# polarlightman/Scoring-rules-for-Gaussian-process-regression-a-new-approach-to-inference

Measured on AMD Instinct MI355X. Metric: GP fit+predict+CRPS wall-clock (ms) at n=20k full / n=40k FITC; HBM GB/s & MFMA%, higher is better.
Workload: dtype f64; 1 GPU; C3 full GP fit(NLML+LOO-CRPS+LOO-LogS)+predict+score; n=20000, d=8, n_test=5000, kernel=ARD, parallelism=single

## Files before the change

include/gpscore.h:

```cpp
#ifndef GPSCORE_H
#define GPSCORE_H

#include <stdint.h>

#ifdef __cplusplus
extern "C" {
#endif

typedef struct gps_ctx gps_ctx;

enum { GPS_ARD = 0, GPS_RBF = 1 };
enum { GPS_FULL = 0, GPS_LOWER = 1 };

enum {
  GPS_OBJ_NLML = 0,
  GPS_OBJ_LOO_CRPS = 1,
  GPS_OBJ_LOO_LOGS = 2,
  GPS_OBJ_LOGDET = 3,
  GPS_OBJ_QUAD = 4,
  GPS_N_OBJ = 5
};
enum {
  GPS_SC_CRPS = 0, GPS_SC_LOGS = 1, GPS_SC_MSLL = 2, GPS_SC_SMSE = 3,
  GPS_SC_MSE = 4, GPS_SC_COVER = 5, GPS_N_SC = 6
};

#define GPS_ABI_VERSION 800
int gps_version(void);
int gps_build_id(char* out, int cap);
int gps_ctx_create(int device, gps_ctx** out);
int gps_ctx_destroy(gps_ctx* ctx);
const char* gps_last_error(gps_ctx* ctx);
int gps_ctx_set_stream(gps_ctx* ctx, void* hip_stream);
void* gps_ctx_stream(gps_ctx* ctx);
int gps_ctx_synchronize(gps_ctx* ctx);

enum {
  GPS_OPT_OVERLAP = 0,
  GPS_OPT_GEMM_MAP = 3,
  GPS_OPT_TINY_GEMM = 7,
  GPS_OPT_GRAM_REG = 9,
  GPS_OPT_GRAPH = 10,
  GPS_OPT_PRED_PRE = 11,
  GPS_OPT_DAG = 12,
  GPS_OPT_AR_CHUNKS = 15,
  GPS_OPT_DAG_TILES = 13,
  GPS_OPT_STREAM_K = 18,
  GPS_OPT_DAG_WGS = 19,
  GPS_OPT_DAG_GROUP = 17,
  GPS_OPT_SLAB_XCD = 26,
  GPS_OPT_DAG_ORDER = 25,
  GPS_OPT_FITC_DEP = 27,
};
int gps_ctx_set_option(gps_ctx* ctx, int key, int value);

enum { GPS_STAT_GRAPHS = 0, GPS_STAT_GRAPH_CAP = 1, GPS_STAT_GRAPH_OVERFLOW = 2,
       GPS_STAT_DEVICE_BYTES = 3, GPS_STAT_GRAPH_DROPPED = 4, GPS_STAT_GRAPH_EVICTED = 5,
       GPS_N_STATS = 6 };
int gps_ctx_stats(gps_ctx* ctx, int64_t* out, int cap);

int gps_dag_task_list(int T, int flags, uint32_t* out, int cap);

typedef struct gps_gemm_desc {
  int32_t lay_a, lay_b, epi;
  int32_t M, N, K;
  int64_t lda, ldb, ldc;
  double alpha, beta;
  int32_t tri, tri_off;
  int32_t lower_out, mirror;
  int32_t kend;
  int32_t tile, ksplit, map_mode;
  int32_t use_ws, sk_alone, dep_mode;
  int32_t reserved;
  int64_t ld_out, c_kslice_stride;
} gps_gemm_desc;
enum { GPS_GEMM_PLAN_TILE = 0, GPS_GEMM_PLAN_KSPLIT = 1, GPS_GEMM_PLAN_MAP = 2,
       GPS_GEMM_PLAN_SK_DP = 3, GPS_GEMM_PLAN_SK_WGS = 4, GPS_GEMM_PLAN_SLAB_XCD = 5,
       GPS_GEMM_PLAN_GRID_X = 6, GPS_GEMM_PLAN_GRID_Y = 7, GPS_N_GEMM_PLAN = 8 };
int gps_gemm_diag_check(const gps_gemm_desc* d, int have_c, int have_kscale, int have_w,
                        const int32_t* kr, int have_out0, int have_out1);
int gps_gemm_diag(gps_ctx* ctx, const gps_gemm_desc* d, const double* A, const double* B,
                  double* C, const double* kscale, const double* w, const int32_t* kr,
                  double* out0, double* out1, int32_t* plan);
int64_t gps_gemm_schedule(const gps_gemm_desc* d, const int32_t* kr, int have_kscale, int slots,
                          int32_t* plan, int32_t* items, int64_t cap);

int gps_prof_enable(gps_ctx* ctx, int on);
int gps_prof_collect(gps_ctx* ctx, char* json_out, int64_t cap);
int gps_phase_enable(gps_ctx* ctx, int on);
int gps_phase_collect(gps_ctx* ctx, char* json_out, int64_t cap);
int gps_rccl_info(int* version, char* path, int cap);

int gps_gram(gps_ctx* ctx, int kind, const double* X, int64_t n, const double* Xp,
             int64_t m, int d, double log_sf2, const double* log_ell, int n_ell,
             double diag_add, int uplo, double* out);
int gps_potrf(gps_ctx* ctx, int64_t n, double* A, int64_t lda, double* logdet);
int gps_potrs(gps_ctx* ctx, int64_t n, int64_t nrhs, const double* A, int64_t lda,
              const double* B, int64_t ldb, double* X, int64_t ldx);
int gps_diag_inv(gps_ctx* ctx, int64_t n, const double* A, int64_t lda, double* dinv);
int gps_gemm(gps_ctx* ctx, int transA, int transB, int64_t M, int64_t N, int64_t K, double alpha,
             const double* A, int64_t lda, const double* B, int64_t ldb, double beta, double* C,
             int64_t ldc);
int gps_scores(gps_ctx* ctx, const double* mu, const double* var, const double* y,
               int64_t nt, double ytr_mean, double ytr_var_unbiased, double out[GPS_N_SC]);

int gps_full_set_data(gps_ctx* ctx, const double* X, const double* y, int64_t n, int d);
int gps_full_set_test(gps_ctx* ctx, const double* Xt, const double* yt, int64_t nt);
int gps_full_fit(gps_ctx* ctx, int kind, const double* theta, int n_ell,
                 double obj[GPS_N_OBJ], double* mu_loo, double* var_loo);
int gps_full_grad(gps_ctx* ctx, int kind, const double* theta, int n_ell, int objective,
                  double obj[GPS_N_OBJ], double* grad);
int gps_full_predict(gps_ctx* ctx, double* mu, double* var, double sc[GPS_N_SC]);

int gps_fitc_set_data(gps_ctx* ctx, const double* X, const double* y, int64_t n, int d,
                      double ytr_mean, double ytr_var_unbiased, int64_t n_total);
int gps_fitc_set_test(gps_ctx* ctx, const double* Xt, const double* yt, int64_t nt,
                      int64_t nt_total);
int gps_fitc_set_inducing(gps_ctx* ctx, const double* Z, int64_t m);
int gps_fitc_fit(gps_ctx* ctx, const double* theta, int n_ell, double obj[GPS_N_OBJ],
                 double* mu_loo, double* var_loo);
int gps_fitc_grad(gps_ctx* ctx, const double* theta, int n_ell, int objective,
                  double obj[GPS_N_OBJ], double* grad, double* grad_z);
int gps_fitc_predict(gps_ctx* ctx, double* mu, double* var, double sc[GPS_N_SC]);
int gps_fitc_intermediates(gps_ctx* ctx, double* Knm, double* lam, double* Lm_inv, double* Lb_inv,
                           double* Kmm);

enum { GPS_BLOCK_DSS = 0, GPS_BLOCK_KC = 1, GPS_BLOCK_ES = 2 };
int gps_full_blockloo(gps_ctx* ctx, int kind, const double* theta, int n_ell, int nfold,
                      int objective, double* value, double* grad, double* fold_values);
int gps_full_blockloo_es(gps_ctx* ctx, int kind, const double* theta, int n_ell, int nfold,
                         int num_sim, double beta, const double* draws, double* value,
                         double* grad, double* fold_values);
int gps_fitc_blockloo(gps_ctx* ctx, const double* theta, int n_ell, int nfold, int objective,
                      double* value, double* grad, double* grad_z, double* fold_values);
int gps_energy_score(gps_ctx* ctx, const double* m, const double* C, int64_t b, const double* y,
                     int num_sim, double beta, const double* draws, double* out);

int gps_full_predict_cov(gps_ctx* ctx, int64_t r0, int64_t r1, double* mu, double* cov,
                         int64_t ldc);
int gps_fitc_predict_cov(gps_ctx* ctx, int64_t r0, int64_t r1, double* mu, double* cov,
                         int64_t ldc);
enum { GPS_JOINT_DSS = 0, GPS_JOINT_ES = 1 };
int gps_full_predict_joint(gps_ctx* ctx, int nblock, int objective, int num_sim, double beta,
                           const double* draws, double* value, double* block_values);
int gps_fitc_predict_joint(gps_ctx* ctx, int nblock, int objective, int num_sim, double beta,
                           const double* draws, double* value, double* block_values);
int gps_full_predict_draws(gps_ctx* ctx, int64_t r0, int64_t r1, int nsamp, const double* xi,
                           double* out);
int gps_fitc_predict_draws(gps_ctx* ctx, int64_t r0, int64_t r1, int nsamp, const double* xi,
                           double* out);

enum { GPS_SURF_LOO_CRPS = 0, GPS_SURF_INSAMPLE_CRPS = 1, GPS_SURF_NLML = 2, GPS_SURF_LOO_LOGS = 3,
       GPS_N_SURF = 4 };
enum { GPS_SURF_LOGS_ADD_NOISE = 1 };
int gps_full_surface(gps_ctx* ctx, const double* X, const double* y, int64_t n, int d,
                     double log_sf2, const double* ell, int64_t n_ell, const double* noise_sd,
                     int64_t n_noise, int flags, double* out);

int gps_comm_unique_id(char uid[128]);
int gps_comm_init(gps_ctx* ctx, int nranks, int rank, const char uid[128]);
int gps_comm_init_local(gps_ctx* ctx, int nranks, int rank, long long group);
enum { GPS_COMM_NONE = 0, GPS_COMM_RCCL = 1, GPS_COMM_LOCAL = 2 };
int gps_comm_info(gps_ctx* ctx, int* nranks, int* rank, int* kind);
int gps_comm_destroy(gps_ctx* ctx);

#ifdef __cplusplus
}
#endif
#endif
```

scoring-rules-for-gaussian-process-regression-a-new-approach-to-inference_amd/csrc/api.hip:

```cpp
#include "api_internal.h"

namespace gpsapi {

thread_local std::string g_err;

int fail(gps_ctx* ctx, int code, const std::string& msg) {
  if (ctx) ctx->err = msg;
  g_err = msg;
  return code;
}

hipError_t sync_ctx_streams(gps_ctx* ctx) {
  for (hipStream_t st : {ctx->stream, ctx->side, ctx->aux[0], ctx->aux[1]})
    if (st) {
      const hipError_t e = hipStreamSynchronize(st);
      if (e != hipSuccess) return e;
    }
  return hipSuccess;
}

hipError_t drop_graphs_in(gps_ctx* ctx, const void* p, size_t bytes) {
  if (!ctx || !p || ctx->pgraphs.empty()) return hipSuccess;
  const uintptr_t lo = (uintptr_t)p, hi = lo + bytes;
  bool synced = false;
  for (size_t i = 0; i < ctx->pgraphs.size();) {
    bool hit = false;
    for (uintptr_t v : ctx->pgraphs[i].key) hit |= v >= lo && v < hi;
    if (!hit) { ++i; continue; }
    if (!synced) {
      const hipError_t e = sync_ctx_streams(ctx);
      if (e != hipSuccess) return e;
      synced = true;
    }
    const hipError_t e = hipGraphExecDestroy(ctx->pgraphs[i].exec);
    ctx->pgraphs.erase(ctx->pgraphs.begin() + (ptrdiff_t)i);
    ++ctx->graph_dropped;
    if (e != hipSuccess) return e;
  }
  return hipSuccess;
}

void forget_zeroed(gps_ctx* ctx, const void* p, size_t bytes) {
  const uintptr_t lo = (uintptr_t)p, hi = lo + bytes;
  for (auto it = ctx->zeroed.lower_bound(lo); it != ctx->zeroed.end() && it->first < hi;)
    it = ctx->zeroed.erase(it);
}

hipError_t ensure(gps_ctx* ctx, DBuf& b, size_t bytes) {
  if (bytes == 0) bytes = 16;
  if (b.cap >= bytes) return hipSuccess;
  if (b.p) {
    forget_zeroed(ctx, b.p, b.cap);
    hipError_t e = drop_graphs_in(ctx, b.p, b.cap);
    if (e != hipSuccess) return e;
    e = hipFree(b.p);
    if (e != hipSuccess) return e;
  }
  b.p = nullptr;
  b.cap = 0;
  hipError_t e = hipMalloc(&b.p, bytes);
  if (e == hipSuccess) b.cap = bytes;
  return e;
}
void release(gps_ctx* ctx, DBuf& b) {
  if (b.p) {
    forget_zeroed(ctx, b.p, b.cap);
    (void)drop_graphs_in(ctx, b.p, b.cap);
    (void)hipFree(b.p);
  }
  b.p = nullptr;
  b.cap = 0;
}

int get_event(gps_ctx* c) {
  if (c->ev_used == c->ev.size()) {
    hipEvent_t e;
    if (hipEventCreate(&e) != hipSuccess) return -1;
    c->ev.push_back(e);
  }
  return (int)c->ev_used++;
}


int phase_event(gps_ctx* c, hipStream_t st) {
  if (c->ph_used == c->ph_ev.size()) {
    hipEvent_t e;
    if (hipEventCreate(&e) != hipSuccess) return -1;
    c->ph_ev.push_back(e);
  }
  const int i = (int)c->ph_used++;
  return hipEventRecord(c->ph_ev[i], st) == hipSuccess ? i : -1;
}
void phase_mark(gps_ctx* c, const char* name) {
  if (!c->phase) return;
  const int e = phase_event(c, c->stream);
  if (e >= 0) c->ph_marks.push_back({name, e});
}

hipEvent_t sync_event(gps_ctx* c) {
  if (c->sync_used == c->sync_ev.size()) {
    hipEvent_t e;
    if (hipEventCreateWithFlags(&e, hipEventDisableTiming) != hipSuccess) return nullptr;
    c->sync_ev.push_back(e);
  }
  return c->sync_ev[c->sync_used++];
}


GemmParams gp0() {
  GemmParams p;
  memset(&p, 0, sizeof(p));
  p.alpha = 1.0;
  p.ksplit = 1;
  return p;
}

const char* gemm_tag(int al, int bl, int epi, const GemmParams& p) {
  (void)al;
  (void)bl;
  if (epi == EPI_COLRED) return "gemm_trmm_colred";
  if (epi == EPI_ROWSQ || epi == EPI_ROWSQ_DOT) return "gemm_rowsq";
  const int64_t tiles = (int64_t)(p.M / GPS_TILE) * (p.N / GPS_TILE) / (p.lower_out ? 2 : 1);
  const int cls = tiles < 16 ? 0 : (tiles < 256 ? 1 : 2);
  static const char* syrk[3] = {"gemm_syrk_s", "gemm_syrk_m", "gemm_syrk_l"};
  static const char* trmm[3] = {"gemm_trmm_s", "gemm_trmm_m", "gemm_trmm_l"};
  static const char* plain[3] = {"gemm_s", "gemm_m", "gemm_l"};
  if (p.lower_out) return p.ksplit > 1 ? "gemm_syrk_splitk" : syrk[cls];
  return p.tri ? trmm[cls] : plain[cls];
}

double gemm_flops(const GemmParams& p) {
  const double M = p.M, N = p.N, K = p.K;
  if (p.lower_out && p.tri == TRI_K_GE_I) {
    double f = 0.0;
    for (int64_t i = 0; i < p.M; i += GPS_TILE) f += (double)(i + GPS_TILE) * (K - i);
    return 2.0 * GPS_TILE * f;
  }
  if (p.lower_out) return M * (M + 1) * K;
  if ((p.tri == TRI_K_LE_I || p.tri == TRI_K_LE_J) && p.tri_off) {
    const double len = p.tri == TRI_K_LE_I ? M : N, other = p.tri == TRI_K_LE_I ? N : M;
    const double o = p.tri_off, e = std::min<double>(K, o + len);
    return other * (e * e - o * o) + 2.0 * other * K * std::max(0.0, o + len - e);
  }
  if (p.tri) return M * N * K;
  return 2.0 * M * N * K;
}

int gemm(gps_ctx* ctx, int al, int bl, int epi, const GemmParams& p, hipStream_t st,
         GemmLaunchInfo* info) {
  if (!st) st = ctx->stream;
  GemmParams q = p;
  if (q.map_mode == 0) q.map_mode = ctx->gemm_map;
  if (epi == EPI_STORE && (q.ksplit == 1 || q.tile == 64) && !q.ws) {
    DBuf& ws = st == ctx->side      ? ctx->ws_side
               : st == ctx->aux[0] ? ctx->ws_aux[0]
               : st == ctx->aux[1] ? ctx->ws_aux[1]
                                   : ctx->ws_main;
    HIPCHK(ensure(ctx, ws, (size_t)kSplitWsDoubles * 8));
    q.ws = ws.d();
    q.ws_cap = kSplitWsDoubles;
    if (st == ctx->stream && ctx->sk_cnt.p) {
      q.sk_cnt = static_cast<int*>(ctx->sk_cnt.p);
      q.sk_slots = 2 * ctx->ncu;
    }
  }
  std::string tag = gemm_tag(al, bl, epi, p);
  if (ctx->prof > 1) {
    const GemmPlan plan = gemm_plan(epi, q, q.ws ? q.ws_cap : 0);
    char buf[160];
    snprintf(buf, sizeof(buf), " %c%c %dx%dx%d tri%d t%d ks%d ld%lld", al ? 'T' : 'N',
             bl ? 'T' : 'N', p.M, p.N, p.K, (int)p.tri, plan.tile, plan.ksplit, (long long)p.lda);
    tag += buf;
  }
  Prof pr(ctx, tag, gemm_flops(p), 0, st);
  HIPCHK(launch_gemm(al, bl, epi, q, st, info));
  return 0;
}

int gram(gps_ctx* ctx, const char* tag, const double* x, int n, const double* xp, int m, int d,
         const Theta& th, double diag_add, int lower, int pad_identity, double* out, int64_t ldo,
         int M, int N, hipStream_t st) {
  GramParams g;
  memset(&g, 0, sizeof(g));
  g.x = x;
  g.xp = xp;
  g.out = out;
  g.ldo = ldo;
  g.n = n;
  g.m = m;
  g.M = M;
  g.N = N;
  g.d = d;
  g.sf2 = th.sf2;
  g.diag_add = diag_add;
  g.lower = lower;
  g.pad_identity = pad_identity;
  for (int k = 0; k < d; ++k) g.inv_ell[k] = th.inv_ell[k];
  const double elems = lower ? 0.5 * (double)M * (M + 1) : (double)M * N;
  Prof pr(ctx, tag, 0, 8.0 * elems, st);
  HIPCHK(launch_gram(g, st ? st : ctx->stream));
  return 0;
}

int pred_rows(gps_ctx* ctx, int64_t r0, int64_t r1, const double* w, hipStream_t st) {
  const int64_t np = ctx->n_pad, ntp = ctx->nt_pad, tiles_m = np / GPS_TILE;
  GemmParams p = gp0();
  p.A = ctx->Linv.d() + r0 * np; p.lda = np; p.B = ctx->Ksf.d(); p.ldb = np;
  p.M = (int)(r1 - r0); p.N = (int)ntp; p.K = (int)r1; p.tri = TRI_K_LE_I; p.tri_off = (int)r0;
  p.w = w + r0;
  p.out0 = ctx->pslab.d() + (r0 / GPS_TILE) * ntp;
  p.out1 = ctx->pslab.d() + (tiles_m + r0 / GPS_TILE) * ntp;
  p.ld_out = ntp;
  return gemm(ctx, LAY_N, LAY_T, EPI_COLRED, p, st);
}

int fitc_rowsq_cols(gps_ctx* ctx, const double* Lx, int64_t c0, int64_t c1, hipStream_t st) {
  const int64_t np = ctx->fn_pad, mp = ctx->m_pad;
  GemmParams p = gp0();
  p.A = ctx->Knm.d(); p.lda = mp; p.B = Lx + c0 * mp; p.ldb = mp;
  p.M = (int)np; p.N = (int)(c1 - c0); p.K = (int)c1; p.tri = TRI_K_LE_J; p.tri_off = (int)c0;
  p.kend = (int)pad_to(ctx->m, 16);
  p.out0 = ctx->fslab.d() + (c0 / GPS_TILE) * np; p.ld_out = np;
  return gemm(ctx, LAY_N, LAY_T, EPI_ROWSQ, p, st);
}

int fitc_rowsq_dep(gps_ctx* ctx, const double* L, int* sig, int64_t ncols, int mode,
                   hipStream_t st, int64_t nb_dag) {
  const int64_t np = ctx->fn_pad, mp = ctx->m_pad;
  GemmParams p = gp0();
  p.A = ctx->Knm.d(); p.lda = mp; p.B = L; p.ldb = mp;
  p.M = (int)np; p.N = (int)ncols; p.K = (int)ncols; p.tri = TRI_K_LE_J;
  p.kend = (int)pad_to(ctx->m, 16);
  p.out0 = ctx->fslab.d(); p.ld_out = np;
  p.dep_sig = sig; p.dep_q = sig + kSigQueue; p.dep_err = static_cast<int*>(ctx->info.p) + 1;
  p.dep_grid = dag_width(ctx, nb_dag, true); p.dep_mode = mode;
  return gemm(ctx, LAY_N, LAY_T, EPI_ROWSQ, p, st);
}

int dag_list_key(const gps_ctx* ctx, int64_t nb) {
  return (int)(3 * nb + ctx->dag_order);
}

bool dag_block(const gps_ctx* ctx, int64_t nb) { return ctx->dag && nb >= 2 && nb <= ctx->dag_tiles; }

void dag_blocks(const gps_ctx* ctx, int64_t nb, std::vector<int>& sizes, int64_t& cnt) {
  if (nb <= 1) return;
  if (dag_block(ctx, nb)) {
    sizes.push_back((int)nb);
    cnt += dag_cnt_ints((int)nb);
    return;
  }
  dag_blocks(ctx, nb / 2, sizes, cnt);
  dag_blocks(ctx, nb - nb / 2, sizes, cnt);
}

int dag_width(const gps_ctx* ctx, int64_t nb, bool half) {
  const int auto_w = half ? std::max(4, ctx->ncu / 2) : ctx->ncu;
  return (int)std::min<int64_t>(ctx->dag_wgs > 0 ? ctx->dag_wgs : auto_w, std::max<int64_t>(4, 2 * nb * nb));
}

int potrf_inv_rec(gps_ctx* ctx, double* A, int64_t lda, double* Linv, int64_t ldl, double* W,
                  int nb, double* logdiag, int* info, int base, int nreal, double* Lout,
                  int64_t ldlo, bool top) {
  hipStream_t s = ctx->stream;
  if (nb == 1) {
    Prof pr(ctx, "potrf_diag128", 2.0 * 128 * 128 * 128 / 3.0, 0);
    HIPCHK(launch_potrf_leaf(A, lda, Linv, ldl, Lout, ldlo, logdiag, info, base, nreal, s));
    return 0;
  }
  if (dag_block(ctx, nb)) {
    auto it = ctx->dag_lists.find(dag_list_key(ctx, nb));
    const int64_t need = dag_cnt_ints(nb);
    if (it == ctx->dag_lists.end() || ctx->dag_cnt_used + need > (int64_t)(ctx->dag_cnt.cap / 4))
      return fail(ctx, -2, "persistent factorisation: task list / counters not prepared");
    DagParams d;
    d.A = A; d.lda = lda; d.Linv = Linv; d.ldl = ldl; d.Lout = Lout; d.ldlo = ldlo;
    d.logdiag = logdiag; d.info = info; d.base = base; d.nreal = nreal; d.T = nb;
    d.tasks = static_cast<const uint32_t*>(it->second.first.p); d.ntasks = it->second.second;
    d.cnt = static_cast<int*>(ctx->dag_cnt.p) + ctx->dag_cnt_used;
    d.spin_ticks = 200000000ull;
    d.group = ctx->dag_group;
    d.sig = ctx->dag_sig;
    ctx->dag_sig = nullptr;
    ctx->dag_cnt_used += need;
    const double nn = 128.0 * nb;
    Prof pr(ctx, "potrf_dag", 2.0 * nn * nn * nn / 3.0, 0);
    HIPCHK(launch_potrf_dag(d, dag_width(ctx, nb, ctx->dag_half), s));
    return 0;
  }
  const int n1b = nb / 2, n2b = nb - n1b;
  const int n1 = n1b * GPS_TILE, n2 = n2b * GPS_TILE;
  double* A21 = A + (int64_t)n1 * lda;
  double* A22 = A21 + n1;
  double* Li21 = Linv + (int64_t)n1 * ldl;
  double* Li22 = Li21 + n1;
  int rc;
  const bool pre_here = top && ctx->pre.kind == PRE_FITC_Q && ctx->pre.n1 == n1;
  const bool pre_dep = pre_here && ctx->pre.sig && ctx->overlap && dag_block(ctx, n1b);
  auto join_dep = [&]() {
    if (!pre_dep) return;
    hipEvent_t j = sync_event(ctx);
    if (j && hipEventRecord(j, ctx->aux[1]) == hipSuccess) (void)hipStreamWaitEvent(s, j, 0);
  };
  if (pre_dep) {
    hipEvent_t f = sync_event(ctx);
    if (!f) return fail(ctx, -2, "hipEventCreate failed");
    HIPCHK(hipEventRecord(f, s));
    HIPCHK(hipStreamWaitEvent(ctx->aux[1], f, 0));
    if ((rc = fitc_rowsq_dep(ctx, Linv, ctx->pre.sig, n1, 1, ctx->aux[1], n1b))) {
      join_dep();
      return rc;
    }
    ctx->dag_sig = ctx->pre.sig;
  }
  rc = potrf_inv_rec(ctx, A, lda, Linv, ldl, W, n1b, logdiag, info, base, nreal, Lout, ldlo);
  ctx->dag_sig = nullptr;
  if (rc) {
    join_dep();
    return rc;
  }
  {
    GemmParams p = gp0();
    p.A = A21; p.lda = lda; p.B = Linv; p.ldb = ldl; p.C = W; p.ldc = n1;
    p.M = n2; p.N = n1; p.K = n1; p.tri = TRI_K_LE_J;
    if ((rc = gemm(ctx, LAY_N, LAY_T, EPI_STORE, p))) return rc;
  }
  if (Lout) HIPCHK(hipMemcpy2DAsync(Lout + (int64_t)n1 * ldlo, ldlo * 8, W, (size_t)n1 * 8,
                                    (size_t)n1 * 8, n2, hipMemcpyDeviceToDevice, s));
  const bool forked = ctx->overlap;
  hipStream_t ts = forked ? ctx->side : s;
  hipEvent_t fork = sync_event(ctx), join = sync_event(ctx);
  if (!fork || !join) return fail(ctx, -2, "hipEventCreate failed");
  if (forked) {
    HIPCHK(hipEventRecord(fork, s));
    HIPCHK(hipStreamWaitEvent(ts, fork, 0));
  }
  {
    GemmParams p = gp0();
    p.A = W; p.lda = n1; p.B = W; p.ldb = n1; p.C = A22; p.ldc = lda;
    p.M = n2; p.N = n2; p.K = n1; p.alpha = -1.0; p.beta = 1.0; p.lower_out = 1;
    p.sk_alone = forked ? 0 : 1;
    if ((rc = gemm(ctx, LAY_N, LAY_T, EPI_STORE, p))) return rc;
  }
  {
    GemmParams p = gp0();
    p.A = W; p.lda = n1; p.B = Linv; p.ldb = ldl; p.C = A21; p.ldc = lda;
    p.M = n2; p.N = n1; p.K = n1; p.tri = TRI_K_GE_J;
    if ((rc = gemm(ctx, LAY_N, LAY_N, EPI_STORE, p, ts))) return rc;
  }
  if (forked) HIPCHK(hipEventRecord(join, ts));
  if (pre_here) {
    hipStream_t ps = !ctx->overlap ? s : pre_dep ? ctx->aux[1] : ctx->aux[0];
    if (ps != s) {
      hipEvent_t f = sync_event(ctx);
      ctx->pre.join = sync_event(ctx);
      if (!f || !ctx->pre.join) return fail(ctx, -2, "hipEventCreate failed");
      HIPCHK(hipEventRecord(f, s));
      HIPCHK(hipStreamWaitEvent(ps, f, 0));
    }
    if ((rc = pre_dep ? fitc_rowsq_dep(ctx, Linv, ctx->pre.sig, n1, 2, ps, n1b)
                      : fitc_rowsq_cols(ctx, Linv, 0, n1, ps)))
      return rc;
    if (ps != s) HIPCHK(hipEventRecord(ctx->pre.join, ps));
  }
  if ((rc = potrf_inv_rec(ctx, A22, lda, Li22, ldl, W + (int64_t)n1 * n2, n2b, logdiag + n1, info,
                          base + n1, nreal - n1, Lout ? Lout + (int64_t)n1 * ldlo + n1 : nullptr,
                          ldlo)))
    return rc;
  if (forked) HIPCHK(hipStreamWaitEvent(s, join, 0));
  {
    GemmParams p = gp0();
    p.A = Li22; p.lda = ldl; p.B = A21; p.ldb = lda; p.C = Li21; p.ldc = ldl;
    p.M = n2; p.N = n1; p.K = n2; p.alpha = -1.0; p.tri = TRI_K_LE_I;
    if ((rc = gemm(ctx, LAY_N, LAY_N, EPI_STORE, p))) return rc;
  }
  if (top && ctx->pre.join) {
    HIPCHK(hipStreamWaitEvent(s, ctx->pre.join, 0));
    ctx->pre.join = nullptr;
  }
  return 0;
}

size_t potrf_ws_doubles(int64_t n_pad) {
  int64_t nb = n_pad / GPS_TILE, tot = 0;
  while (nb > 1) {
    const int64_t n1 = (nb / 2) * GPS_TILE, n2 = (nb - nb / 2) * GPS_TILE;
    tot += n1 * n2;
    nb = nb - nb / 2;
  }
  return (size_t)std::max<int64_t>(tot, GPS_TILE * GPS_TILE);
}

int reset_info(gps_ctx* ctx) {
  HIPCHK(hipMemsetAsync(ctx->info.p, 0x7f, 2 * sizeof(int), ctx->stream));
  return 0;
}


hipError_t zero_factor(gps_ctx* ctx, double* p, int64_t n_pad, hipStream_t s) {
  const hipError_t e = hipMemsetAsync(p, 0, (size_t)n_pad * n_pad * 8, s);
  if (e == hipSuccess) ctx->zeroed[(uintptr_t)p] = n_pad;
  return e;
}
bool factor_zeroed(const gps_ctx* ctx, const double* p, int64_t n_pad) {
  const auto it = ctx->zeroed.find((uintptr_t)p);
  return it != ctx->zeroed.end() && it->second == n_pad;
}

int potrf_inv(gps_ctx* ctx, double* A, int64_t n_pad, double* Linv, double* W, double* logdiag,
              int nreal, double* Lout) {
  if (!factor_zeroed(ctx, Linv, n_pad) || (Lout && !factor_zeroed(ctx, Lout, n_pad)))
    return fail(ctx, -1, "potrf_inv: factor buffer not zeroed for this size (internal contract)");
  std::vector<int> dsizes;
  int64_t dcnt = 0;
  dag_blocks(ctx, n_pad / GPS_TILE, dsizes, dcnt);
  for (int T : dsizes) {
    const int lk = dag_list_key(ctx, T);
    if (ctx->dag_lists.count(lk)) continue;
    const std::vector<uint32_t> tl = dag_task_list(T, ctx->dag_order, true);
    auto& e = ctx->dag_lists[lk];
    HIPCHK(ensure(ctx, e.first, tl.size() * 4));
    HIPCHK(hipMemcpyAsync(e.first.p, tl.data(), tl.size() * 4, hipMemcpyHostToDevice, ctx->stream));
    HIPCHK(hipStreamSynchronize(ctx->stream));
    e.second = (int)tl.size();
  }
  if (dcnt && ctx->dag_cnt.cap < (size_t)dcnt * 4) {
    HIPCHK(hipStreamSynchronize(ctx->stream));
    HIPCHK(ensure(ctx, ctx->dag_cnt, std::max<size_t>((size_t)dcnt * 4, (size_t)1 << 20)));
    HIPCHK(hipMemsetAsync(ctx->dag_cnt.p, 0, ctx->dag_cnt.cap, ctx->stream));
    HIPCHK(hipStreamSynchronize(ctx->stream));
  }
  auto eager = [&]() {
    ctx->sync_used = 0;
    ctx->pre.join = nullptr;
    ctx->dag_cnt_used = 0;
    return potrf_inv_rec(ctx, A, n_pad, Linv, n_pad, W, (int)(n_pad / GPS_TILE), logdiag,
                         static_cast<int*>(ctx->info.p), 0, nreal, Lout, n_pad, true);
  };
  if (!ctx->graphs || ctx->prof || n_pad <= GPS_TILE) return eager();
  HIPCHK(ensure(ctx, ctx->ws_main, (size_t)kSplitWsDoubles * 8));
  HIPCHK(ensure(ctx, ctx->ws_side, (size_t)kSplitWsDoubles * 8));
  const bool pre = ctx->pre.kind == PRE_FITC_Q;
  std::vector<uintptr_t> key = {
      (uintptr_t)A, (uintptr_t)n_pad, (uintptr_t)Linv, (uintptr_t)W, (uintptr_t)logdiag,
      (uintptr_t)nreal, (uintptr_t)Lout, (uintptr_t)ctx->stream, (uintptr_t)ctx->side,
      (uintptr_t)ctx->overlap, (uintptr_t)ctx->gemm_map,
      (uintptr_t)g_tiny_gemm, (uintptr_t)g_stream_k, (uintptr_t)g_slab_xcd, (uintptr_t)ctx->info.p, (uintptr_t)ctx->ws_main.p,
      (uintptr_t)ctx->ws_side.p, (uintptr_t)pre,
      pre ? (uintptr_t)ctx->pre.n1 : 0, pre ? (uintptr_t)ctx->aux[0] : 0,
      pre ? (uintptr_t)ctx->Knm.p : 0, pre ? (uintptr_t)ctx->fslab.p : 0,
      pre ? (uintptr_t)ctx->fn_pad : 0, pre ? (uintptr_t)ctx->m_pad : 0, pre ? (uintptr_t)ctx->pre.sig : 0,
      (uintptr_t)ctx->dag, (uintptr_t)ctx->dag_tiles, (uintptr_t)ctx->dag_group, (uintptr_t)ctx->dag_wgs, (uintptr_t)ctx->dag_half,
      (uintptr_t)ctx->dag_cnt.p, (uintptr_t)ctx->sk_cnt.p, (uintptr_t)ctx->dag_sig};
  for (int T : dsizes) key.push_back((uintptr_t)ctx->dag_lists[dag_list_key(ctx, T)].first.p);
  for (auto& g : ctx->pgraphs)
    if (g.key == key) {
      g.last_use = ++ctx->graph_tick;
      HIPCHK(hipGraphLaunch(g.exec, ctx->stream));
      return 0;
    }
  if (ctx->pgraphs.size() >= kMaxGraphs) {
    size_t lru = 0;
    for (size_t i = 1; i < ctx->pgraphs.size(); ++i)
      if (ctx->pgraphs[i].last_use < ctx->pgraphs[lru].last_use) lru = i;
    HIPCHK(sync_ctx_streams(ctx));
    const hipError_t e = hipGraphExecDestroy(ctx->pgraphs[lru].exec);
    ctx->pgraphs.erase(ctx->pgraphs.begin() + (ptrdiff_t)lru);
    ++ctx->graph_evicted;
    HIPCHK(e);
  }
  const size_t nev = 2 * (size_t)(n_pad / GPS_TILE) + 8;
  while (ctx->sync_ev.size() < nev) {
    hipEvent_t e;
    HIPCHK(hipEventCreateWithFlags(&e, hipEventDisableTiming));
    ctx->sync_ev.push_back(e);
  }
  HIPCHK(hipStreamBeginCapture(ctx->stream, hipStreamCaptureModeThreadLocal));
  int rc = eager();
  hipGraph_t graph = nullptr;
  const hipError_t ec = hipStreamEndCapture(ctx->stream, &graph);
  if (rc || ec != hipSuccess) {
    if (graph) (void)hipGraphDestroy(graph);
    if (rc) return rc;
    HIPCHK(ec);
  }
  hipGraphExec_t exec = nullptr;
  const hipError_t ei = hipGraphInstantiate(&exec, graph, nullptr, nullptr, 0);
  (void)hipGraphDestroy(graph);
  HIPCHK(ei);
  ctx->pgraphs.push_back({key, exec, ++ctx->graph_tick});
  HIPCHK(hipGraphLaunch(exec, ctx->stream));
  return 0;
}

int check_info(gps_ctx* ctx) {
  HIPCHK(hipMemcpyAsync(ctx->hinfo, ctx->info.p, 2 * sizeof(int), hipMemcpyDeviceToHost, ctx->stream));
  HIPCHK(hipStreamSynchronize(ctx->stream));
  if (ctx->hinfo[1] == 2)
    return fail(ctx, -4, "persistent factorisation: the task queue did not run to completion "
                         "(counters not zero at launch; internal error)");
  if (ctx->hinfo[1] != 0x7f7f7f7f)
    return fail(ctx, -4, "persistent factorisation: a task's dependency wait timed out (internal error)");
  const int info = *ctx->hinfo;
  if (info != 0x7f7f7f7f) {
    char buf[160];
    snprintf(buf, sizeof(buf),
             "cholesky: the leading minor of order %d is not positive definite", info);
    return fail(ctx, info, buf);
  }
  return 0;
}

int set_theta(gps_ctx* ctx, Theta& th, int kind, const double* theta, int n_ell, int d) {
  ARGCHK(theta != nullptr, "theta is NULL");
  ARGCHK(kind == GPS_ARD || kind == GPS_RBF, "kind must be GPS_ARD or GPS_RBF");
  ARGCHK(n_ell == 1 || n_ell == d, "n_ell must be 1 or d");
  th.kind = kind;
  th.sf2 = std::exp(theta[0]);
  th.sn2 = std::exp(theta[1 + n_ell]);
  for (int k = 0; k < d; ++k) {
    const double b = theta[1 + (n_ell == 1 ? 0 : k)];
    th.inv_ell[k] = kind == GPS_ARD ? std::exp(-b) : std::exp(-0.5 * b);
  }
  return 0;
}

int upload(gps_ctx* ctx, DBuf& b, const double* h, int64_t rows, int64_t cols, int64_t rows_pad) {
  HIPCHK(ensure(ctx, b, (size_t)rows_pad * cols * 8));
  HIPCHK(hipMemsetAsync(b.p, 0, (size_t)rows_pad * cols * 8, ctx->stream));
  if (rows * cols)
    HIPCHK(hipMemcpyAsync(b.p, h, (size_t)rows * cols * 8, hipMemcpyHostToDevice, ctx->stream));
  return 0;
}

void score_bundle(const double* sums, double nt, double out[GPS_N_SC]) {
  out[GPS_SC_CRPS] = sums[0] / nt;
  out[GPS_SC_LOGS] = sums[1] / nt;
  out[GPS_SC_MSLL] = sums[2] / nt;
  out[GPS_SC_SMSE] = sums[3] / sums[4];
  out[GPS_SC_MSE] = sums[3] / nt;
  out[GPS_SC_COVER] = sums[5] / nt;
}

int bind(gps_ctx* ctx) {
  if (!ctx) {
    g_err = "NULL context";
    return -1;
  }
  HIPCHK(hipSetDevice(ctx->device));
  return 0;
}

bool sharded(const gps_ctx* ctx) { return ctx->comm != nullptr || ctx->lgroup != nullptr; }



std::vector<DBuf*> ctx_buffers(gps_ctx* ctx) {
  return {&ctx->info, &ctx->small, &ctx->X, &ctx->y, &ctx->Xt, &ctx->yt, &ctx->A,
                 &ctx->Linv, &ctx->W, &ctx->logdiag, &ctx->beta, &ctx->alpha, &ctx->dinv,
                 &ctx->slab, &ctx->mu_loo, &ctx->var_loo, &ctx->Ksf, &ctx->s1, &ctx->s2,
                 &ctx->mu, &ctx->var, &ctx->Lout, &ctx->pslab, &ctx->fX, &ctx->fy, &ctx->fXt, &ctx->fyt,
                 &ctx->Z, &ctx->Kmm, &ctx->Am, &ctx->Lm, &ctx->Lb, &ctx->ldm, &ctx->ldb,
                 &ctx->Knm, &ctx->q, &ctx->lam, &ctx->ilam, &ctx->ys, &ctx->slabB, &ctx->red,
                 &ctx->c, &ctx->tvec, &ctx->r, &ctx->g, &ctx->fmu_loo, &ctx->fvar_loo,
                 &ctx->Ksm, &ctx->qm, &ctx->qb, &ctx->fmu, &ctx->fvar, &ctx->fslab, &ctx->fslab_pre, &ctx->t0,
                 &ctx->t1, &ctx->t2, &ctx->t3, &ctx->t4, &ctx->ws_main, &ctx->ws_side, &ctx->ws_aux[0], &ctx->ws_aux[1],
                 &ctx->gu, &ctx->gct, &ctx->gv, &ctx->Mx, &ctx->gslab, &ctx->gout, &ctx->fgv,
                 &ctx->fgm, &ctx->fgB, &ctx->fR, &ctx->fgred, &ctx->fgslab, &ctx->fgout, &ctx->bP,
                 &ctx->bL, &ctx->bPI, &ctx->bH, &ctx->bvec, &ctx->bGblk, &ctx->bT, &ctx->bkr,
                 &ctx->bEf, &ctx->bF, &ctx->ebuf, &ctx->edraws,
                 &ctx->bSg, &ctx->bBf, &ctx->bLf, &ctx->bldf, &ctx->bRem, &ctx->bW, &ctx->bkv,
                 &ctx->bLR, &ctx->bLRv,
                 &ctx->ebuf_aux[0], &ctx->ebuf_aux[1], &ctx->ebuf_aux[2], &ctx->bPIs, &ctx->bRW, &ctx->escale, &ctx->bfv, &ctx->rpart, &ctx->dag_cnt, &ctx->sk_cnt, &ctx->dsig,
                 &ctx->jK, &ctx->jV, &ctx->jslab, &ctx->jS, &ctx->jL, &ctx->jLo, &ctx->jW, &ctx->jvec,
                 &ctx->jE, &ctx->jdraws, &ctx->jxi, &ctx->jout};
}


std::mutex g_groups_mu;
std::map<long long, std::weak_ptr<LocalGroup>> g_groups;

}

extern "C" {

int gps_version(void) { return GPS_ABI_VERSION; }


int make_aux_streams(gps_ctx* ctx) {
  for (hipStream_t* a : {&ctx->side, &ctx->aux[0], &ctx->aux[1]})
    HIPCHK(hipStreamCreateWithFlags(a, hipStreamNonBlocking));
  return 0;
}
int gps_ctx_create(int device, gps_ctx** out) {
  gps_ctx* ctx = nullptr;
  if (!out) return fail(nullptr, -1, "out is NULL");
  int ndev = 0;
  hipError_t e = hipGetDeviceCount(&ndev);
  if (e != hipSuccess || ndev == 0)
    return fail(nullptr, -2, std::string("no HIP device: ") + hipGetErrorString(e));
  if (device < 0 || device >= ndev) return fail(nullptr, -1, "device index out of range");
  ctx = new gps_ctx();
  ctx->device = device;
  HIPCHK(hipSetDevice(device));
  HIPCHK(hipStreamCreateWithFlags(&ctx->stream, hipStreamNonBlocking));
  HIPCHK(hipDeviceGetAttribute(&ctx->ncu, hipDeviceAttributeMultiprocessorCount, device));
  if (int rc = make_aux_streams(ctx)) return rc;
  HIPCHK(hipHostMalloc((void**)&ctx->hsmall, 256 * sizeof(double), hipHostMallocDefault));
  HIPCHK(hipHostMalloc((void**)&ctx->hinfo, 16, hipHostMallocDefault));
  HIPCHK(ensure(ctx, ctx->info, 16));
  HIPCHK(ensure(ctx, ctx->small, 256 * sizeof(double)));
  HIPCHK(ensure(ctx, ctx->sk_cnt, (size_t)kStreamKTiles * sizeof(int)));
  HIPCHK(hipMemsetAsync(ctx->sk_cnt.p, 0, (size_t)kStreamKTiles * sizeof(int), ctx->stream));
  HIPCHK(hipStreamSynchronize(ctx->stream));
  *out = ctx;
  return 0;
}

int gps_ctx_destroy(gps_ctx* ctx) {
  if (!ctx) return 0;
  (void)hipSetDevice(ctx->device);
  for (hipStream_t st : {ctx->stream, ctx->side, ctx->aux[0], ctx->aux[1]})
    if (st) (void)hipStreamSynchronize(st);
  if (ctx->comm) ncclCommDestroy(ctx->comm);
  leave_local_group(ctx);
  for (auto& g : ctx->pgraphs) (void)hipGraphExecDestroy(g.exec);
  ctx->pgraphs.clear();
  for (DBuf* b : ctx_buffers(ctx)) release(ctx, *b);
  for (auto& kv : ctx->dag_lists) release(ctx, kv.second.first);
  for (hipEvent_t e : ctx->ev) (void)hipEventDestroy(e);
  for (hipEvent_t e : ctx->ph_ev) (void)hipEventDestroy(e);
  for (hipEvent_t e : ctx->sync_ev) (void)hipEventDestroy(e);
  for (hipEvent_t e : ctx->ar_ev) (void)hipEventDestroy(e);
  for (hipEvent_t e : {ctx->pre_fork, ctx->pre_join, ctx->preb_fork, ctx->kn_fork, ctx->kn_join,
                       ctx->b_fork, ctx->b_join})
    if (e) (void)hipEventDestroy(e);
  if (ctx->side) (void)hipStreamDestroy(ctx->side);
  for (hipStream_t l : ctx->aux)
    if (l) (void)hipStreamDestroy(l);
  if (ctx->hsmall) (void)hipHostFree(ctx->hsmall);
  if (ctx->hinfo) (void)hipHostFree(ctx->hinfo);
  if (ctx->own_stream && ctx->stream) (void)hipStreamDestroy(ctx->stream);
  delete ctx;
  return 0;
}

const char* gps_last_error(gps_ctx* ctx) { return ctx ? ctx->err.c_str() : g_err.c_str(); }

int gps_ctx_set_stream(gps_ctx* ctx, void* hip_stream) {
  if (int rc = bind(ctx)) return rc;
  HIPCHK(hipStreamSynchronize(ctx->stream));
  if (ctx->own_stream && ctx->stream) HIPCHK(hipStreamDestroy(ctx->stream));
  if (hip_stream) {
    ctx->stream = static_cast<hipStream_t>(hip_stream);
    ctx->own_stream = false;
  } else {
    HIPCHK(hipStreamCreateWithFlags(&ctx->stream, hipStreamNonBlocking));
    ctx->own_stream = true;
  }
  return 0;
}

int gps_ctx_set_option(gps_ctx* ctx, int key, int value) {
  if (int rc = bind(ctx)) return rc;
  switch (key) {
    case GPS_OPT_OVERLAP: ctx->overlap = value != 0; return 0;
    case GPS_OPT_GEMM_MAP:
      ARGCHK(value >= 0 && value <= 6, "GPS_OPT_GEMM_MAP must be in 0..6");
      ctx->gemm_map = value;
      return 0;
    case GPS_OPT_AR_CHUNKS:
      ARGCHK(value >= 1 && value <= 64, "GPS_OPT_AR_CHUNKS must be in 1..64");
      ctx->ar_chunks = value;
      return 0;
    case GPS_OPT_TINY_GEMM: g_tiny_gemm = value != 0; return 0;
    case GPS_OPT_STREAM_K:
      ARGCHK(value >= 0 && value <= 2, "GPS_OPT_STREAM_K must be 0, 1 or 2");
      g_stream_k = value;
      return 0;
    case GPS_OPT_SLAB_XCD: g_slab_xcd = value != 0; return 0;
    case GPS_OPT_GRAM_REG:
      ARGCHK(value >= 0 && value <= 2, "GPS_OPT_GRAM_REG must be 0, 1 or 2");
      g_gram_reg = value;
      return 0;
    case GPS_OPT_GRAPH: ctx->graphs = value != 0; return 0;
    case GPS_OPT_PRED_PRE: ctx->pred_pre = value != 0; return 0;
    case GPS_OPT_DAG: ctx->dag = value != 0; return 0;
    case GPS_OPT_DAG_WGS:
      ARGCHK(value >= 0, "GPS_OPT_DAG_WGS must be >= 0");
      ctx->dag_wgs = value;
      return 0;
    case GPS_OPT_FITC_DEP: ctx->fitc_dep = value != 0; return 0;
    case GPS_OPT_DAG_ORDER:
      ARGCHK(value >= 0 && value <= 2, "GPS_OPT_DAG_ORDER must be 0, 1 or 2");
      ctx->dag_order = value;
      return 0;
    case GPS_OPT_DAG_GROUP:
      ARGCHK(value >= 2 && value <= 4, "GPS_OPT_DAG_GROUP must be 2, 3 or 4");
      ctx->dag_group = value;
      return 0;
    case GPS_OPT_DAG_TILES:
      ARGCHK(value >= 2 && value <= 64, "GPS_OPT_DAG_TILES must be in 2..64");
      ctx->dag_tiles = value;
      return 0;
    default: return fail(ctx, -1, "unknown option");
  }
}

void* gps_ctx_stream(gps_ctx* ctx) { return ctx ? (void*)ctx->stream : nullptr; }

int gps_ctx_synchronize(gps_ctx* ctx) {
  if (int rc = bind(ctx)) return rc;
  HIPCHK(hipStreamSynchronize(ctx->stream));
  return 0;
}

int gps_ctx_stats(gps_ctx* ctx, int64_t* out, int cap) {
  if (int rc = bind(ctx)) return rc;
  ARGCHK(out != nullptr && cap >= 0, "out is NULL or cap < 0");
  size_t bytes = 0;
  for (DBuf* b : ctx_buffers(ctx)) bytes += b->cap;
  int64_t v[GPS_N_STATS];
  v[GPS_STAT_GRAPHS] = (int64_t)ctx->pgraphs.size();
  v[GPS_STAT_GRAPH_CAP] = (int64_t)kMaxGraphs;
  v[GPS_STAT_GRAPH_OVERFLOW] = ctx->graph_overflow;
  v[GPS_STAT_GRAPH_DROPPED] = ctx->graph_dropped;
  v[GPS_STAT_GRAPH_EVICTED] = ctx->graph_evicted;
  v[GPS_STAT_DEVICE_BYTES] = (int64_t)bytes;
  for (int i = 0; i < cap && i < GPS_N_STATS; ++i) out[i] = v[i];
  return GPS_N_STATS;
}

int gps_dag_task_list(int T, int flags, uint32_t* out, int cap) {
  if (T < 2 || T > 64 || cap < 0 || (cap > 0 && !out) || (flags & ~13))
    return fail(nullptr, -1, "bad arguments");
  const std::vector<uint32_t> tl = dag_task_list(T, (flags >> 2 & 3) == 0 ? 1 : (flags >> 2 & 3) == 3 ? 0 : flags >> 2 & 3,
                                                 (flags & 1) != 0);
  for (int i = 0; i < cap && i < (int)tl.size(); ++i) out[i] = tl[i];
  return (int)tl.size();
}

int gps_phase_enable(gps_ctx* ctx, int on) {
  if (int rc = bind(ctx)) return rc;
  ctx->phase = on != 0;
  return 0;
}

int gps_phase_collect(gps_ctx* ctx, char* json_out, int64_t cap) {
  if (int rc = bind(ctx)) return rc;
  HIPCHK(sync_ctx_streams(ctx));
  std::map<std::string, std::pair<int, double>> agg;
  std::vector<std::string> order;
  for (size_t i = 1; i < ctx->ph_marks.size(); ++i) {
    const auto& m = ctx->ph_marks[i];
    if (m.first == "start") continue;
    float ms = 0.f;
    HIPCHK(hipEventElapsedTime(&ms, ctx->ph_ev[ctx->ph_marks[i - 1].second], ctx->ph_ev[m.second]));
    if (!agg.count(m.first)) order.push_back(m.first);
    agg[m.first].first += 1;
    agg[m.first].second += ms;
  }
  std::string js = "{\"phases\": {";
  for (size_t i = 0; i < order.size(); ++i) {
    char buf[160];
    snprintf(buf, sizeof(buf), "%s\"%s\": {\"count\": %d, \"ms\": %.6f}", i ? ", " : "",
             order[i].c_str(), agg[order[i]].first, agg[order[i]].second);
    js += buf;
  }
  js += "}, \"allreduce\": [";
  for (size_t i = 0; i < ctx->ph_ar.size(); ++i) {
    float ms = 0.f;
    HIPCHK(hipEventElapsedTime(&ms, ctx->ph_ev[ctx->ph_ar[i].e0], ctx->ph_ev[ctx->ph_ar[i].e1]));
    char buf[96];
    snprintf(buf, sizeof(buf), "%s[%.0f, %.6f]", i ? ", " : "", ctx->ph_ar[i].bytes, ms);
    js += buf;
  }
  js += "]}";
  ctx->ph_marks.clear();
  ctx->ph_ar.clear();
  ctx->ph_used = 0;
  if (!json_out || cap <= (int64_t)js.size()) return fail(ctx, -1, "json buffer too small");
  memcpy(json_out, js.c_str(), js.size() + 1);
  return 0;
}

int gps_rccl_info(int* version, char* path, int cap) {
  if (!version || !path || cap < 1) return fail(nullptr, -1, "bad arguments");
  *version = 0;
  if (ncclGetVersion(version) != ncclSuccess) return fail(nullptr, -3, "ncclGetVersion failed");
  Dl_info di;
  memset(&di, 0, sizeof(di));
  const char* f = dladdr(reinterpret_cast<void*>(&ncclAllReduce), &di) && di.dli_fname ? di.dli_fname : "";
  snprintf(path, (size_t)cap, "%s", f);
  return 0;
}

int gps_prof_enable(gps_ctx* ctx, int on) {
  if (int rc = bind(ctx)) return rc;
  ctx->prof = on;
  return 0;
}

int gps_prof_collect(gps_ctx* ctx, char* json_out, int64_t cap) {
  if (int rc = bind(ctx)) return rc;
  HIPCHK(hipStreamSynchronize(ctx->stream));
  struct Agg { int count = 0; double ms = 0, flop = 0, bytes = 0; };
  std::map<std::string, Agg> agg;
  for (const ProfRec& r : ctx->recs) {
    float ms = 0.f;
    HIPCHK(hipEventElapsedTime(&ms, ctx->ev[r.e0], ctx->ev[r.e1]));
    Agg& a = agg[r.tag];
    a.count++;
    a.ms += ms;
    a.flop += r.flop;
    a.bytes += r.bytes;
  }
  ctx->recs.clear();
  ctx->ev_used = 0;
  std::string js = "{";
  bool first = true;
  for (auto& kv : agg) {
    char buf[256];
    snprintf(buf, sizeof(buf), "%s\"%s\": {\"count\": %d, \"ms\": %.6f, \"flop\": %.6e, \"bytes\": %.6e}",
             first ? "" : ", ", kv.first.c_str(), kv.second.count, kv.second.ms, kv.second.flop,
             kv.second.bytes);
    js += buf;
    first = false;
  }
  js += "}";
  if (!json_out || cap <= (int64_t)js.size()) return fail(ctx, -1, "json buffer too small");
  memcpy(json_out, js.c_str(), js.size() + 1);
  return 0;
}

int gps_gram(gps_ctx* ctx, int kind, const double* X, int64_t n, const double* Xp, int64_t m, int d,
             double log_sf2, const double* log_ell, int n_ell, double diag_add, int uplo,
             double* out) {
  if (int rc = bind(ctx)) return rc;
  ARGCHK(X && Xp && out && log_ell, "NULL argument");
  ARGCHK(n > 0 && m > 0 && d >= 1 && d <= GPS_MAX_D, "bad shape");
  ARGCHK(uplo == GPS_FULL || (uplo == GPS_LOWER && n == m), "uplo=LOWER needs a square Gram");
  std::vector<double> theta(n_ell + 2);
  theta[0] = log_sf2;
  for (int k = 0; k < n_ell; ++k) theta[1 + k] = log_ell[k];
  theta[1 + n_ell] = 0.0;
  Theta th;
  if (int rc = set_theta(ctx, th, kind, theta.data(), n_ell, d)) return rc;
  const int64_t M = pad_to(n, 32), N = pad_to(m);
  if (int rc = upload(ctx, ctx->t0, X, n, d, n)) return rc;
  if (int rc = upload(ctx, ctx->t1, Xp, m, d, m)) return rc;
  HIPCHK(ensure(ctx, ctx->t2, (size_t)M * N * 8));
  HIPCHK(hipMemsetAsync(ctx->t2.p, 0, (size_t)M * N * 8, ctx->stream));
  if (int rc = gram(ctx, "gram_user", ctx->t0.d(), (int)n, ctx->t1.d(), (int)m, d, th, diag_add,
                    uplo == GPS_LOWER, 0, ctx->t2.d(), N, (int)M, (int)N))
    return rc;
  HIPCHK(hipMemcpy2DAsync(out, (size_t)m * 8, ctx->t2.p, (size_t)N * 8, (size_t)m * 8, n,
                          hipMemcpyDeviceToHost, ctx->stream));
  HIPCHK(hipStreamSynchronize(ctx->stream));
  return 0;
}

int factor_user(gps_ctx* ctx, int64_t n, const double* A, int64_t lda, bool want_L) {
  ARGCHK(A && n > 0 && lda >= n, "bad matrix argument");
  const int64_t np = pad_to(n);
  HIPCHK(ensure(ctx, ctx->t0, (size_t)n * lda * 8));
  HIPCHK(hipMemcpyAsync(ctx->t0.p, A, (size_t)n * lda * 8, hipMemcpyHostToDevice, ctx->stream));
  HIPCHK(ensure(ctx, ctx->t1, (size_t)np * np * 8));
  HIPCHK(launch_pad_copy(ctx->t0.d(), lda, ctx->t1.d(), np, (int)n, (int)n, (int)np, (int)np, 1,
                         ctx->stream));
  HIPCHK(ensure(ctx, ctx->t2, (size_t)np * np * 8));
  HIPCHK(zero_factor(ctx, ctx->t2.d(), np, ctx->stream));
  HIPCHK(ensure(ctx, ctx->t3, potrf_ws_doubles(np) * 8));
  HIPCHK(ensure(ctx, ctx->t4, (size_t)np * 8 * (want_L ? np + 1 : 1)));
  double* logdiag = ctx->t4.d();
  double* Lout = want_L ? ctx->t4.d() + np : nullptr;
  if (want_L) HIPCHK(zero_factor(ctx, Lout, np, ctx->stream));
  if (int rc = reset_info(ctx)) return rc;
  if (int rc = potrf_inv(ctx, ctx->t1.d(), np, ctx->t2.d(), ctx->t3.d(), logdiag, (int)n, Lout))
    return rc;
  return check_info(ctx);
}

int gps_potrf(gps_ctx* ctx, int64_t n, double* A, int64_t lda, double* logdet) {
  if (int rc = bind(ctx)) return rc;
  if (int rc = factor_user(ctx, n, A, lda, true)) return rc;
  const int64_t np = pad_to(n);
  HIPCHK(launch_dot(ctx->t4.d(), nullptr, (int)np, ctx->small.d(), ctx->stream));
  HIPCHK(hipMemcpy2DAsync(A, (size_t)lda * 8, ctx->t4.d() + np, (size_t)np * 8, (size_t)n * 8, n,
                          hipMemcpyDeviceToHost, ctx->stream));
  HIPCHK(hipMemcpyAsync(ctx->hsmall, ctx->small.p, 8, hipMemcpyDeviceToHost, ctx->stream));
  HIPCHK(hipStreamSynchronize(ctx->stream));
  if (logdet) *logdet = 2.0 * ctx->hsmall[0];
  return 0;
}

int gps_potrs(gps_ctx* ctx, int64_t n, int64_t nrhs, const double* A, int64_t lda, const double* B,
              int64_t ldb, double* X, int64_t ldx) {
  if (int rc = bind(ctx)) return rc;
  ARGCHK(B && X && nrhs > 0 && ldb >= nrhs && ldx >= nrhs, "bad rhs argument");
  if (int rc = factor_user(ctx, n, A, lda, false)) return rc;
  const int64_t np = pad_to(n), rp = pad_to(nrhs);
  HIPCHK(ensure(ctx, ctx->t0, (size_t)n * ldb * 8));
  HIPCHK(hipMemcpyAsync(ctx->t0.p, B, (size_t)n * ldb * 8, hipMemcpyHostToDevice, ctx->stream));
  DBuf Bp, Y;
  HIPCHK(ensure(ctx, Bp, (size_t)np * rp * 8));
  HIPCHK(ensure(ctx, Y, (size_t)np * rp * 8));
  int rc = 0;
  do {
    hipError_t e = launch_pad_copy(ctx->t0.d(), ldb, Bp.d(), rp, (int)n, (int)nrhs, (int)np,
                                   (int)rp, 0, ctx->stream);
    if (e != hipSuccess) { rc = fail(ctx, -2, hipGetErrorString(e)); break; }
    GemmParams p = gp0();
    p.A = ctx->t2.d(); p.lda = np; p.B = Bp.d(); p.ldb = rp; p.C = Y.d(); p.ldc = rp;
    p.M = (int)np; p.N = (int)rp; p.K = (int)np; p.tri = TRI_K_LE_I;
    if ((rc = gemm(ctx, LAY_N, LAY_N, EPI_STORE, p))) break;
    GemmParams q = gp0();
    q.A = ctx->t2.d(); q.lda = np; q.B = Y.d(); q.ldb = rp; q.C = Bp.d(); q.ldc = rp;
    q.M = (int)np; q.N = (int)rp; q.K = (int)np; q.tri = TRI_K_GE_I;
    if ((rc = gemm(ctx, LAY_T, LAY_N, EPI_STORE, q))) break;
    e = hipMemcpy2DAsync(X, (size_t)ldx * 8, Bp.p, (size_t)rp * 8, (size_t)nrhs * 8, n,
                         hipMemcpyDeviceToHost, ctx->stream);
    if (e == hipSuccess) e = hipStreamSynchronize(ctx->stream);
    if (e != hipSuccess) rc = fail(ctx, -2, hipGetErrorString(e));
  } while (0);
  release(ctx, Bp);
  release(ctx, Y);
  return rc;
}

int gps_diag_inv(gps_ctx* ctx, int64_t n, const double* A, int64_t lda, double* dinv) {
  if (int rc = bind(ctx)) return rc;
  ARGCHK(dinv, "dinv is NULL");
  if (int rc = factor_user(ctx, n, A, lda, false)) return rc;
  const int64_t np = pad_to(n);
  const int64_t nchunk = (np + 255) / 256;
  HIPCHK(ensure(ctx, ctx->t0, (size_t)(nchunk * np * 2 + np) * 8));
  double* out = ctx->t0.d() + nchunk * np * 2;
  HIPCHK(launch_colred(ctx->t2.d(), np, (int)np, (int)np, 1, nullptr, nullptr, nullptr, out,
                       ctx->t0.d(), ctx->stream));
  HIPCHK(hipMemcpyAsync(dinv, out, (size_t)n * 8, hipMemcpyDeviceToHost, ctx->stream));
  HIPCHK(hipStreamSynchronize(ctx->stream));
  return 0;
}

int gps_gemm(gps_ctx* ctx, int transA, int transB, int64_t M, int64_t N, int64_t K, double alpha,
             const double* A, int64_t lda, const double* B, int64_t ldb, double beta, double* C,
             int64_t ldc) {
  if (int rc = bind(ctx)) return rc;
  ARGCHK(A && B && C && M > 0 && N > 0 && K > 0, "bad gemm argument");
  const int64_t Mp = pad_to(M), Np = pad_to(N), Kp = pad_to(K);
  const int64_t ar = transA ? K : M, ac = transA ? M : K, arp = transA ? Kp : Mp, acp = transA ? Mp : Kp;
  const int64_t br = transB ? N : K, bc = transB ? K : N, brp = transB ? Np : Kp, bcp = transB ? Kp : Np;
  ARGCHK(lda >= ac && ldb >= bc && ldc >= N, "leading dimension too small");
  HIPCHK(ensure(ctx, ctx->t0, (size_t)(ar * lda + br * ldb + M * ldc) * 8));
  double* rawA = ctx->t0.d();
  double* rawB = rawA + ar * lda;
  double* rawC = rawB + br * ldb;
  HIPCHK(hipMemcpyAsync(rawA, A, (size_t)ar * lda * 8, hipMemcpyHostToDevice, ctx->stream));
  HIPCHK(hipMemcpyAsync(rawB, B, (size_t)br * ldb * 8, hipMemcpyHostToDevice, ctx->stream));
  HIPCHK(ensure(ctx, ctx->t1, (size_t)(arp * acp + brp * bcp + Mp * Np) * 8));
  double* pA = ctx->t1.d();
  double* pB = pA + arp * acp;
  double* pC = pB + brp * bcp;
  HIPCHK(launch_pad_copy(rawA, lda, pA, acp, (int)ar, (int)ac, (int)arp, (int)acp, 0, ctx->stream));
  HIPCHK(launch_pad_copy(rawB, ldb, pB, bcp, (int)br, (int)bc, (int)brp, (int)bcp, 0, ctx->stream));
  if (beta != 0.0) {
    HIPCHK(hipMemcpyAsync(rawC, C, (size_t)M * ldc * 8, hipMemcpyHostToDevice, ctx->stream));
    HIPCHK(launch_pad_copy(rawC, ldc, pC, Np, (int)M, (int)N, (int)Mp, (int)Np, 0, ctx->stream));
  }
  GemmParams p = gp0();
  p.A = pA; p.lda = acp; p.B = pB; p.ldb = bcp; p.C = pC; p.ldc = Np;
  p.M = (int)Mp; p.N = (int)Np; p.K = (int)Kp; p.alpha = alpha; p.beta = beta;
  if (int rc = gemm(ctx, transA ? LAY_T : LAY_N, transB ? LAY_T : LAY_N, EPI_STORE, p)) return rc;
  HIPCHK(hipMemcpy2DAsync(C, (size_t)ldc * 8, pC, (size_t)Np * 8, (size_t)N * 8, M,
                          hipMemcpyDeviceToHost, ctx->stream));
  HIPCHK(hipStreamSynchronize(ctx->stream));
  return 0;
}

double* row_part(gps_ctx* ctx, int64_t rows, int nv) {
  if (ensure(ctx, ctx->rpart, (size_t)(std::max<int64_t>(rows, 1) + 255) / 256 * nv * 8) != hipSuccess)
    return nullptr;
  return ctx->rpart.d();
}

int gps_scores(gps_ctx* ctx, const double* mu, const double* var, const double* y, int64_t nt,
               double ytr_mean, double ytr_var_unbiased, double out[GPS_N_SC]) {
  if (int rc = bind(ctx)) return rc;
  ARGCHK(mu && var && y && out && nt > 0, "bad argument");
  if (int rc = upload(ctx, ctx->t0, mu, nt, 1, nt)) return rc;
  if (int rc = upload(ctx, ctx->t1, var, nt, 1, nt)) return rc;
  if (int rc = upload(ctx, ctx->t2, y, nt, 1, nt)) return rc;
  double* part = row_part(ctx, nt, 6);
  ARGCHK(part != nullptr, "out of device memory");
  HIPCHK(launch_score_sums(ctx->t0.d(), ctx->t1.d(), ctx->t2.d(), (int)nt, ytr_mean,
                           ytr_var_unbiased, ctx->small.d(), part, ctx->stream));
  HIPCHK(hipMemcpyAsync(ctx->hsmall, ctx->small.p, 6 * 8, hipMemcpyDeviceToHost, ctx->stream));
  HIPCHK(hipStreamSynchronize(ctx->stream));
  score_bundle(ctx->hsmall, (double)nt, out);
  return 0;
}

}
```

scoring-rules-for-gaussian-process-regression-a-new-approach-to-inference_amd/csrc/api_diag.hip:

```cpp
#include "api_internal.h"

static_assert(sizeof(gps_gemm_desc) == 128, "gps_gemm_desc layout");

namespace gpsapi {

struct DiagExtents {
  int64_t a, b, c, kscale, w, kr, out0, out1;
};

static bool diag_check(const gps_gemm_desc& d, bool have_c, bool have_kscale, bool have_w,
                       const int32_t* kr, bool have_out0, bool have_out1, DiagExtents& x,
                       std::string& why) {
#define DIAG_REQ(cond, msg) \
  do {                      \
    if (!(cond)) {          \
      why = msg;            \
      return false;         \
    }                       \
  } while (0)
  DIAG_REQ(d.dep_mode == 0, "dep_mode: the dependent row-norm launch cannot run alone");
  DIAG_REQ((d.lay_a == LAY_N || d.lay_a == LAY_T) && (d.lay_b == LAY_N || d.lay_b == LAY_T),
           "layouts must be 0 or 1");
  DIAG_REQ(d.epi == EPI_STORE || d.epi == EPI_ROWSQ || d.epi == EPI_COLRED || d.epi == EPI_ROWSQ_DOT,
           "unknown epilogue");
  DIAG_REQ(d.M > 0 && d.N > 0 && d.K > 0 && d.M % GPS_TILE == 0 && d.N % GPS_TILE == 0 && d.K % 16 == 0,
           "M and N must be positive multiples of 128, K of 16");
  DIAG_REQ(d.M <= (1 << 18) && d.N <= (1 << 18) && (int64_t)d.M * d.N <= ((int64_t)1 << 27) &&
               d.K <= 65536,
           "M, N <= 2^18 with M*N <= 2^27, and K <= 65536");
  DIAG_REQ(d.lda > 0 && d.lda % 2 == 0 && d.lda >= (d.lay_a == LAY_N ? d.K : d.M) && d.lda <= (1 << 20),
           "lda must be even and at least A's stored row length");
  DIAG_REQ(d.ldb > 0 && d.ldb % 2 == 0 && d.ldb >= (d.lay_b == LAY_N ? d.N : d.K) && d.ldb <= (1 << 20),
           "ldb must be even and at least B's stored row length");
  DIAG_REQ(d.tri >= TRI_NONE && d.tri <= TRI_KR_J, "unknown tri mode");
  DIAG_REQ(d.tri_off >= 0 && d.tri_off % 16 == 0 && d.tri_off <= (1 << 24),
           "tri_off must be a non-negative multiple of 16");
  DIAG_REQ(d.tri_off == 0 || (d.tri >= TRI_K_LE_I && d.tri <= TRI_K_GE_I),
           "tri_off needs one of the four triangular k-range modes");
  if (d.tri == TRI_KR_J) {
    DIAG_REQ(kr != nullptr, "TRI_KR_J needs kr");
    for (int g = 0; g < 2 * (d.N / 16); ++g)
      DIAG_REQ(kr[g] >= 0 && kr[g] <= d.K && kr[g] % 16 == 0,
               "kr entries must be multiples of 16 in [0, K]");
  }
  DIAG_REQ(d.kend >= 0 && d.kend % 16 == 0, "kend must be 0 or a positive multiple of 16");
  DIAG_REQ((d.lower_out == 0 || d.lower_out == 1) && (d.mirror == 0 || d.mirror == 1),
           "lower_out and mirror are flags");
  DIAG_REQ(!d.lower_out || d.M == d.N, "lower_out needs a square output");
  DIAG_REQ(!d.mirror || d.lower_out, "mirror needs lower_out");
  DIAG_REQ(d.tile == 0 || d.tile == 16 || d.tile == 32 || d.tile == 64 || d.tile == 128,
           "tile must be 0, 16, 32, 64 or 128");
  DIAG_REQ(d.ksplit >= 1 && d.ksplit <= 8, "ksplit must be in 1..8");
  DIAG_REQ(d.map_mode >= 0 && d.map_mode <= 6, "map_mode must be in 0..6");
  DIAG_REQ(d.map_mode != 3 || (!d.lower_out && d.tri >= TRI_K_LE_I && d.tri <= TRI_K_GE_I),
           "map_mode 3 needs a triangular operand and a full output");
  const bool small = d.tile == 16 || d.tile == 32;
  if (small) {
    DIAG_REQ(d.epi == EPI_STORE && !have_kscale, "the small kernel has no epilogue and no kscale");
    DIAG_REQ(d.ksplit == 1 || d.ksplit == 2 || d.ksplit == 4,
             "the small kernel runs 1, 2 or 4 waves per block");
  }
  DIAG_REQ(d.tile != 64 || d.epi == EPI_STORE, "the epilogues run on 128-tiles");
  x = DiagExtents{};
  x.a = (int64_t)(d.lay_a == LAY_N ? d.M : d.K) * d.lda;
  x.b = (int64_t)(d.lay_b == LAY_N ? d.K : d.N) * d.ldb;
  x.kscale = have_kscale ? d.K : 0;
  x.kr = d.tri == TRI_KR_J ? 2 * (d.N / 16) : 0;
  const bool split = !small && d.ksplit > 1;
  if (d.epi == EPI_STORE) {
    DIAG_REQ(have_c, "C is NULL");
    DIAG_REQ(d.ldc > 0 && d.ldc % 2 == 0 && d.ldc >= d.N && d.ldc <= (1 << 20),
             "ldc must be even and at least N");
    x.c = (int64_t)d.M * d.ldc;
    if (split && d.use_ws) {
      DIAG_REQ((int64_t)d.ksplit * d.M * d.N <= kSplitWsDoubles, "the slabs exceed the workspace");
    } else if (split) {
      DIAG_REQ(d.tile == 0 || d.tile == 128, "the unslabbed split runs on 128-tiles");
      DIAG_REQ(d.beta == 0.0 && !d.mirror, "the unslabbed split needs beta 0 and no mirror");
      DIAG_REQ(d.c_kslice_stride % 2 == 0 && d.c_kslice_stride >= x.c &&
                   d.c_kslice_stride <= ((int64_t)1 << 32),
               "c_kslice_stride must be even and at least M*ldc");
      x.c = (int64_t)d.ksplit * d.c_kslice_stride;
    }
  } else {
    DIAG_REQ(d.lay_a == LAY_N && d.lay_b == LAY_T, "the epilogues exist for A [i][k], B [j][k] only");
    DIAG_REQ(d.tile == 0 || d.tile == 128, "the epilogues run on 128-tiles");
    DIAG_REQ(d.ksplit == 1 && !d.mirror, "the epilogues take no split and no mirror");
    DIAG_REQ(have_out0 && d.ld_out > 0 && d.ld_out <= (1 << 20), "out0 / ld_out missing");
    if (d.epi == EPI_COLRED) {
      DIAG_REQ(have_w && have_out1, "EPI_COLRED needs w and out1");
      DIAG_REQ(d.ld_out >= d.N, "ld_out must be at least N");
      x.w = d.M;
      x.out0 = x.out1 = (int64_t)(d.M / GPS_TILE) * d.ld_out;
    } else {
      DIAG_REQ(d.ld_out >= d.M, "ld_out must be at least M");
      x.out0 = (int64_t)(d.N / GPS_TILE) * d.ld_out;
      if (d.epi == EPI_ROWSQ_DOT) {
        DIAG_REQ(have_w && have_out1, "EPI_ROWSQ_DOT needs w and out1");
        DIAG_REQ(d.tri == TRI_K_LE_J && d.K == d.tri_off + d.N,
                 "EPI_ROWSQ_DOT needs TRI_K_LE_J with K = tri_off + N");
        x.w = d.K;
        x.out1 = d.M;
      }
    }
  }
#undef DIAG_REQ
  return true;
}

static GemmParams desc_params(const gps_gemm_desc& d) {
  GemmParams p = gp0();
  p.lda = d.lda; p.ldb = d.ldb; p.ldc = d.ldc; p.c_kslice_stride = d.c_kslice_stride;
  p.M = d.M; p.N = d.N; p.K = d.K; p.alpha = d.alpha; p.beta = d.beta; p.ld_out = d.ld_out;
  p.lower_out = d.lower_out; p.ksplit = d.ksplit; p.tri = d.tri; p.tri_off = d.tri_off;
  p.map_mode = d.map_mode; p.tile = d.tile; p.mirror = d.mirror; p.kend = d.kend;
  p.sk_alone = d.sk_alone;
  return p;
}
static bool own_slabs(const gps_gemm_desc& d) {
  return d.ksplit > 1 && d.tile != 16 && d.tile != 32 && d.tile != 64 && d.use_ws;
}

}

extern "C" {

int gps_gemm_diag_check(const gps_gemm_desc* d, int have_c, int have_kscale, int have_w,
                        const int32_t* kr, int have_out0, int have_out1) {
  if (!d) return fail(nullptr, -1, "description is NULL");
  DiagExtents x;
  std::string why;
  if (!diag_check(*d, have_c != 0, have_kscale != 0, have_w != 0, kr, have_out0 != 0,
                  have_out1 != 0, x, why))
    return fail(nullptr, -1, "gps_gemm_diag: " + why);
  return 0;
}

int gps_gemm_diag(gps_ctx* ctx, const gps_gemm_desc* d, const double* A, const double* B,
                  double* C, const double* kscale, const double* w, const int32_t* kr,
                  double* out0, double* out1, int32_t* plan) {
  if (!d || !A || !B || !plan) return fail(ctx, -1, "gps_gemm_diag: NULL argument");
  DiagExtents x;
  std::string why;
  if (!diag_check(*d, C != nullptr, kscale != nullptr, w != nullptr, kr, out0 != nullptr,
                  out1 != nullptr, x, why))
    return fail(ctx, -1, "gps_gemm_diag: " + why);
  if (int rc = bind(ctx)) return rc;
  hipStream_t s = ctx->stream;
  auto even = [](int64_t n) { return (n + 1) & ~(int64_t)1; };
  HIPCHK(ensure(ctx, ctx->t0, (size_t)(even(x.a) + even(x.b)) * 8));
  HIPCHK(ensure(ctx, ctx->t1, (size_t)std::max<int64_t>(even(x.c), 2) * 8));
  HIPCHK(ensure(ctx, ctx->t2, (size_t)(even(x.kscale) + even(x.w) + even(x.out0) + even(x.out1) +
                                       even((x.kr + 1) / 2) + 2) * 8));
  double* dA = ctx->t0.d();
  double* dB = dA + even(x.a);
  double* dC = ctx->t1.d();
  double* dks = ctx->t2.d();
  double* dw = dks + even(x.kscale);
  double* do0 = dw + even(x.w);
  double* do1 = do0 + even(x.out0);
  int* dkr = reinterpret_cast<int*>(do1 + even(x.out1));
  auto up = [&](void* dst, const void* src, int64_t bytes) {
    return bytes ? hipMemcpyAsync(dst, src, (size_t)bytes, hipMemcpyHostToDevice, s) : hipSuccess;
  };
  HIPCHK(up(dA, A, x.a * 8));
  HIPCHK(up(dB, B, x.b * 8));
  HIPCHK(up(dC, C, x.c * 8));
  HIPCHK(up(dks, kscale, x.kscale * 8));
  HIPCHK(up(dw, w, x.w * 8));
  HIPCHK(up(do0, out0, x.out0 * 8));
  HIPCHK(up(do1, out1, x.out1 * 8));
  HIPCHK(up(dkr, kr, x.kr * 4));
  GemmParams p = desc_params(*d);
  p.A = dA; p.B = dB; p.C = x.c ? dC : nullptr;
  p.kscale = x.kscale ? dks : nullptr;
  p.w = x.w ? dw : nullptr;
  p.out0 = x.out0 ? do0 : nullptr; p.out1 = x.out1 ? do1 : nullptr;
  p.kr = x.kr ? dkr : nullptr;
  if (own_slabs(*d)) {
    HIPCHK(ensure(ctx, ctx->ws_main, (size_t)kSplitWsDoubles * 8));
    p.ws = ctx->ws_main.d();
    p.ws_cap = kSplitWsDoubles;
  }
  GemmLaunchInfo info{};
  if (int rc = gemm(ctx, d->lay_a, d->lay_b, d->epi, p, nullptr, &info)) return rc;
  auto down = [&](void* dst, const void* src, int64_t bytes) {
    return bytes ? hipMemcpyAsync(dst, src, (size_t)bytes, hipMemcpyDeviceToHost, s) : hipSuccess;
  };
  HIPCHK(down(C, dC, x.c * 8));
  HIPCHK(down(out0, do0, x.out0 * 8));
  HIPCHK(down(out1, do1, x.out1 * 8));
  HIPCHK(hipStreamSynchronize(s));
  const int v[GPS_N_GEMM_PLAN] = {info.tile, info.ksplit, info.map_mode, info.sk_dp,
                                  info.sk_wgs, info.slab_xcd, info.grid_x, info.grid_y};
  for (int i = 0; i < GPS_N_GEMM_PLAN; ++i) plan[i] = v[i];
  return 0;
}

int64_t gps_gemm_schedule(const gps_gemm_desc* d, const int32_t* kr, int have_kscale, int slots,
                          int32_t* plan, int32_t* items, int64_t cap) {
  if (!d || !plan || cap < 0 || (cap > 0 && !items) || slots < 0 || slots > 4096)
    return fail(nullptr, -1, "gps_gemm_schedule: bad argument");
  DiagExtents x;
  std::string why;
  if (!diag_check(*d, true, have_kscale != 0, true, kr, true, true, x, why))
    return fail(nullptr, -1, "gps_gemm_schedule: " + why);
  static double mark[2];
  GemmParams p = desc_params(*d);
  p.A = p.B = mark; p.C = p.out0 = p.out1 = mark; p.w = mark;
  p.kscale = have_kscale ? mark : nullptr;
  p.kr = d->tri == TRI_KR_J ? kr : nullptr;
  if (own_slabs(*d) || (d->epi == EPI_STORE && (p.ksplit == 1 || p.tile == 64))) {
    p.ws = mark;
    p.ws_cap = kSplitWsDoubles;
    if (!own_slabs(*d) && slots > 0) {
      p.sk_cnt = reinterpret_cast<int*>(mark);
      p.sk_slots = slots;
    }
  }
  GemmLaunchInfo info{};
  const int64_t n = gemm_schedule(d->lay_a, d->lay_b, d->epi, p, info, items, cap);
  if (n < 0) return fail(nullptr, -1, "gps_gemm_schedule: launch_gemm refuses the launch");
  const int v[GPS_N_GEMM_PLAN] = {info.tile, info.ksplit, info.map_mode, info.sk_dp,
                                  info.sk_wgs, info.slab_xcd, info.grid_x, info.grid_y};
  for (int i = 0; i < GPS_N_GEMM_PLAN; ++i) plan[i] = v[i];
  return n;
}

}
```

scoring-rules-for-gaussian-process-regression-a-new-approach-to-inference_amd/csrc/api_internal.h:

```cpp
#pragma once
#include <dlfcn.h>
#include <rccl/rccl.h>
#include <stdio.h>
#include <string.h>

#include <chrono>
#include <climits>
#include <cmath>
#include <condition_variable>
#include <map>
#include <memory>
#include <mutex>
#include <string>
#include <vector>

#include "gps_internal.h"
#include "gpscore.h"

using namespace gps;

namespace gpsapi {


struct DBuf {
  void* p = nullptr;
  size_t cap = 0;
  double* d() const { return static_cast<double*>(p); }
};

struct ProfRec {
  std::string tag;
  int e0, e1;
  double flop, bytes;
};

struct Theta {
  int kind = GPS_ARD;
  double sf2 = 1.0, sn2 = 1.0;
  double inv_ell[GPS_MAX_D];
};

struct LocalGroup {
  std::mutex mu;
  std::condition_variable cv;
  int n = 0, arrived = 0;
  uint64_t gen = 0;
  size_t count = 0;
  bool mismatch = false, last_mismatch = false;
  bool aborted = false;
  std::vector<std::vector<double>> in;
  std::vector<double> sum;
  std::vector<char> taken;
  int joined = 0;
  int device = -1;
  bool device_ok = true;
  std::vector<double*> stage;
  std::vector<size_t> stage_cap;
  std::vector<hipEvent_t> ready, done;
  std::vector<hipStream_t> gstream;
  std::vector<hipEvent_t> staged, summed;
  ~LocalGroup() {
    for (hipEvent_t e : done)
      if (e) (void)hipEventSynchronize(e);
    for (hipStream_t g : gstream)
      if (g) {
        (void)hipStreamSynchronize(g);
        (void)hipStreamDestroy(g);
      }
    for (const std::vector<hipEvent_t>* v : {&ready, &done, &staged, &summed})
      for (hipEvent_t e : *v)
        if (e) (void)hipEventDestroy(e);
    for (double* p : stage)
      if (p) (void)hipFree(p);
  }
};

extern std::mutex g_groups_mu;
extern std::map<long long, std::weak_ptr<LocalGroup>> g_groups;

}
using namespace gpsapi;


enum { PRE_NONE = 0, PRE_FITC_Q = 1 };

struct gps_ctx {
  int device = 0;
  hipStream_t stream = nullptr;
  bool own_stream = true;
  hipStream_t side = nullptr;
  hipStream_t aux[2] = {nullptr, nullptr};
  bool overlap = true;
  int gemm_map = 0;
  int ar_chunks = 4;
  std::vector<hipEvent_t> ar_ev;
  int ncu = 0;
  std::vector<hipEvent_t> sync_ev;
  size_t sync_used = 0;
  bool graphs = true;
  bool pred_pre = true;
  bool dag = true;
  int dag_tiles = 20;
  int dag_group = 3;
  int dag_wgs = 0;
  int dag_order = 1;
  bool dag_half = false;
  bool fitc_dep = true;
  int* dag_sig = nullptr;
  DBuf dsig;
  std::map<int, std::pair<DBuf, int>> dag_lists;
  std::map<uintptr_t, int64_t> zeroed;
  DBuf dag_cnt;
  DBuf sk_cnt;
  int64_t dag_cnt_used = 0;
  struct PrePass {
    int kind = 0;
    int64_t n1 = 0;
    const double* L = nullptr;
    hipEvent_t join = nullptr;
    int* sig = nullptr;
  } pre;
  struct PotrfGraph {
    std::vector<uintptr_t> key;
    hipGraphExec_t exec = nullptr;
    uint64_t last_use = 0;
  };
  std::vector<PotrfGraph> pgraphs;
  uint64_t graph_tick = 0;
  int64_t graph_overflow = 0;
  int64_t graph_dropped = 0;
  int64_t graph_evicted = 0;
  std::string err;
  int prof = 0;
  std::vector<hipEvent_t> ev;
  size_t ev_used = 0;
  std::vector<ProfRec> recs;
  bool phase = false;
  std::vector<hipEvent_t> ph_ev;
  size_t ph_used = 0;
  std::vector<std::pair<std::string, int>> ph_marks;
  struct PhAr { double bytes; int e0, e1; };
  std::vector<PhAr> ph_ar;
  double* hsmall = nullptr;
  int* hinfo = nullptr;
  DBuf info, small;
  DBuf X, y, Xt, yt, A, Linv, W, logdiag, beta, alpha, dinv, slab, mu_loo, var_loo, Ksf, s1, s2,
      mu, var, Lout, pslab;
  int n_ell = 1;
  DBuf gu, gct, gv, Mx, gslab, gout;
  int64_t n = 0, n_pad = 0, nt = 0, nt_pad = 0;
  int d = 0;
  double ytr_mean = 0, ytr_var = 1;
  bool have_data = false, have_test = false, fitted = false;
  bool have_yt = false, f_have_yt = false;
  Theta th;
  DBuf fX, fy, fXt, fyt, Z, Kmm, Am, Lm, Lb, ldm, ldb, Knm, q, lam, ilam, ys, slabB, red, c, tvec,
      r, g, fmu_loo, fvar_loo, Ksm, qm, qb, fmu, fvar, fslab;
  DBuf fgv, fgm, fgB, fR, fgred, fgslab, fgout;
  DBuf bP, bL, bPI, bH, bvec, bGblk, bT, bkr, bEf, bF, ebuf, edraws;
  DBuf bSg, bBf, bLf, bldf, bRem, bW, bkv;
  DBuf bLR, bLRv;
  DBuf ebuf_aux[3], bPIs, bRW;
  DBuf escale;
  DBuf bfv;
  DBuf rpart;
  DBuf jK, jV, jslab, jS, jL, jLo, jW, jvec, jE, jdraws, jxi, jout;
  int64_t fn = 0, fn_pad = 0, fnt = 0, fnt_pad = 0, m = 0, m_pad = 0, fn_total = 0, fnt_total = 0;
  int fd = 0;
  double f_ytr_mean = 0, f_ytr_var = 1;
  bool f_data = false, f_test = false, f_z = false, f_fitted = false;
  bool f_pre = false;
  bool f_pre_b = false;
  hipEvent_t pre_fork = nullptr, pre_join = nullptr, preb_fork = nullptr;
  hipEvent_t kn_fork = nullptr, kn_join = nullptr;
  hipEvent_t b_fork = nullptr, b_join = nullptr;
  DBuf fslab_pre;
  Theta fth;
  ncclComm_t comm = nullptr;
  std::shared_ptr<LocalGroup> lgroup;
  int nranks = 1, rank = 0;
  DBuf t0, t1, t2, t3, t4;
  DBuf ws_main, ws_side, ws_aux[2];
};


namespace gpsapi {

struct EsArgs {
  int S = 0;
  double beta = 1.0;
  const double* draws = nullptr;
  double lam_lb = 0.0;
  double diag_ub = 0.0;
  double scale = 0.0;
};
std::vector<int64_t> fold_bounds(int64_t n, int nfold);
int es_fold(gps_ctx* ctx, hipStream_t s, DBuf& eb, bool conc, const EsArgs& es, const double* xi_src,
            int64_t b, int64_t bp, const double* PI, const double* r, double trace_c, double* w,
            double* G, int64_t ldg, double* g, double* out);

extern thread_local std::string g_err;
int fail(gps_ctx* ctx, int code, const std::string& msg);

#define HIPCHK(expr)                                                                      \
  do {                                                                                    \
    hipError_t _e = (expr);                                                               \
    if (_e != hipSuccess)                                                                 \
      return fail(ctx, -2, std::string(#expr) + " failed: " + hipGetErrorString(_e));   \
  } while (0)

#define NCCLCHK(expr)                                                                     \
  do {                                                                                    \
    ncclResult_t _r = (expr);                                                             \
    if (_r != ncclSuccess)                                                                \
      return fail(ctx, -3, std::string(#expr) + " failed: " + ncclGetErrorString(_r));  \
  } while (0)

#define ARGCHK(cond, msg)                  \
  do {                                     \
    if (!(cond)) return fail(ctx, -1, msg); \
  } while (0)

constexpr int64_t kSplitWsDoubles = 32ll << 20;
constexpr size_t kMaxGraphs = 64;

int get_event(gps_ctx* c);
struct Prof {
  gps_ctx* c;
  hipStream_t st;
  int e0 = -1;
  std::string tag;
  double flop, bytes;
  Prof(gps_ctx* c_, std::string t, double f, double b, hipStream_t s_ = nullptr)
      : c(c_), st(s_ ? s_ : c_->stream), tag(t), flop(f), bytes(b) {
    if (c->prof && (e0 = get_event(c)) >= 0) (void)hipEventRecord(c->ev[e0], st);
  }
  ~Prof() {
    if (!c->prof || e0 < 0) return;
    const int e1 = get_event(c);
    if (e1 < 0) return;
    (void)hipEventRecord(c->ev[e1], st);
    c->recs.push_back({tag, e0, e1, flop, bytes});
  }
};

hipError_t sync_ctx_streams(gps_ctx* ctx);
hipError_t drop_graphs_in(gps_ctx* ctx, const void* p, size_t bytes);
void forget_zeroed(gps_ctx* ctx, const void* p, size_t bytes);
hipError_t ensure(gps_ctx* ctx, DBuf& b, size_t bytes);
void release(gps_ctx* ctx, DBuf& b);
int get_event(gps_ctx* c);
int phase_event(gps_ctx* c, hipStream_t st);
void phase_mark(gps_ctx* c, const char* name);
hipEvent_t sync_event(gps_ctx* c);
GemmParams gp0();
const char* gemm_tag(int al, int bl, int epi, const GemmParams& p);
double gemm_flops(const GemmParams& p);
int gemm(gps_ctx* ctx, int al, int bl, int epi, const GemmParams& p, hipStream_t st = nullptr,
         GemmLaunchInfo* info = nullptr);
int gram(gps_ctx* ctx, const char* tag, const double* x, int n, const double* xp, int m, int d,
         const Theta& th, double diag_add, int lower, int pad_identity, double* out, int64_t ldo,
         int M, int N, hipStream_t st = nullptr);
int pred_rows(gps_ctx* ctx, int64_t r0, int64_t r1, const double* w, hipStream_t st);
int fitc_rowsq_cols(gps_ctx* ctx, const double* Lx, int64_t c0, int64_t c1, hipStream_t st);
int fitc_rowsq_dep(gps_ctx* ctx, const double* L, int* sig, int64_t ncols, int mode,
                   hipStream_t st, int64_t nb_dag);
int dag_list_key(const gps_ctx* ctx, int64_t nb);
bool dag_block(const gps_ctx* ctx, int64_t nb);
void dag_blocks(const gps_ctx* ctx, int64_t nb, std::vector<int>& sizes, int64_t& cnt);
int dag_width(const gps_ctx* ctx, int64_t nb, bool half);
int potrf_inv_rec(gps_ctx* ctx, double* A, int64_t lda, double* Linv, int64_t ldl, double* W,
                  int nb, double* logdiag, int* info, int base, int nreal, double* Lout,
                  int64_t ldlo, bool top = false);
size_t potrf_ws_doubles(int64_t n_pad);
int reset_info(gps_ctx* ctx);
hipError_t zero_factor(gps_ctx* ctx, double* p, int64_t n_pad, hipStream_t s);
bool factor_zeroed(const gps_ctx* ctx, const double* p, int64_t n_pad);
int potrf_inv(gps_ctx* ctx, double* A, int64_t n_pad, double* Linv, double* W, double* logdiag,
              int nreal, double* Lout);
int check_info(gps_ctx* ctx);
int set_theta(gps_ctx* ctx, Theta& th, int kind, const double* theta, int n_ell, int d);
int upload(gps_ctx* ctx, DBuf& b, const double* h, int64_t rows, int64_t cols, int64_t rows_pad);
void score_bundle(const double* sums, double nt, double out[GPS_N_SC]);
int bind(gps_ctx* ctx);
bool sharded(const gps_ctx* ctx);
std::vector<DBuf*> ctx_buffers(gps_ctx* ctx);
void leave_local_group(gps_ctx* ctx);
int group_barrier(gps_ctx* ctx, LocalGroup& G, size_t count);
int allreduce_sum(gps_ctx* ctx, double* buf, size_t count, hipStream_t s);
int allreduce_sum_impl(gps_ctx* ctx, double* buf, size_t count, hipStream_t s);

}

extern "C" {
int make_aux_streams(gps_ctx* ctx);
int factor_user(gps_ctx* ctx, int64_t n, const double* A, int64_t lda, bool want_L);
double* row_part(gps_ctx* ctx, int64_t rows, int nv);
int full_fit_core(gps_ctx* ctx, int kind, const double* theta, int n_ell);
int fitc_syrk_ks(const gps_ctx* ctx);
int fitc_syrk_rows(gps_ctx* ctx, const double* kscale, int ks, int64_t R0, int64_t R1);
int fitc_syrk(gps_ctx* ctx, const double* kscale, const double* base, double* dst,
              bool packed = false, const double* A = nullptr, int64_t lda = 0);
int fitc_syrk_allreduce(gps_ctx* ctx, double* red, int64_t blen, int64_t tail);
int fitc_test_prepass(gps_ctx* ctx);
int fitc_test_prepass_b(gps_ctx* ctx);
int fitc_fit_core(gps_ctx* ctx, const double* theta, int n_ell, double obj[GPS_N_OBJ],
                  bool pre_test = false);
int fitc_knm_xt(gps_ctx* ctx, int64_t ldc, const double* X, double* C);
int fitc_lt_vec(gps_ctx* ctx, const double* X, const double* x, double* y);
int fitc_tri_right(gps_ctx* ctx, const double* A, int64_t lda, const double* X, double* C,
                   int64_t ldc, int64_t rows);
int fitc_tri_left_t(gps_ctx* ctx, const double* X, const double* B, double* C);
}
```

scoring-rules-for-gaussian-process-regression-a-new-approach-to-inference_amd/csrc/gemm_schedule.h:

```cpp
#pragma once
#include "gps_internal.h"

#define GPS_HD __host__ __device__ __forceinline__

namespace gps {

constexpr int BK = 16;
constexpr int GROUP_M = 8;

GPS_HD int sched_min(int a, int b) { return a < b ? a : b; }

GPS_HD bool tile_of(const GemmParams& p, int t, int& ti, int& tj) {
  if (p.lower_out) {
    int r = (int)((sqrt(8.0 * (double)t + 1.0) - 1.0) * 0.5);
    while ((r + 1) * (r + 2) / 2 <= t) ++r;
    while (r * (r + 1) / 2 > t) --r;
    ti = r;
    tj = t - r * (r + 1) / 2;
    return true;
  }
  if (p.map_mode == 3) {
    const int x = t & 7, i = t >> 3;
    if (p.tri == TRI_K_LE_I || p.tri == TRI_K_GE_I) {
      const int bw = (p.tiles_n + 7) >> 3;
      const int ri = i / bw;
      tj = x * bw + i % bw;
      ti = p.tri == TRI_K_LE_I ? p.tiles_m - 1 - ri : ri;
      return tj < p.tiles_n && ri < p.tiles_m;
    }
    const int bh = (p.tiles_m + 7) >> 3;
    const int cj = i / bh;
    ti = x * bh + i % bh;
    tj = p.tri == TRI_K_LE_J ? p.tiles_n - 1 - cj : cj;
    return ti < p.tiles_m && cj < p.tiles_n;
  }
  if (p.map_mode == 5) {
    const int x = t & 7, i = t >> 3;
    const bool wi = p.tri == TRI_K_LE_I || p.tri == TRI_K_GE_I;
    const int nb = wi ? p.tiles_n : p.tiles_m, nw = wi ? p.tiles_m : p.tiles_n;
    const int bb = (nb + 7) >> 3, per = ((bb + 7) >> 3) * 64;
    const int wg = i / per, rem = i - wg * per, w = rem & 63;
    const int bi = x * bb + (rem >> 6) * 8 + (w & 7), wk = wg * 8 + (w >> 3);
    if (bi >= sched_min(nb, x * bb + bb) || wk >= nw) return false;
    const int widx = (p.tri == TRI_K_LE_I || p.tri == TRI_K_LE_J) ? nw - 1 - wk : wk;
    ti = wi ? widx : bi;
    tj = wi ? bi : widx;
    return true;
  }
  const int per_group = GROUP_M * p.tiles_n;
  const int g = t / per_group;
  const int first = g * GROUP_M;
  const int gm = sched_min(GROUP_M, p.tiles_m - first);
  const int tt = t - g * per_group;
  ti = first + tt % gm;
  tj = tt / gm;
  if (p.map_mode != 0) return true;
  if (p.tri == TRI_K_LE_I) ti = p.tiles_m - 1 - ti;
  else if (p.tri == TRI_K_LE_J) tj = p.tiles_n - 1 - tj;
  return true;
}

GPS_HD int xcd_remap(int b, int nblk) {
  const int q = nblk / 8, r = nblk % 8, x = b % 8;
  return (x < r ? x * (q + 1) : r * (q + 1) + (x - r) * q) + b / 8;
}

GPS_HD bool pair_of(const GemmParams& p, int b, int nblk, int& ri, int& q, int& qh) {
  const int np = (p.tiles_n + 1) >> 1;
  const int l = xcd_remap(b, nblk);
  const int per_group = GROUP_M * np, g = l / per_group, first = g * GROUP_M;
  const int gm = sched_min(GROUP_M, p.tiles_m - first), tt = l - g * per_group;
  ri = first + tt % gm;
  q = tt / gm;
  qh = p.tiles_n - 1 - q;
  return q < qh;
}

GPS_HD void slab_xcd_of(int bx, int by, int nt, int ny, int& t, int& slice) {
  const int l = xcd_remap(bx + by * nt, nt * ny);
  t = l % nt;
  slice = l / nt;
}

GPS_HD void tile_k_range(const GemmParams& p, int row0, int col0, int tile, int& kb, int& ke) {
  kb = 0;
  ke = p.K;
  switch (p.tri) {
    case TRI_K_LE_I: ke = sched_min(ke, p.tri_off + row0 + tile); break;
    case TRI_K_LE_J: ke = sched_min(ke, p.tri_off + col0 + tile); break;
    case TRI_K_GE_J: kb = p.tri_off + col0; break;
    case TRI_K_GE_I: kb = p.tri_off + row0; break;
    case TRI_KR_J:
      kb = p.kr[2 * (col0 / 16)];
      ke = p.kr[2 * ((col0 + tile) / 16 - 1) + 1];
      break;
    default: break;
  }
}

GPS_HD void slice_part(int nk, int parts, int s, int& s0, int& s1) {
  const int q = nk / parts, r = nk % parts;
  s0 = s * q + sched_min(s, r);
  s1 = s0 + q + (s < r ? 1 : 0);
}

template <int TE>
GPS_HD bool small_block_of(const GemmParams& p, int t, int& ti, int& tj) {
  const int tm = p.M / TE, tn = p.N / TE;
  bool valid;
  if (p.lower_out) {
    constexpr int u = 64 / TE;
    auto pre = [](int r) { const int a = r / u, b = r % u; return u * (u * a * (a + 1) / 2 + b * (a + 1)); };
    valid = t < pre(tm);
    if (valid) {
      int lo = 0, hi = tm;
      while (hi - lo > 1) { const int mid = (lo + hi) / 2; if (pre(mid) <= t) lo = mid; else hi = mid; }
      ti = lo;
      tj = t - pre(ti);
    }
  } else {
    valid = t < tm * tn;
    if (valid) { ti = t / tn; tj = t - ti * tn; }
  }
  return valid;
}

struct StreamKPart {
  int64_t I, S;
  GPS_HD int64_t bnd(int64_t q) const { return q * I / S; }
  GPS_HD int owner(int64_t x) const {
    int64_t q = x * S / I;
    while (q + 1 < S && bnd(q + 1) <= x) ++q;
    while (q > 0 && bnd(q) > x) --q;
    return (int)q;
  }
};

}
```

scoring-rules-for-gaussian-process-regression-a-new-approach-to-inference_amd/csrc/gps_internal.h:

```cpp
#pragma once

#include <hip/hip_runtime.h>
#include <stdint.h>

#include <string>
#include <vector>

#define GPS_TILE 128
#define GPS_MAX_D 64

namespace gps {

inline int64_t pad_to(int64_t n, int64_t t = GPS_TILE) { return (n + t - 1) / t * t; }

struct GramParams {
  const double* x;
  const double* xp;
  double* out;
  int64_t ldo;
  int n, m;
  int M, N;
  int d;
  double sf2;
  double diag_add;
  int lower;
  int pad_identity;
  double inv_ell[GPS_MAX_D];
  int edge;
};

enum Layout { LAY_N = 0, LAY_T = 1 };
enum Tri {
  TRI_NONE = 0,
  TRI_K_LE_I = 1,
  TRI_K_LE_J = 2,
  TRI_K_GE_J = 3,
  TRI_K_GE_I = 4,
  TRI_KR_J = 5,
};
enum Epi { EPI_STORE = 0, EPI_ROWSQ = 1, EPI_COLRED = 2, EPI_ROWSQ_DOT = 3 };

struct GemmParams {
  const double* A; int64_t lda;
  const double* B; int64_t ldb;
  double* C; int64_t ldc;
  int64_t c_kslice_stride;
  int M, N, K;
  double alpha, beta;
  const double* kscale;
  const double* w;
  double* out0; double* out1; int64_t ld_out;
  int lower_out;
  int ksplit;
  int tri;
  int tri_off;
  const int* kr;
  int tiles_m, tiles_n;
  int map_mode;
  int tile;
  double* ws;
  int64_t ws_cap;
  int* sk_cnt;
  int sk_slots;
  int sk_dp, sk_wgs;
  int prio;
  int mirror;
  int slab_xcd;
  int kend;
  int sk_alone;
  int* dep_sig; int* dep_q; int* dep_err; int dep_grid; int dep_mode;
};
constexpr int kSigStarted = 0;
constexpr int kSigRowCnt = 64;
constexpr int kSigRdy = 128;
constexpr int kSigQueue = 192;
constexpr int kSigInts = kSigQueue + 8 * 64;

struct GemmPlan { int tile, ksplit; };
GemmPlan gemm_plan(int epi, const GemmParams& p, int64_t ws_cap_doubles);
struct GemmLaunchInfo { int tile, ksplit, map_mode, sk_dp, sk_wgs, slab_xcd, grid_x, grid_y; };
extern int g_gram_reg;
extern int g_tiny_gemm;
extern int g_stream_k;
extern int g_slab_xcd;
constexpr int kStreamKTiles = 4096;

#ifdef __HIPCC__
__device__ __forceinline__ double wave_sum(double v) {
#pragma unroll
  for (int o = 32; o > 0; o >>= 1) v += __shfl_xor(v, o);
  return v;
}

template <int NV>
__device__ void block_sum(double (&v)[NV], double* sh) {
  const int lane = threadIdx.x & 63, wave = threadIdx.x >> 6, nw = blockDim.x >> 6;
#pragma unroll
  for (int q = 0; q < NV; ++q) v[q] = wave_sum(v[q]);
  __syncthreads();
  if (lane == 0)
#pragma unroll
    for (int q = 0; q < NV; ++q) sh[q * 16 + wave] = v[q];
  __syncthreads();
#pragma unroll
  for (int q = 0; q < NV; ++q) {
    double t = 0.0;
    for (int w = 0; w < nw; ++w) t += sh[q * 16 + w];
    v[q] = t;
  }
  __syncthreads();
}

__constant__ static const double g_exp_tab[64][2] = {
    {0x1.0000000000000p+0, 0x0.0p+0}, {0x1.02c9a3e778061p+0, -0x1.19083535b085dp-56},
    {0x1.059b0d3158574p+0, 0x1.d73e2a475b465p-55}, {0x1.0874518759bc8p+0, 0x1.186be4bb284ffp-57},
    {0x1.0b5586cf9890fp+0, 0x1.8a62e4adc610bp-54}, {0x1.0e3ec32d3d1a2p+0, 0x1.03a1727c57b53p-59},
    {0x1.11301d0125b51p+0, -0x1.6c51039449b3ap-54}, {0x1.1429aaea92de0p+0, -0x1.32fbf9af1369ep-54},
    {0x1.172b83c7d517bp+0, -0x1.19041b9d78a76p-55}, {0x1.1a35beb6fcb75p+0, 0x1.e5b4c7b4968e4p-55},
    {0x1.1d4873168b9aap+0, 0x1.e016e00a2643cp-54}, {0x1.2063b88628cd6p+0, 0x1.dc775814a8495p-55},
    {0x1.2387a6e756238p+0, 0x1.9b07eb6c70573p-54}, {0x1.26b4565e27cddp+0, 0x1.2bd339940e9d9p-55},
    {0x1.29e9df51fdee1p+0, 0x1.612e8afad1255p-55}, {0x1.2d285a6e4030bp+0, 0x1.0024754db41d5p-54},
    {0x1.306fe0a31b715p+0, 0x1.6f46ad23182e4p-55}, {0x1.33c08b26416ffp+0, 0x1.32721843659a6p-54},
    {0x1.371a7373aa9cbp+0, -0x1.63aeabf42eae2p-54}, {0x1.3a7db34e59ff7p+0, -0x1.5e436d661f5e3p-56},
    {0x1.3dea64c123422p+0, 0x1.ada0911f09ebcp-55}, {0x1.4160a21f72e2ap+0, -0x1.ef3691c309278p-58},
    {0x1.44e086061892dp+0, 0x1.89b7a04ef80d0p-59}, {0x1.486a2b5c13cd0p+0, 0x1.3c1a3b69062f0p-56},
    {0x1.4bfdad5362a27p+0, 0x1.d4397afec42e2p-56}, {0x1.4f9b2769d2ca7p+0, -0x1.4b309d25957e3p-54},
    {0x1.5342b569d4f82p+0, -0x1.07abe1db13cadp-55}, {0x1.56f4736b527dap+0, 0x1.9bb2c011d93adp-54},
    {0x1.5ab07dd485429p+0, 0x1.6324c054647adp-54}, {0x1.5e76f15ad2148p+0, 0x1.ba6f93080e65ep-54},
    {0x1.6247eb03a5585p+0, -0x1.383c17e40b497p-54}, {0x1.6623882552225p+0, -0x1.bb60987591c34p-54},
    {0x1.6a09e667f3bcdp+0, -0x1.bdd3413b26456p-54}, {0x1.6dfb23c651a2fp+0, -0x1.bbe3a683c88abp-57},
    {0x1.71f75e8ec5f74p+0, -0x1.16e4786887a99p-55}, {0x1.75feb564267c9p+0, -0x1.0245957316dd3p-54},
    {0x1.7a11473eb0187p+0, -0x1.41577ee04992fp-55}, {0x1.7e2f336cf4e62p+0, 0x1.05d02ba15797ep-56},
    {0x1.82589994cce13p+0, -0x1.d4c1dd41532d8p-54}, {0x1.868d99b4492edp+0, -0x1.fc6f89bd4f6bap-54},
    {0x1.8ace5422aa0dbp+0, 0x1.6e9f156864b27p-54}, {0x1.8f1ae99157736p+0, 0x1.5cc13a2e3976cp-55},
    {0x1.93737b0cdc5e5p+0, -0x1.75fc781b57ebcp-57}, {0x1.97d829fde4e50p+0, -0x1.d185b7c1b85d1p-54},
    {0x1.9c49182a3f090p+0, 0x1.c7c46b071f2bep-56}, {0x1.a0c667b5de565p+0, -0x1.359495d1cd533p-54},
    {0x1.a5503b23e255dp+0, -0x1.d2f6edb8d41e1p-54}, {0x1.a9e6b5579fdbfp+0, 0x1.0fac90ef7fd31p-54},
    {0x1.ae89f995ad3adp+0, 0x1.7a1cd345dcc81p-54}, {0x1.b33a2b84f15fbp+0, -0x1.2805e3084d708p-57},
    {0x1.b7f76f2fb5e47p+0, -0x1.5584f7e54ac3bp-56}, {0x1.bcc1e904bc1d2p+0, 0x1.23dd07a2d9e84p-55},
    {0x1.c199bdd85529cp+0, 0x1.11065895048ddp-55}, {0x1.c67f12e57d14bp+0, 0x1.2884dff483cadp-54},
    {0x1.cb720dcef9069p+0, 0x1.503cbd1e949dbp-56}, {0x1.d072d4a07897cp+0, -0x1.cbc3743797a9cp-54},
    {0x1.d5818dcfba487p+0, 0x1.2ed02d75b3707p-55}, {0x1.da9e603db3285p+0, 0x1.c2300696db532p-54},
    {0x1.dfc97337b9b5fp+0, -0x1.1a5cd4f184b5cp-54}, {0x1.e502ee78b3ff6p+0, 0x1.39e8980a9cc8fp-55},
    {0x1.ea4afa2a490dap+0, -0x1.e9c23179c2893p-54}, {0x1.efa1bee615a27p+0, 0x1.dc7f486a4b6b0p-54},
    {0x1.f50765b6e4540p+0, 0x1.9d3e12dd8a18bp-54}, {0x1.fa7c1819e90d8p+0, 0x1.74853f3a5931ep-55},
};
__device__ __forceinline__ void exp_tab_stage(double2* tab) {
  if (threadIdx.x < 64) tab[threadIdx.x] = make_double2(g_exp_tab[threadIdx.x][0], g_exp_tab[threadIdx.x][1]);
}
__device__ __forceinline__ double exp_neg(double x, const double2* tab) {
  x = x < -746.0 ? -746.0 : x;
  const double j = rint(x * 0x1.71547652b82fep+6);
  const int n = (int)j;
  const double r = fma(-j, 0x1.1cf79abc9e3b4p-42, fma(-j, 0x1.62e42fef80000p-7, x));
  const double pr = r * fma(r, fma(r, fma(r, fma(r, 1.0 / 120.0, 1.0 / 24.0), 1.0 / 6.0), 0.5), 1.0);
  const double2 t = tab[n & 63];
  return ldexp(t.x + fma(t.x, pr, t.y), n >> 6);
}

__device__ __forceinline__ double crps_term(double m, double c, double y) {
  const double s = sqrt(c);
  const double z = (y - m) / s;
  const double cdf = 0.5 * (1.0 + erf(z * 0.70710678118654752440));
  const double pdf = 0.39894228040143267794 * exp(-z * z * 0.5);
  return s * (z * (2.0 * cdf - 1.0) + 2.0 * pdf - 0.56418958354775628695);
}
__device__ __forceinline__ double logs_term(double m, double c, double y) {
  const double e = y - m;
  return e * e / (2.0 * c) + log(sqrt(c)) + 0.91893853320467274178;
}
#endif

struct GradParams {
  const double* x;
  int n, d;
  double sf2;
  double inv_ell[GPS_MAX_D];
  const double* Ainv; const double* Mx; int64_t ldm;
  const double* alpha; const double* v;
  double a0, a1, a2, a3;
  double* slab;
};

struct FitcContractParams {
  const double* xr; const double* xc;
  int nr, nc, nc_pad, d;
  double sf2;
  double inv_ell[GPS_MAX_D];
  int nt;
  const double* R[4]; int64_t ldr[4]; double coef[4]; const double* rs[4];
  double pc[2]; const double* pv[2]; const double* qv[2];
  double* slab;
  double* zslab;
  int rchunk;
};

#define GPS_SURFACE_MAX_N 128
struct SurfaceParams {
  const double* x; const double* y;
  int n, d;
  double sf2;
  const double* ell; int nl;
  const double* sd; int ns;
  int logs_add_noise;
  double* out;
};

hipError_t launch_surface(const SurfaceParams& p, hipStream_t s);
hipError_t launch_gram(const GramParams& p, hipStream_t s);
hipError_t launch_gemm(int alay, int blay, int epi, const GemmParams& p, hipStream_t s,
                       GemmLaunchInfo* info = nullptr, GemmParams* resolved = nullptr);
constexpr int kGemmItemInts = 8;
int64_t gemm_schedule(int alay, int blay, int epi, const GemmParams& p, GemmLaunchInfo& info,
                      int32_t* items, int64_t cap);

hipError_t launch_potrf_leaf(const double* A, int64_t lda, double* Linv, int64_t ldl,
                             double* Lout, int64_t ldlo, double* logdiag, int* info,
                             int base, int n_real_in_block, hipStream_t s);

struct DagParams {
  double* A; int64_t lda;
  double* Linv; int64_t ldl;
  double* Lout; int64_t ldlo;
  double* logdiag; int* info; int base; int nreal;
  int T;
  const uint32_t* tasks; int ntasks;
  int* cnt;
  unsigned long long spin_ticks;
  unsigned long long* trace = nullptr;
  int group = 3;
  int* sig = nullptr;
};
hipError_t launch_potrf_dag(const DagParams& p, int nwg, hipStream_t s);
std::vector<uint32_t> dag_task_list(int T, int order = 1, bool fine = true);
inline int64_t dag_cnt_ints(int T) { return (16 + 2 * (int64_t)T * T + 63) / 64 * 64; }

hipError_t launch_gemv_lower(const double* L, int64_t ldl, const double* x, double* y,
                             int n_pad, hipStream_t s);
hipError_t launch_gemv_full(const double* M, int64_t ldm, const double* x, double* y,
                            int rows, int cols, hipStream_t s);
hipError_t launch_colred(const double* M, int64_t ldm, int rows, int cols, int lower,
                         const double* w, const double* rowscale, double* s1, double* s2,
                         double* slab, hipStream_t s, int crows = 256);
hipError_t launch_slab_sum(const double* slab, int64_t ld, int nslab, int64_t len,
                           const double* init, double* out, hipStream_t s);
hipError_t launch_sym_slab_sum(const double* slab, int64_t slice_stride, int nslab, int M,
                               const double* base, double* dst, hipStream_t s);

hipError_t launch_sym_pack(const double* slab, int64_t slice_stride, int nslab, int r0, int r1,
                           int M, double* packed, hipStream_t s);
hipError_t launch_sym_unpack(const double* packed, int m, int M, const double* base, int full,
                             double* dst, hipStream_t s);
hipError_t launch_full_loo(const double* y, const double* slab, int nslab, int64_t ld,
                           const double* beta, const double* logdiag, int n, double* alpha,
                           double* dinv, double* mu_loo, double* var_loo, double* obj,
                           double* part, hipStream_t s);
hipError_t launch_surface_point_sums(const double* y, const double* alpha, const double* dinv,
                                     int n, double s2, int add_noise, double* sums, double* part,
                                     hipStream_t s);
int launch_colred_partials(const double* M, int64_t ldm, int rows, int cols, int lower,
                           const double* w, double* slab, hipStream_t s);
hipError_t launch_pred_finalize(const double* s1, const double* s2, int nt, double base_var,
                                double* mu, double* var, hipStream_t s);
hipError_t launch_fitc_pred_finalize(const double* qm, const double* qb, int nt, double base_var,
                                     double* var, hipStream_t s);
hipError_t launch_score_sums(const double* mu, const double* var, const double* y, int nt,
                             double ytr_mean, double ytr_var, double* sums, double* part,
                             hipStream_t s);
hipError_t launch_fitc_lambda(const double* slab, int64_t ld, int nslab, const double* y, int n,
                              int n_pad, double sf2, double sn2, double* q, double* lam,
                              double* inv_lam, double* ys, double* scal, double* part,
                              hipStream_t s);
hipError_t launch_fitc_loo(const double* y, const double* lam, const double* slab, int64_t ld,
                           int nslab, const double* g, int n, int n_pad, double* r,
                           double* mu_loo, double* var_loo, double* sums, double* part,
                           hipStream_t s);
hipError_t launch_trmv_lower(const double* L, int64_t ldl, const double* x, double* y,
                             int n_pad, int trans, hipStream_t s);
hipError_t launch_dot(const double* a, const double* b, int n, double* out, hipStream_t s);
hipError_t launch_pad_copy(const double* src, int64_t lds, double* dst, int64_t ldd, int rows,
                           int cols, int rows_pad, int cols_pad, int pad_identity, hipStream_t s);

hipError_t launch_loo_grad_terms(const double* y, const double* alpha, const double* dinv, int n,
                                 int n_pad, int obj, double* u, double* ct, hipStream_t s);
hipError_t launch_sym_mirror(double* M, int64_t ld, int n_pad, hipStream_t s);
hipError_t launch_norm_inf(const double* A, int64_t lda, int n, double* rowsum, double* out,
                           hipStream_t s);
int grad_contract_passes(int d);
int64_t grad_contract_slab_doubles(int n, int d);
hipError_t launch_grad_contract(const GradParams& p, double* out, hipStream_t s);

hipError_t launch_fold_terms(const double* y, const double* r, const double* c, int b, double* gm,
                             double* gc, double* out, hipStream_t s);
hipError_t launch_fold_grad(const double* PI, int64_t ldp, const double* H, int64_t ldh,
                            const double* r, const double* w, int b, double c0, double c1,
                            double c2, double c3, double gr, double gw, double* G, int64_t ldg,
                            double* g, hipStream_t s);
hipError_t launch_add_diag(double* P, int64_t ld, const double* vals, int nreal, int npad,
                           hipStream_t s);
hipError_t launch_row_scale(double* M, int64_t ld, int rows, int cols, const double* scale,
                            hipStream_t s);
hipError_t launch_vec_mul(const double* a, const double* b, int n, double* out, hipStream_t s);
hipError_t launch_fold_sum(const double* slab, int64_t stride, int nslab, int skip, const double* base,
                           const double* base2, double sgn, double* dst, int64_t len, hipStream_t s);
constexpr int kLocalSumMax = 64;
struct LocalSumPtrs {
  const double* p[kLocalSumMax];
};
hipError_t launch_local_sum(const LocalSumPtrs& sp, int n, int64_t count, double* out, hipStream_t s);
hipError_t launch_row_dots(const double* A, int64_t lda, const double* B, int64_t ldb,
                           const double* t, int rows, int cols, double* at, double* ab,
                           hipStream_t s);
hipError_t launch_lr_fold_vec(int mode, int b, int bp, const double* lam, const double* x,
                              const double* at, const double* ab, const double* r, const double* c,
                              const double* w, const double* gc, const double* q, double* o1,
                              double* o2, hipStream_t s);
hipError_t launch_lr_combine(const double* X, int64_t ldx, const double* Y, int64_t ldy,
                             const double* lam, const double* rs, double c0, const double* u1,
                             const double* v1, double c1, const double* u2, const double* v2,
                             double c2, int rows, int rows_pad, int cols, double* out, int64_t ldo,
                             hipStream_t s);
hipError_t launch_fold_logdet(const double* ldf, const double* ldb, int m, const double* lam, int b,
                              double* out, hipStream_t s);
hipError_t launch_blk_mdiag(const double* F, int64_t ldf, const double* US, int64_t ldus,
                            const double* U, int64_t ldu, int m_pad, const double* gd,
                            const double* lam, const double* v, const double* alpha, int n,
                            int n_pad, double* md, double* sc, double* Y, int64_t ldy,
                            hipStream_t s);
hipError_t launch_ns_init(const double* C, int64_t ldc, int b, int bp, double scale, double pad,
                          double* Y, hipStream_t s);
hipError_t launch_diag_add_const(double* M, int64_t ld, int n, double c, hipStream_t s);
hipError_t launch_sym_avg(double* M, int64_t ld, int n, hipStream_t s);
hipError_t launch_scaled_row(const double* src, int b, int bp, double scale, double* dst,
                             hipStream_t s);
hipError_t launch_row_axpy(double* C, int64_t ldc, const double* Z, int64_t ldz, const double* sv,
                           int rows, int cols, hipStream_t s);
hipError_t launch_ns_resid(const double* T, int64_t ld, int n, double* out, hipStream_t s);
hipError_t launch_es_dist(const double* Z, const double* Zh, int64_t ld, int S, int bp, double* D,
                          int64_t ldd, hipStream_t s);
hipError_t launch_es_reduce(double* D, int64_t ldd, int S, int Sp, double beta, int grad,
                            double* rs, double* cs, double* out, hipStream_t s);

struct JointCovParams {
  const double* x;
  int b, bp, d;
  double sf2, sn2;
  double inv_ell[GPS_MAX_D];
  const double* slab; int64_t stride; int ks;
  double* out;
};
hipError_t launch_joint_cov(const JointCovParams& p, hipStream_t s);
hipError_t launch_joint_resid(const double* y, const double* mu, int b, int bp, double* r,
                              hipStream_t s);
hipError_t launch_joint_dss(const double* logdiag, const double* t, int b, double* out,
                            hipStream_t s);
hipError_t launch_sign_fill(double* dst, int npos, int n, hipStream_t s);
hipError_t launch_row_add(double* M, int64_t ld, const double* mu, int rows, int cols,
                          hipStream_t s);

hipError_t launch_fitc_grad_terms(const double* y, const double* lam, const double* r,
                                  const double* g, int n, int n_pad, int obj, double n_total,
                                  double* alpha, double* dinv, double* v, double* ulam, double* h,
                                  double* hl2, hipStream_t s);
hipError_t launch_fitc_grad_v(const double* ulam, const double* z, const double* lam, int n,
                              double* v, hipStream_t s);
hipError_t launch_fitc_grad_mdiag(const double* KN, int64_t ldkn, const double* K, int64_t ldk,
                                  int m_pad, const double* lam, const double* r, const double* dinv,
                                  const double* alpha, const double* v, const double* h, double a,
                                  int n, int n_pad, double* mdiag, double* s1, double* s2,
                                  double* s3, hipStream_t s);
hipError_t launch_fitc_grad_y(const double* U, const double* UP, int64_t ld, const double* s1,
                              const double* s2, int rows, int cols, double* Y, hipStream_t s);
int fitc_contract_passes(int d);
int64_t fitc_contract_slab_doubles(int nr, int nc_pad, int d);
hipError_t launch_fitc_grad_contract(FitcContractParams p, double* out, double* zout,
                                     hipStream_t s);

}
```

scoring-rules-for-gaussian-process-regression-a-new-approach-to-inference_amd/csrc/kernels_gemm.hip:

```cpp
#include "gemm_schedule.h"
#include "gps_internal.h"

namespace gps {

typedef double d4 __attribute__((ext_vector_type(4)));
typedef double dv2 __attribute__((ext_vector_type(2)));


__device__ __forceinline__ int dep_band0(int tm, int x) { return (int)((int64_t)tm * x / 8); }
__device__ __forceinline__ int dep_ld(const int* p) {
  return __hip_atomic_load(p, __ATOMIC_RELAXED, __HIP_MEMORY_SCOPE_AGENT);
}
__device__ bool dep_take(const GemmParams& p, double* smem, int& ti, int& tj) {
  const int T = p.tiles_n, tm = p.tiles_m;
  if (p.dep_mode == 2) {
    const int b = (int)blockIdx.x;
    tj = T - 1 - b / tm;
    ti = b - (b / tm) * tm;
    if (tj < 0) return false;
    int x = 7;
    while (x > 0 && dep_band0(tm, x) > ti) --x;
    const int len = dep_band0(tm, x + 1) - dep_band0(tm, x);
    return ti - dep_band0(tm, x) >= min(p.dep_q[x * 64 + tj], len);
  }
  int* sh = reinterpret_cast<int*>(smem);
  if (threadIdx.x < 64) {
    const int lane = (int)threadIdx.x;
    unsigned int xcc;
    asm volatile("s_getreg_b32 %0, hwreg(HW_REG_XCC_ID)" : "=s"(xcc));
    const int me = (int)(xcc & 7);
    int* st = p.dep_sig + kSigRdy;
    const int xb = (me + lane) & 7;
    const int b0 = dep_band0(tm, xb), len = dep_band0(tm, xb + 1) - b0;
    int res = -1;
    unsigned long long t0 = __builtin_amdgcn_s_memrealtime();
    int seen = -1;
    unsigned int polls = 0;
    for (;;) {
      const int sv = lane < T ? dep_ld(st + lane) : 0;
      const unsigned long long ready = __ballot(sv != 0);
      unsigned long long cand = __ballot(sv == 1);
      while (cand && res < 0) {
        const int j = 63 - __builtin_clzll(cand);
        cand &= ~(1ull << j);
        int* qj = p.dep_q + xb * 64 + j;
        const int qv = lane < 8 ? dep_ld(qj) : 0;
        unsigned long long open = __ballot(lane < 8 && qv < len);
        while (open && res < 0) {
          const int l = __builtin_ctzll(open);
          open &= open - 1;
          int r = 0;
          if (lane == l) r = __hip_atomic_fetch_add(qj, 1, __ATOMIC_RELAXED, __HIP_MEMORY_SCOPE_AGENT);
          r = __shfl(r, l);
          const int lb0 = __shfl(b0, l), llen = __shfl(len, l);
          if (r < llen) res = (lb0 + r) << 8 | j;
        }
        if (res < 0 && lane == 0)
          __hip_atomic_store(st + j, 2, __ATOMIC_RELAXED, __HIP_MEMORY_SCOPE_AGENT);
      }
      const int nready = __popcll(ready);
      if (res >= 0 || nready == T) break;
      if (dep_ld(p.dep_err) != 0x7f7f7f7f) break;
      const unsigned long long now = __builtin_amdgcn_s_memrealtime();
      if (dep_ld(p.dep_sig + kSigStarted) < p.dep_grid) {
        if (now - t0 > 2000) break;
      } else {
        if (nready != seen) {
          seen = nready;
          t0 = now;
          polls = 0;
        } else if (++polls > 100000u && now - t0 > 200000000ull) {
          if (lane == 0) __hip_atomic_store(p.dep_err, 3, __ATOMIC_RELAXED, __HIP_MEMORY_SCOPE_AGENT);
          break;
        }
      }
      __builtin_amdgcn_s_sleep(2);
    }
    __builtin_amdgcn_fence(__ATOMIC_ACQUIRE, "agent");
    if (lane == 0) sh[0] = res;
  }
  __syncthreads();
  const int res = __builtin_amdgcn_readfirstlane(sh[0]);
  __syncthreads();
  if (res < 0) return false;
  ti = res >> 8;
  tj = res & 255;
  return true;
}

template <int ALAY, int BLAY, int EPI, int TILE>
__device__ __forceinline__ void gemm_tile(const GemmParams& p, int ti, int tj, int kslice,
                                          double* smem, int kb_o = -1, int ke_o = -1,
                                          double* part = nullptr);
template <int ALAY, int BLAY>
__device__ void gemm_sk_block(const GemmParams& p, int s, double* smem);

template <int ALAY, int BLAY, int EPI, int TILE>
__global__ __launch_bounds__(256) void gemm_f64_kernel(GemmParams p) {
  constexpr int LS = TILE + 16;
  constexpr int STAGE = 2 * BK * LS;
  __shared__ __attribute__((aligned(16))) double smem[2 * STAGE];
  const bool remap = p.map_mode == 2 || (p.map_mode == 0 && p.tri == TRI_NONE);
  if constexpr (EPI == EPI_STORE && TILE == 128) {
    if (p.sk_wgs > 0 && (int)blockIdx.x >= p.sk_dp) {
      gemm_sk_block<ALAY, BLAY>(p, (int)blockIdx.x - p.sk_dp, smem);
      return;
    }
  }
  if constexpr (EPI == EPI_ROWSQ) {
    if (p.dep_mode) {
      int ti, tj;
      if (dep_take(p, smem, ti, tj)) gemm_tile<ALAY, BLAY, EPI, TILE>(p, ti, tj, 0, smem);
      return;
    }
  }
  if constexpr (EPI == EPI_ROWSQ || EPI == EPI_ROWSQ_DOT) {
    if (p.map_mode == 6) {
      int ri, q, qh;
      const bool second = pair_of(p, (int)blockIdx.x, (int)gridDim.x, ri, q, qh);
      gemm_tile<ALAY, BLAY, EPI, TILE>(p, ri, qh, 0, smem);
      if (second) {
        __syncthreads();
        gemm_tile<ALAY, BLAY, EPI, TILE>(p, ri, q, 0, smem);
      }
      return;
    }
  }
  int ti, tj;
  if (p.slab_xcd) {
    int t, slice;
    slab_xcd_of((int)blockIdx.x, (int)blockIdx.y, (int)gridDim.x, (int)gridDim.y, t, slice);
    if (!tile_of(p, t, ti, tj)) return;
    gemm_tile<ALAY, BLAY, EPI, TILE>(p, ti, tj, slice, smem);
    return;
  }
  const int nblk = p.sk_wgs > 0 ? p.sk_dp : (int)gridDim.x;
  if (!tile_of(p, remap ? xcd_remap(blockIdx.x, nblk) : (int)blockIdx.x, ti, tj)) return;
  gemm_tile<ALAY, BLAY, EPI, TILE>(p, ti, tj, blockIdx.y, smem);
}

template <int TILE>
__device__ __forceinline__ void store_acc(const GemmParams& p, int ti, int tj, int kslice,
                                          const d4 (&acc)[TILE / 32][TILE / 32]) {
  constexpr int WT = TILE / 2, MI = WT / 16;
  const int tid = threadIdx.x, lane = tid & 63, wave = tid >> 6;
  const int wr = wave >> 1, wc = wave & 1;
  const int lrow = lane >> 4, lcol = lane & 15;
  const int row0 = ti * TILE, col0 = tj * TILE;
  double* Cb = p.C + (int64_t)kslice * p.c_kslice_stride;
#pragma unroll
  for (int mi = 0; mi < MI; ++mi)
#pragma unroll
    for (int r = 0; r < 4; ++r) {
      const int row = row0 + wr * WT + mi * 16 + lrow + 4 * r;
      double* crow = Cb + (int64_t)row * p.ldc + col0 + wc * WT + lcol;
#pragma unroll
      for (int ni = 0; ni < MI; ++ni) {
        double v = p.alpha * acc[mi][ni][r];
        if (p.beta != 0.0) v = fma(p.beta, crow[ni * 16], v);
        crow[ni * 16] = v;
      }
    }
}

template <int ALAY, int BLAY>
__device__ void gemm_sk_block(const GemmParams& p, int s, double* smem) {
  constexpr int TILE = 128, MI = TILE / 32, TT = TILE * TILE;
  const int tiles = p.lower_out ? p.tiles_m * (p.tiles_m + 1) / 2 : p.tiles_m * p.tiles_n;
  const int nk = p.K / BK;
  const StreamKPart part{(int64_t)(tiles - p.sk_dp) * nk, (int64_t)p.sk_wgs};
  const int tid = threadIdx.x;
  int64_t it = part.bnd(s);
  const int64_t it1 = part.bnd(s + 1);
  while (it < it1) {
    const int u = (int)(it / nk);
    const int k0 = (int)(it - (int64_t)u * nk);
    const int k1 = (int)min<int64_t>(nk, k0 + (it1 - it));
    int ti, tj;
    tile_of(p, p.sk_dp + u, ti, tj);
    const int s0 = part.owner((int64_t)u * nk), s1 = part.owner((int64_t)u * nk + nk - 1);
    if (s0 == s1) {
      gemm_tile<ALAY, BLAY, EPI_STORE, TILE>(p, ti, tj, 0, smem);
      __syncthreads();
    } else {
      gemm_tile<ALAY, BLAY, EPI_STORE, TILE>(p, ti, tj, 0, smem, k0 * BK, k1 * BK,
                                             p.ws + (int64_t)(u + s) * TT);
      asm volatile("s_waitcnt vmcnt(0)" ::: "memory");
      __syncthreads();
      unsigned int* flag = reinterpret_cast<unsigned int*>(smem);
      if (tid == 0) {
        __builtin_amdgcn_fence(__ATOMIC_RELEASE, "agent");
        asm volatile("s_waitcnt vmcnt(0)" ::: "memory");
        const int t = __hip_atomic_fetch_add(p.sk_cnt + u, 1, __ATOMIC_RELAXED, __HIP_MEMORY_SCOPE_AGENT);
        const unsigned int last = t == s1 - s0 ? 1u : 0u;
        if (last) {
          __hip_atomic_store(p.sk_cnt + u, 0, __ATOMIC_RELAXED, __HIP_MEMORY_SCOPE_AGENT);
          __builtin_amdgcn_fence(__ATOMIC_ACQUIRE, "agent");
          asm volatile("s_waitcnt vmcnt(0)" ::: "memory");
        }
        flag[0] = last;
      }
      __syncthreads();
      const unsigned int last = __builtin_amdgcn_readfirstlane(flag[0]);
      __syncthreads();
      if (last) {
        d4 acc[MI][MI];
#pragma unroll
        for (int mi = 0; mi < MI; ++mi)
#pragma unroll
          for (int ni = 0; ni < MI; ++ni) acc[mi][ni] = (d4){0.0, 0.0, 0.0, 0.0};
        for (int q = s0; q <= s1; ++q) {
          const double* src = p.ws + (int64_t)(u + q) * TT + tid;
#pragma unroll
          for (int mi = 0; mi < MI; ++mi)
#pragma unroll
            for (int ni = 0; ni < MI; ++ni)
#pragma unroll
              for (int r = 0; r < 4; ++r) acc[mi][ni][r] += src[((mi * MI + ni) * 4 + r) * 256];
        }
        store_acc<TILE>(p, ti, tj, 0, acc);
      }
    }
    it += k1 - k0;
  }
}

template <int ALAY, int BLAY, int EPI, int TILE>
__device__ __forceinline__ void gemm_tile(const GemmParams& p, int ti, int tj, int kslice,
                                          double* smem, int kb_o, int ke_o, double* part) {
  constexpr int LS = TILE + 16;
  constexpr int STAGE = 2 * BK * LS;
  constexpr int WT = TILE / 2;
  constexpr int MI = WT / 16;
  constexpr int PER = TILE * BK / 256;
  constexpr int NQ = PER / 2;
  constexpr int TPR = TILE / PER;
  constexpr int TPI = BK / PER;
  constexpr bool SK = TILE == 64 || (ALAY == LAY_N && BLAY == LAY_T);
  auto rowoff = [](int k) { return k * LS + (SK ? 4 * (k >> 2) : 0); };
  const int tid = threadIdx.x, lane = tid & 63, wave = tid >> 6;
  const int wr = wave >> 1, wc = wave & 1;
  const int row0 = ti * TILE, col0 = tj * TILE;

  int kb, ke;
  tile_k_range(p, row0, col0, TILE, kb, ke);
  if (p.kend > 0 && ke > p.kend) ke = p.kend;
  if (kb_o >= 0) {
    kb = kb_o;
    ke = ke_o;
  } else if (p.ksplit > 1) {
    int s0, s1;
    slice_part(ke > kb ? (ke - kb) / BK : 0, p.ksplit, kslice, s0, s1);
    ke = kb + s1 * BK;
    kb = kb + s0 * BK;
  }
  const int nk = ke > kb ? (ke - kb) / BK : 0;

  dv2 ra[NQ], rb[NQ];
  auto load_tile = [&](int k0) {
    if constexpr (ALAY == LAY_T) {
      const int k = tid / TPR, i = (tid % TPR) * 2;
      const dv2* src = reinterpret_cast<const dv2*>(p.A + (int64_t)(k0 + k) * p.lda + row0 + i);
#pragma unroll
      for (int q = 0; q < NQ; ++q) ra[q] = src[q * TPR];
      if (p.kscale) {
        const double sc = p.kscale[k0 + k];
#pragma unroll
        for (int q = 0; q < NQ; ++q) { ra[q].x *= sc; ra[q].y *= sc; }
      }
    } else {
      const int i = tid / TPI, k = (tid % TPI) * PER;
      const dv2* src = reinterpret_cast<const dv2*>(p.A + (int64_t)(row0 + i) * p.lda + k0 + k);
#pragma unroll
      for (int q = 0; q < NQ; ++q) ra[q] = src[q];
      if (p.kscale) {
#pragma unroll
        for (int q = 0; q < NQ; ++q) {
          ra[q].x *= p.kscale[k0 + k + 2 * q];
          ra[q].y *= p.kscale[k0 + k + 2 * q + 1];
        }
      }
    }
    if constexpr (BLAY == LAY_N) {
      const int k = tid / TPR, j = (tid % TPR) * 2;
      const dv2* src = reinterpret_cast<const dv2*>(p.B + (int64_t)(k0 + k) * p.ldb + col0 + j);
#pragma unroll
      for (int q = 0; q < NQ; ++q) rb[q] = src[q * TPR];
    } else {
      const int j = tid / TPI, k = (tid % TPI) * PER;
      const dv2* src = reinterpret_cast<const dv2*>(p.B + (int64_t)(col0 + j) * p.ldb + k0 + k);
#pragma unroll
      for (int q = 0; q < NQ; ++q) rb[q] = src[q];
    }
  };
  auto store_tile = [&](int buf) {
    double* As = smem + buf * STAGE;
    double* Bs = As + BK * LS;
    if constexpr (ALAY == LAY_T) {
      const int k = tid / TPR, i = (tid % TPR) * 2;
#pragma unroll
      for (int q = 0; q < NQ; ++q) *reinterpret_cast<dv2*>(&As[rowoff(k) + i + 2 * TPR * q]) = ra[q];
    } else {
      const int i = tid / TPI, k = (tid % TPI) * PER;
#pragma unroll
      for (int q = 0; q < NQ; ++q) {
        As[rowoff(k + 2 * q) + i] = ra[q].x;
        As[rowoff(k + 2 * q + 1) + i] = ra[q].y;
      }
    }
    if constexpr (BLAY == LAY_N) {
      const int k = tid / TPR, j = (tid % TPR) * 2;
#pragma unroll
      for (int q = 0; q < NQ; ++q) *reinterpret_cast<dv2*>(&Bs[rowoff(k) + j + 2 * TPR * q]) = rb[q];
    } else {
      const int j = tid / TPI, k = (tid % TPI) * PER;
#pragma unroll
      for (int q = 0; q < NQ; ++q) {
        Bs[rowoff(k + 2 * q) + j] = rb[q].x;
        Bs[rowoff(k + 2 * q + 1) + j] = rb[q].y;
      }
    }
  };

  d4 acc[MI][MI];
#pragma unroll
  for (int mi = 0; mi < MI; ++mi)
#pragma unroll
    for (int ni = 0; ni < MI; ++ni) acc[mi][ni] = (d4){0.0, 0.0, 0.0, 0.0};

  auto compute = [&](int buf) {
    const double* As = smem + buf * STAGE;
    const double* Bs = As + BK * LS;
#pragma unroll
    for (int kk = 0; kk < BK / 4; ++kk) {
      const int krow = rowoff(kk * 4 + (lane >> 4)) + (lane & 15);
      double a[MI], b[MI];
#pragma unroll
      for (int mi = 0; mi < MI; ++mi) a[mi] = As[krow + wr * WT + mi * 16];
#pragma unroll
      for (int ni = 0; ni < MI; ++ni) b[ni] = Bs[krow + wc * WT + ni * 16];
#pragma unroll
      for (int mi = 0; mi < MI; ++mi)
#pragma unroll
        for (int ni = 0; ni < MI; ++ni)
          acc[mi][ni] = __builtin_amdgcn_mfma_f64_16x16x4f64(a[mi], b[ni], acc[mi][ni], 0, 0, 0);
    }
  };

  const bool rdot = EPI == EPI_ROWSQ_DOT && tj == p.tiles_n - 1 && kb == 0;
  double dacc = 0.0;
  auto row_dot = [&](int buf, int k0) {
    if constexpr (EPI == EPI_ROWSQ_DOT) {
      if (rdot && tid < TILE) {
        const double* As = smem + buf * STAGE;
#pragma unroll
        for (int k = 0; k < BK; ++k) dacc = fma(As[rowoff(k) + tid], p.w[k0 + k], dacc);
      }
    }
  };

  if (nk > 0) {
    load_tile(kb);
    store_tile(0);
    __syncthreads();
    for (int it = 0; it < nk - 1; ++it) {
      load_tile(kb + (it + 1) * BK);
      if (p.prio) __builtin_amdgcn_s_setprio(1);
      compute(it & 1);
      if (p.prio) __builtin_amdgcn_s_setprio(0);
      row_dot(it & 1, kb + it * BK);
      store_tile((it + 1) & 1);
      __syncthreads();
    }
    compute((nk - 1) & 1);
    row_dot((nk - 1) & 1, kb + (nk - 1) * BK);
  }
  if constexpr (EPI == EPI_ROWSQ_DOT) {
    if (rdot && tid < TILE) p.out1[row0 + tid] = dacc;
  }

  const int lrow = lane >> 4, lcol = lane & 15;
  if constexpr (EPI == EPI_STORE) {
    if (part) {
#pragma unroll
      for (int mi = 0; mi < MI; ++mi)
#pragma unroll
        for (int ni = 0; ni < MI; ++ni)
#pragma unroll
          for (int r = 0; r < 4; ++r) part[((mi * MI + ni) * 4 + r) * 256 + tid] = acc[mi][ni][r];
      return;
    }
    store_acc<TILE>(p, ti, tj, kslice, acc);
  } else if constexpr (EPI == EPI_ROWSQ || EPI == EPI_ROWSQ_DOT) {
    double* red = smem;
    __syncthreads();
#pragma unroll
    for (int mi = 0; mi < MI; ++mi)
#pragma unroll
      for (int r = 0; r < 4; ++r) {
        double s = 0.0;
#pragma unroll
        for (int ni = 0; ni < MI; ++ni) s = fma(acc[mi][ni][r], acc[mi][ni][r], s);
        s += __shfl_xor(s, 1);
        s += __shfl_xor(s, 2);
        s += __shfl_xor(s, 4);
        s += __shfl_xor(s, 8);
        if (lcol == 0) red[wc * TILE + wr * WT + mi * 16 + lrow + 4 * r] = s;
      }
    __syncthreads();
    if (tid < TILE)
      p.out0[(int64_t)tj * p.ld_out + row0 + tid] = p.alpha * p.alpha * (red[tid] + red[TILE + tid]);
  } else {
    double* red = smem;
    __syncthreads();
    double wv[MI][4];
#pragma unroll
    for (int mi = 0; mi < MI; ++mi)
#pragma unroll
      for (int r = 0; r < 4; ++r) wv[mi][r] = p.w[row0 + wr * WT + mi * 16 + lrow + 4 * r];
#pragma unroll
    for (int ni = 0; ni < MI; ++ni) {
      double s1 = 0.0, s2 = 0.0;
#pragma unroll
      for (int mi = 0; mi < MI; ++mi)
#pragma unroll
        for (int r = 0; r < 4; ++r) {
          s1 = fma(acc[mi][ni][r], wv[mi][r], s1);
          s2 = fma(acc[mi][ni][r], acc[mi][ni][r], s2);
        }
      s1 += __shfl_xor(s1, 16);
      s1 += __shfl_xor(s1, 32);
      s2 += __shfl_xor(s2, 16);
      s2 += __shfl_xor(s2, 32);
      if (lrow == 0) {
        red[wr * 2 * TILE + wc * WT + ni * 16 + lcol] = s1;
        red[wr * 2 * TILE + TILE + wc * WT + ni * 16 + lcol] = s2;
      }
    }
    __syncthreads();
    if (tid < TILE) {
      p.out0[(int64_t)ti * p.ld_out + col0 + tid] = p.alpha * (red[tid] + red[2 * TILE + tid]);
      p.out1[(int64_t)ti * p.ld_out + col0 + tid] =
          p.alpha * p.alpha * (red[TILE + tid] + red[3 * TILE + tid]);
    }
  }
}

template <int ALAY, int BLAY, int R, int WPT>
__global__ __launch_bounds__(256) void gemm_f64_small_kernel(GemmParams p) {
  constexpr int TE = 16 * R;
  constexpr int TPB = 4 / WPT;
  constexpr int G = R == 1 ? 4 : 2;
  constexpr int NACC = R * R * 4;
  __shared__ double red[WPT > 1 ? 4 * NACC * 64 : 1];
  const int lane = threadIdx.x & 63, wave = threadIdx.x >> 6;
  const int slot = wave / WPT, part = wave - slot * WPT;
  const int t = blockIdx.x * TPB + slot;
  int ti = 0, tj = 0;
  const bool valid = small_block_of<TE>(p, t, ti, tj);
  if (WPT == 1 && !valid) return;
  const int row0 = ti * TE, col0 = tj * TE;
  int kb, ke;
  tile_k_range(p, row0, col0, TE, kb, ke);
  const int nk = valid && ke > kb ? (ke - kb) / 16 : 0;
  int c0, c1;
  slice_part(nk, WPT, part, c0, c1);
  const int r = lane & 15, g = lane >> 4;

  typedef double Frag[G][R][4];
  auto load_chunk = [&](int c, double (&a)[R][4], double (&b)[R][4]) {
    const int k = kb + 16 * c + 4 * g;
#pragma unroll
    for (int i = 0; i < R; ++i) {
      const int row = row0 + 16 * i + r;
      if constexpr (ALAY == LAY_N) {
        const dv2* s = reinterpret_cast<const dv2*>(p.A + (int64_t)row * p.lda + k);
        const dv2 u0 = s[0], u1 = s[1];
        a[i][0] = u0.x; a[i][1] = u0.y; a[i][2] = u1.x; a[i][3] = u1.y;
      } else {
#pragma unroll
        for (int e = 0; e < 4; ++e) a[i][e] = p.A[(int64_t)(k + e) * p.lda + row];
      }
      const int col = col0 + 16 * i + r;
      if constexpr (BLAY == LAY_T) {
        const dv2* s = reinterpret_cast<const dv2*>(p.B + (int64_t)col * p.ldb + k);
        const dv2 u0 = s[0], u1 = s[1];
        b[i][0] = u0.x; b[i][1] = u0.y; b[i][2] = u1.x; b[i][3] = u1.y;
      } else {
#pragma unroll
        for (int e = 0; e < 4; ++e) b[i][e] = p.B[(int64_t)(k + e) * p.ldb + col];
      }
    }
  };
  d4 acc[R][R];
#pragma unroll
  for (int i = 0; i < R; ++i)
#pragma unroll
    for (int j = 0; j < R; ++j) acc[i][j] = (d4){0.0, 0.0, 0.0, 0.0};
  auto load_group = [&](int c, Frag& a, Frag& b) {
#pragma unroll
    for (int j = 0; j < G; ++j)
      if (c + j < c1) load_chunk(c + j, a[j], b[j]);
  };
  auto mma_group = [&](int c, const Frag& a, const Frag& b) {
#pragma unroll
    for (int j = 0; j < G; ++j)
      if (c + j < c1) {
#pragma unroll
        for (int kk = 0; kk < 4; ++kk)
#pragma unroll
          for (int i = 0; i < R; ++i)
#pragma unroll
            for (int jj = 0; jj < R; ++jj)
              acc[i][jj] = __builtin_amdgcn_mfma_f64_16x16x4f64(a[j][i][kk], b[j][jj][kk], acc[i][jj], 0, 0, 0);
      }
  };
  Frag fa0, fb0, fa1, fb1;
  int c = c0;
  if (c < c1) load_group(c, fa0, fb0);
  while (c < c1) {
    if (c + G < c1) load_group(c + G, fa1, fb1);
    mma_group(c, fa0, fb0);
    c += G;
    if (c >= c1) break;
    if (c + G < c1) load_group(c + G, fa0, fb0);
    mma_group(c, fa1, fb1);
    c += G;
  }
  if constexpr (WPT > 1) {
    double* mine = red + (int64_t)wave * NACC * 64 + lane;
    if (part > 0) {
#pragma unroll
      for (int i = 0; i < R; ++i)
#pragma unroll
        for (int j = 0; j < R; ++j)
#pragma unroll
          for (int e = 0; e < 4; ++e) mine[((i * R + j) * 4 + e) * 64] = acc[i][j][e];
    }
    __syncthreads();
    if (part > 0 || !valid) return;
#pragma unroll
    for (int w = 1; w < WPT; ++w) {
      const double* o = mine + w * NACC * 64;
#pragma unroll
      for (int i = 0; i < R; ++i)
#pragma unroll
        for (int j = 0; j < R; ++j)
#pragma unroll
          for (int e = 0; e < 4; ++e) acc[i][j][e] += o[((i * R + j) * 4 + e) * 64];
    }
  }
#pragma unroll
  for (int i = 0; i < R; ++i)
#pragma unroll
    for (int e = 0; e < 4; ++e) {
      double* crow = p.C + (int64_t)(row0 + 16 * i + g + 4 * e) * p.ldc + col0 + r;
#pragma unroll
      for (int j = 0; j < R; ++j) {
        double v = p.alpha * acc[i][j][e];
        if (p.beta != 0.0) v = fma(p.beta, crow[16 * j], v);
        crow[16 * j] = v;
      }
    }
}

static int64_t small_tiles(const GemmParams& p, int te) {
  const int64_t tm = p.M / te, tn = p.N / te;
  if (!p.lower_out) return tm * tn;
  const int64_t u = 64 / te, a = tm / u;
  return u * u * a * (a + 1) / 2;
}

__global__ __launch_bounds__(256) void splitk_reduce_kernel(const double* __restrict__ ws, int ks,
                                                            int M, int N, int lower_tile,
                                                            double alpha, double beta,
                                                            double* __restrict__ C, int64_t ldc) {
  const int64_t e = 2 * ((int64_t)blockIdx.x * 256 + threadIdx.x);
  if (e >= (int64_t)M * N) return;
  const int i = (int)(e / N), j = (int)(e - (int64_t)i * N);
  if (lower_tile && j / lower_tile > i / lower_tile) return;
  const int64_t slab = (int64_t)M * N;
  dv2 s = *reinterpret_cast<const dv2*>(ws + e);
  for (int q = 1; q < ks; ++q) s += *reinterpret_cast<const dv2*>(ws + q * slab + e);
  dv2* c = reinterpret_cast<dv2*>(C + (int64_t)i * ldc + j);
  dv2 v = alpha * s;
  if (beta != 0.0) v += beta * *c;
  *c = v;
}

__global__ __launch_bounds__(256) void splitk_reduce_sym_kernel(const double* __restrict__ ws, int ks,
                                                                int N, double alpha, double beta,
                                                                double* __restrict__ C, int64_t ldc) {
  __shared__ double t[32][33];
  const int b = blockIdx.x;
  int r = (int)((sqrt(8.0 * (double)b + 1.0) - 1.0) * 0.5);
  while ((r + 1) * (r + 2) / 2 <= b) ++r;
  while (r * (r + 1) / 2 > b) --r;
  const int c = b - r * (r + 1) / 2;
  const int tx = threadIdx.x & 31, ty = threadIdx.x >> 5;
  const int64_t slab = (int64_t)N * N;
#pragma unroll
  for (int k = 0; k < 4; ++k) {
    const int i = r * 32 + ty + 8 * k, j = c * 32 + tx;
    const int64_t e = (int64_t)i * N + j;
    double sum = ws[e];
    for (int q = 1; q < ks; ++q) sum += ws[q * slab + e];
    double v = alpha * sum;
    double* cp = C + (int64_t)i * ldc + j;
    if (beta != 0.0) v += beta * *cp;
    *cp = v;
    t[ty + 8 * k][tx] = v;
  }
  if (r == c) return;
  __syncthreads();
#pragma unroll
  for (int k = 0; k < 4; ++k) C[(int64_t)(c * 32 + ty + 8 * k) * ldc + r * 32 + tx] = t[tx][ty + 8 * k];
}

int g_tiny_gemm = 1;
int g_slab_xcd = 1;
int g_stream_k = 2;

static int small_wpt(int K) { return K >= 64 ? 4 : (K >= 32 ? 2 : 1); }

static int64_t tiles_for(const GemmParams& p, int tile) {
  const int64_t tm = p.M / tile, tn = p.N / tile;
  return p.lower_out ? tm * (tm + 1) / 2 : tm * tn;
}

GemmPlan gemm_plan(int epi, const GemmParams& p, int64_t ws_cap) {
  if (p.tile) return {p.tile, p.ksplit > 1 ? p.ksplit : 1};
  if (epi != EPI_STORE || p.ksplit > 1) return {128, p.ksplit > 1 ? p.ksplit : 1};
  if (g_tiny_gemm && !p.kscale && p.K <= 1280) {
    const int64_t mn = (int64_t)p.M * p.N;
    if ((mn <= 256 * 256 && p.K <= 1024) || (p.lower_out && p.M <= 384 && p.K <= 640))
      return {16, small_wpt(p.K)};
    if (p.lower_out ? (p.M <= 640 && p.K <= 640) : (mn <= 1280 * 1280 && (p.tri || p.K <= 640)))
      return {32, small_wpt(p.K)};
  }
  if (tiles_for(p, 128) >= 512) return {128, 1};
  const int64_t t64 = tiles_for(p, 64);
  const int64_t target = p.lower_out ? 2048 : 1024;
  int ks = 1;
  while (ks < 8 && t64 * ks < target && p.K / (2 * ks) >= 64 &&
         (int64_t)(2 * ks) * p.M * p.N <= ws_cap)
    ks *= 2;
  return {64, ks};
}

hipError_t launch_gemm(int alay, int blay, int epi, const GemmParams& pin, hipStream_t s,
                       GemmLaunchInfo* info, GemmParams* resolved) {
  GemmParams p = pin;
  if (p.M % GPS_TILE || p.N % GPS_TILE || p.K % BK || p.M <= 0 || p.N <= 0)
    return hipErrorInvalidValue;
  if ((p.lda & 1) || (p.ldb & 1) || (p.ldc & 1)) return hipErrorInvalidValue;
  if (p.lower_out && p.M != p.N) return hipErrorInvalidValue;
  if (p.mirror && (!p.lower_out || p.M % 32)) return hipErrorInvalidValue;
  if (p.ksplit < 1) p.ksplit = 1;
  if (epi == EPI_ROWSQ_DOT &&
      (!p.w || !p.out1 || p.tri != TRI_K_LE_J || p.tri_off < 0 || p.K != p.tri_off + p.N ||
       p.ksplit != 1))
    return hipErrorInvalidValue;
  const GemmPlan plan = gemm_plan(epi, p, p.ws ? p.ws_cap : 0);
  const int tile = plan.tile;
  if (tile == 16 || tile == 32) {
    if (epi != EPI_STORE || p.kscale) return hipErrorInvalidValue;
    const int wpt = plan.ksplit;
    if (wpt != 1 && wpt != 2 && wpt != 4) return hipErrorInvalidValue;
    const int64_t tt = small_tiles(p, tile);
    const dim3 grid((unsigned)((tt * wpt + 3) / 4)), block(256);
    if (info) *info = {tile, wpt, p.map_mode, 0, 0, 0, (int)grid.x, 1};
    if (resolved) {
      *resolved = p;
      return hipSuccess;
    }
    hipError_t err = hipErrorInvalidValue;
#define GPS_SMALL_CASE(AL, BL, RR, W)                                                           \
    if (err == hipErrorInvalidValue && alay == AL && blay == BL && tile == 16 * RR && wpt == W) { \
      hipLaunchKernelGGL((gemm_f64_small_kernel<AL, BL, RR, W>), grid, block, 0, s, p);           \
      err = hipGetLastError();                                                                    \
    }
#define GPS_SMALL_LAYOUTS(RR, W)                                                                \
    GPS_SMALL_CASE(LAY_N, LAY_T, RR, W) GPS_SMALL_CASE(LAY_N, LAY_N, RR, W)                     \
    GPS_SMALL_CASE(LAY_T, LAY_N, RR, W) GPS_SMALL_CASE(LAY_T, LAY_T, RR, W)
    GPS_SMALL_LAYOUTS(1, 1) GPS_SMALL_LAYOUTS(1, 2) GPS_SMALL_LAYOUTS(1, 4)
    GPS_SMALL_LAYOUTS(2, 1) GPS_SMALL_LAYOUTS(2, 2) GPS_SMALL_LAYOUTS(2, 4)
#undef GPS_SMALL_LAYOUTS
#undef GPS_SMALL_CASE
    if (err == hipSuccess && p.mirror) err = launch_sym_mirror(p.C, p.ldc, p.M, s);
    return err;
  }
  if (tile != 64 && tile != 128) return hipErrorInvalidValue;
  if (tile == 64 && epi != EPI_STORE) return hipErrorInvalidValue;
  p.ksplit = plan.ksplit;
  const bool slabbed = p.ksplit > 1 && p.ws != nullptr;
  if (p.ksplit > 1 && !slabbed && (epi != EPI_STORE || p.beta != 0.0)) return hipErrorInvalidValue;
  if (p.ksplit > 1 && !slabbed && p.mirror) return hipErrorInvalidValue;
  GemmParams q = p;
  if (slabbed) {
    if (epi != EPI_STORE) return hipErrorInvalidValue;
    q.C = p.ws;
    q.ldc = p.N;
    q.c_kslice_stride = (int64_t)p.M * p.N;
    q.alpha = 1.0;
    q.beta = 0.0;
  }
  q.tiles_m = q.M / tile;
  q.tiles_n = q.N / tile;
  int tiles = (int)tiles_for(q, tile);
  const bool rowsq = epi == EPI_ROWSQ || epi == EPI_ROWSQ_DOT;
  if (q.dep_mode) {
    if (epi != EPI_ROWSQ || alay != LAY_N || blay != LAY_T || q.tri != TRI_K_LE_J || q.tri_off != 0 ||
        tile != 128 || q.ksplit != 1 || q.tiles_n > 64 || !q.dep_sig || !q.dep_q || !q.dep_err ||
        q.dep_mode > 2 || q.K != q.N)
      return hipErrorInvalidValue;
    q.map_mode = 0;
    q.prio = 0;
    q.slab_xcd = 0;
    q.sk_dp = q.sk_wgs = 0;
    if (resolved) return hipErrorInvalidValue;
    const dim3 grid((unsigned)(q.tiles_m * q.tiles_n)), block(256);
    hipLaunchKernelGGL((gemm_f64_kernel<LAY_N, LAY_T, EPI_ROWSQ, 128>), grid, block, 0, s, q);
    return hipGetLastError();
  }
  const bool pairable = rowsq && q.tri == TRI_K_LE_J && tile == 128 && q.ksplit == 1;
  if (q.map_mode == 6 && !pairable) q.map_mode = 0;
  const bool paired = pairable;
  if (q.map_mode == 0 && q.tri != TRI_NONE && q.tri != TRI_KR_J && !q.lower_out)
    q.map_mode = rowsq ? (paired ? 6 : 5) : 3;
  else if (q.map_mode == 4) q.map_mode = 0;
  if (q.map_mode == 6) tiles = q.tiles_m * ((q.tiles_n + 1) / 2);
  if (q.map_mode == 5 && (q.lower_out || q.tri == TRI_NONE || q.tri == TRI_KR_J)) q.map_mode = 0;
  if (q.map_mode == 5) {
    const bool wi = q.tri == TRI_K_LE_I || q.tri == TRI_K_GE_I;
    const int nb = wi ? q.tiles_n : q.tiles_m, nw = wi ? q.tiles_m : q.tiles_n;
    tiles = 8 * ((nw + 7) / 8) * (((nb + 7) / 8 + 7) / 8) * 64;
  }
  if (q.map_mode == 3) {
    if (q.lower_out || q.tri == TRI_NONE || q.tri == TRI_KR_J) return hipErrorInvalidValue;
    tiles = (q.tri == TRI_K_LE_I || q.tri == TRI_K_GE_I) ? 8 * ((q.tiles_n + 7) / 8) * q.tiles_m
                                                          : 8 * ((q.tiles_m + 7) / 8) * q.tiles_n;
  }
  q.sk_dp = q.sk_wgs = 0;
  if ((g_stream_k == 1 || (g_stream_k == 2 && q.sk_alone)) && epi == EPI_STORE && tile == 128 &&
      q.ksplit == 1 && q.sk_cnt && q.ws &&
      q.sk_slots > 0 && q.tri == TRI_NONE && (q.lower_out || q.map_mode == 0 || q.map_mode == 2)) {
    const int slots = q.sk_slots, rem = tiles % slots;
    if (tiles >= slots && rem > 0 && 4 * rem <= 3 * slots && rem <= kStreamKTiles &&
        (int64_t)(rem + slots) * 128 * 128 <= q.ws_cap && q.K / BK >= 2) {
      q.sk_dp = tiles - rem;
      const int64_t runs = (int64_t)rem * (q.K / BK);
      q.sk_wgs = runs < slots ? (int)runs : slots;
      tiles = q.sk_dp + q.sk_wgs;
    }
  }
  q.prio = (epi == EPI_STORE || epi == EPI_COLRED) && !q.kscale;
  q.slab_xcd = g_slab_xcd && q.ksplit > 1 && q.sk_wgs == 0 &&
               (q.map_mode == 0 || q.map_mode == 2) && (q.lower_out || q.tri == TRI_NONE);
  dim3 grid(tiles, q.ksplit), block(256);
  if (info) *info = {tile, q.ksplit, q.map_mode, q.sk_dp, q.sk_wgs, q.slab_xcd, tiles, q.ksplit};
  if (resolved) {
    *resolved = q;
    return hipSuccess;
  }
  hipError_t err = hipErrorInvalidValue;
#define GPS_GEMM_CASE(AL, BL, EP, T)                                                        \
  if (err == hipErrorInvalidValue && alay == AL && blay == BL && epi == EP && tile == T) { \
    hipLaunchKernelGGL((gemm_f64_kernel<AL, BL, EP, T>), grid, block, 0, s, q);            \
    err = hipGetLastError();                                                                \
  }
  GPS_GEMM_CASE(LAY_N, LAY_T, EPI_STORE, 128)
  GPS_GEMM_CASE(LAY_N, LAY_N, EPI_STORE, 128)
  GPS_GEMM_CASE(LAY_T, LAY_N, EPI_STORE, 128)
  GPS_GEMM_CASE(LAY_T, LAY_T, EPI_STORE, 128)
  GPS_GEMM_CASE(LAY_N, LAY_T, EPI_ROWSQ, 128)
  GPS_GEMM_CASE(LAY_N, LAY_T, EPI_ROWSQ_DOT, 128)
  GPS_GEMM_CASE(LAY_N, LAY_T, EPI_COLRED, 128)
  GPS_GEMM_CASE(LAY_N, LAY_T, EPI_STORE, 64)
  GPS_GEMM_CASE(LAY_N, LAY_N, EPI_STORE, 64)
  GPS_GEMM_CASE(LAY_T, LAY_N, EPI_STORE, 64)
  GPS_GEMM_CASE(LAY_T, LAY_T, EPI_STORE, 64)
#undef GPS_GEMM_CASE
  if (err != hipSuccess) return err;
  if (!slabbed) return p.mirror ? launch_sym_mirror(p.C, p.ldc, p.M, s) : hipSuccess;
  if (p.mirror) {
    const int64_t t32 = p.M / 32;
    hipLaunchKernelGGL(splitk_reduce_sym_kernel, dim3((unsigned)(t32 * (t32 + 1) / 2)), dim3(256), 0,
                       s, p.ws, p.ksplit, p.N, p.alpha, p.beta, p.C, p.ldc);
    return hipGetLastError();
  }
  const int64_t pairs = (int64_t)p.M * p.N / 2;
  hipLaunchKernelGGL(splitk_reduce_kernel, dim3((unsigned)((pairs + 255) / 256)), dim3(256), 0, s,
                     p.ws, p.ksplit, p.M, p.N, p.lower_out ? tile : 0, p.alpha, p.beta, p.C, p.ldc);
  return hipGetLastError();
}

int64_t gemm_schedule(int alay, int blay, int epi, const GemmParams& p, GemmLaunchInfo& info,
                      int32_t* items, int64_t cap) {
  GemmParams q;
  if (launch_gemm(alay, blay, epi, p, nullptr, &info, &q) != hipSuccess) return -1;
  int64_t n = 0;
  auto emit = [&](int wg, int ti, int tj, int kb, int ke, int slice, int slot, int tickets) {
    if (n < cap) {
      int32_t* o = items + n * kGemmItemInts;
      o[0] = wg; o[1] = ti; o[2] = tj; o[3] = kb; o[4] = ke > kb ? ke : kb; o[5] = slice; o[6] = slot;
      o[7] = tickets;
    }
    ++n;
  };
  const int tile = info.tile;
  if (tile == 16 || tile == 32) {
    const int wpt = info.ksplit, tpb = 4 / wpt;
    for (int b = 0; b < info.grid_x; ++b)
      for (int wave = 0; wave < 4; ++wave) {
        const int slot = wave / wpt, part = wave - slot * wpt;
        int ti = 0, tj = 0;
        const bool valid = tile == 16 ? small_block_of<16>(q, b * tpb + slot, ti, tj)
                                      : small_block_of<32>(q, b * tpb + slot, ti, tj);
        if (!valid) continue;
        int kb, ke, c0, c1;
        tile_k_range(q, ti * tile, tj * tile, tile, kb, ke);
        slice_part(ke > kb ? (ke - kb) / 16 : 0, wpt, part, c0, c1);
        emit(b, ti, tj, kb + 16 * c0, kb + 16 * c1, part, -1, 0);
      }
    return n;
  }
  auto tile_item = [&](int wg, int ti, int tj, int kslice) {
    int kb, ke;
    tile_k_range(q, ti * tile, tj * tile, tile, kb, ke);
    if (q.kend > 0 && ke > q.kend) ke = q.kend;
    if (q.ksplit > 1) {
      int s0, s1;
      slice_part(ke > kb ? (ke - kb) / BK : 0, q.ksplit, kslice, s0, s1);
      ke = kb + s1 * BK;
      kb = kb + s0 * BK;
    }
    emit(wg, ti, tj, kb, ke, kslice, -1, 0);
  };
  const bool rowsq = epi == EPI_ROWSQ || epi == EPI_ROWSQ_DOT;
  const bool remap = q.map_mode == 2 || (q.map_mode == 0 && q.tri == TRI_NONE);
  for (int by = 0; by < info.grid_y; ++by)
    for (int bx = 0; bx < info.grid_x; ++bx) {
      const int wg = bx + by * info.grid_x;
      int ti, tj;
      if (epi == EPI_STORE && tile == 128 && q.sk_wgs > 0 && bx >= q.sk_dp) {
        const int s = bx - q.sk_dp;
        const int tiles = q.lower_out ? q.tiles_m * (q.tiles_m + 1) / 2 : q.tiles_m * q.tiles_n;
        const int nk = q.K / BK;
        const StreamKPart part{(int64_t)(tiles - q.sk_dp) * nk, (int64_t)q.sk_wgs};
        int64_t it = part.bnd(s);
        const int64_t it1 = part.bnd(s + 1);
        while (it < it1) {
          const int u = (int)(it / nk);
          const int k0 = (int)(it - (int64_t)u * nk);
          const int k1 = (int)(nk < k0 + (it1 - it) ? nk : k0 + (it1 - it));
          tile_of(q, q.sk_dp + u, ti, tj);
          const int s0 = part.owner((int64_t)u * nk), s1 = part.owner((int64_t)u * nk + nk - 1);
          if (s0 == s1) tile_item(wg, ti, tj, 0);
          else emit(wg, ti, tj, k0 * BK, k1 * BK, 0, u + s, s1 - s0);
          it += k1 - k0;
        }
        continue;
      }
      if (rowsq && q.map_mode == 6) {
        int ri, c, ch;
        const bool second = pair_of(q, bx, info.grid_x, ri, c, ch);
        tile_item(wg, ri, ch, 0);
        if (second) tile_item(wg, ri, c, 0);
        continue;
      }
      if (q.slab_xcd) {
        int t, slice;
        slab_xcd_of(bx, by, info.grid_x, info.grid_y, t, slice);
        if (tile_of(q, t, ti, tj)) tile_item(wg, ti, tj, slice);
        continue;
      }
      const int nblk = q.sk_wgs > 0 ? q.sk_dp : info.grid_x;
      if (tile_of(q, remap ? xcd_remap(bx, nblk) : bx, ti, tj)) tile_item(wg, ti, tj, by);
    }
  return n;
}

}
```

scoring-rules-for-gaussian-process-regression-a-new-approach-to-inference_amd/gpscore/_lib.py:

```python
from __future__ import annotations

import ctypes
import os

import numpy as np

_HERE = os.path.dirname(os.path.abspath(__file__))
LIB_PATH = os.environ.get("GPSCORE_LIB", os.path.join(_HERE, "libgpscore.so"))
ABI_VERSION = 800
GPS_N_STATS = 6
GPS_COMM_NONE, GPS_COMM_RCCL, GPS_COMM_LOCAL = 0, 1, 2
COMM_KINDS = {GPS_COMM_NONE: "none", GPS_COMM_RCCL: "rccl", GPS_COMM_LOCAL: "local"}

GPS_ARD, GPS_RBF = 0, 1
GPS_FULL, GPS_LOWER = 0, 1
GPS_OPT_OVERLAP, GPS_OPT_GEMM_MAP, GPS_OPT_TINY_GEMM, GPS_OPT_GRAM_REG = 0, 3, 7, 9
GPS_OPT_GRAPH = 10
GPS_OPT_PRED_PRE = 11
GPS_OPT_DAG = 12
GPS_OPT_DAG_TILES = 13
GPS_OPT_DAG_GROUP = 17
GPS_OPT_STREAM_K = 18
GPS_OPT_DAG_WGS = 19
GPS_OPT_DAG_ORDER = 25
GPS_OPT_SLAB_XCD = 26
GPS_OPT_FITC_DEP = 27
GPS_OPT_AR_CHUNKS = 15
OBJ_NAMES = ("nlml", "loo_crps", "loo_logs", "logdet", "quad")
SURFACE_NAMES = ("loo_crps", "insample_crps", "nlml", "loo_logs")
GPS_SURF_LOGS_ADD_NOISE = 1
SCORE_NAMES = ("test_crps", "test_logs", "test_msll", "test_smse", "test_mse", "test_cover")

_c_int, _c_i64, _c_dbl, _c_vp, _c_cp = (ctypes.c_int, ctypes.c_int64, ctypes.c_double,
                                        ctypes.c_void_p, ctypes.c_char_p)
_P = ctypes.POINTER(ctypes.c_double)

_PI = ctypes.POINTER(ctypes.c_int32)


class GemmDesc(ctypes.Structure):
    _fields_ = [("lay_a", ctypes.c_int32), ("lay_b", ctypes.c_int32), ("epi", ctypes.c_int32),
                ("M", ctypes.c_int32), ("N", ctypes.c_int32), ("K", ctypes.c_int32),
                ("lda", _c_i64), ("ldb", _c_i64), ("ldc", _c_i64),
                ("alpha", _c_dbl), ("beta", _c_dbl),
                ("tri", ctypes.c_int32), ("tri_off", ctypes.c_int32),
                ("lower_out", ctypes.c_int32), ("mirror", ctypes.c_int32),
                ("kend", ctypes.c_int32),
                ("tile", ctypes.c_int32), ("ksplit", ctypes.c_int32), ("map_mode", ctypes.c_int32),
                ("use_ws", ctypes.c_int32), ("sk_alone", ctypes.c_int32),
                ("dep_mode", ctypes.c_int32), ("reserved", ctypes.c_int32),
                ("ld_out", _c_i64), ("c_kslice_stride", _c_i64)]


GEMM_PLAN_NAMES = ("tile", "ksplit", "map_mode", "sk_dp", "sk_wgs", "slab_xcd", "grid_x", "grid_y")

SIGNATURES = {
    "gps_version": (_c_int, []),
    "gps_build_id": (_c_int, [_c_cp, _c_int]),
    "gps_ctx_create": (_c_int, [_c_int, ctypes.POINTER(_c_vp)]),
    "gps_ctx_destroy": (_c_int, [_c_vp]),
    "gps_last_error": (_c_cp, [_c_vp]),
    "gps_ctx_set_stream": (_c_int, [_c_vp, _c_vp]),
    "gps_ctx_stream": (_c_vp, [_c_vp]),
    "gps_ctx_synchronize": (_c_int, [_c_vp]),
    "gps_ctx_set_option": (_c_int, [_c_vp, _c_int, _c_int]),
    "gps_ctx_stats": (_c_int, [_c_vp, _c_vp, _c_int]),
    "gps_dag_task_list": (_c_int, [_c_int, _c_int, _c_vp, _c_int]),
    "gps_gemm_diag_check": (_c_int, [ctypes.POINTER(GemmDesc), _c_int, _c_int, _c_int, _PI, _c_int,
                                     _c_int]),
    "gps_gemm_schedule": (_c_i64, [ctypes.POINTER(GemmDesc), _PI, _c_int, _c_int, _PI, _PI, _c_i64]),
    "gps_gemm_diag": (_c_int, [_c_vp, ctypes.POINTER(GemmDesc), _P, _P, _P, _P, _P, _PI, _P, _P,
                               _PI]),
    "gps_prof_enable": (_c_int, [_c_vp, _c_int]),
    "gps_prof_collect": (_c_int, [_c_vp, _c_cp, _c_i64]),
    "gps_phase_enable": (_c_int, [_c_vp, _c_int]),
    "gps_phase_collect": (_c_int, [_c_vp, _c_cp, _c_i64]),
    "gps_rccl_info": (_c_int, [ctypes.POINTER(_c_int), _c_cp, _c_int]),
    "gps_gram": (_c_int, [_c_vp, _c_int, _P, _c_i64, _P, _c_i64, _c_int, _c_dbl, _P, _c_int,
                          _c_dbl, _c_int, _P]),
    "gps_potrf": (_c_int, [_c_vp, _c_i64, _P, _c_i64, _P]),
    "gps_potrs": (_c_int, [_c_vp, _c_i64, _c_i64, _P, _c_i64, _P, _c_i64, _P, _c_i64]),
    "gps_diag_inv": (_c_int, [_c_vp, _c_i64, _P, _c_i64, _P]),
    "gps_gemm": (_c_int, [_c_vp, _c_int, _c_int, _c_i64, _c_i64, _c_i64, _c_dbl, _P, _c_i64, _P,
                          _c_i64, _c_dbl, _P, _c_i64]),
    "gps_scores": (_c_int, [_c_vp, _P, _P, _P, _c_i64, _c_dbl, _c_dbl, _P]),
    "gps_full_set_data": (_c_int, [_c_vp, _P, _P, _c_i64, _c_int]),
    "gps_full_set_test": (_c_int, [_c_vp, _P, _P, _c_i64]),
    "gps_full_fit": (_c_int, [_c_vp, _c_int, _P, _c_int, _P, _P, _P]),
    "gps_full_grad": (_c_int, [_c_vp, _c_int, _P, _c_int, _c_int, _P, _P]),
    "gps_full_predict": (_c_int, [_c_vp, _P, _P, _P]),
    "gps_fitc_set_data": (_c_int, [_c_vp, _P, _P, _c_i64, _c_int, _c_dbl, _c_dbl, _c_i64]),
    "gps_fitc_set_test": (_c_int, [_c_vp, _P, _P, _c_i64, _c_i64]),
    "gps_fitc_set_inducing": (_c_int, [_c_vp, _P, _c_i64]),
    "gps_fitc_fit": (_c_int, [_c_vp, _P, _c_int, _P, _P, _P]),
    "gps_fitc_grad": (_c_int, [_c_vp, _P, _c_int, _c_int, _P, _P, _P]),
    "gps_full_blockloo": (_c_int, [_c_vp, _c_int, _P, _c_int, _c_int, _c_int, _P, _P, _P]),
    "gps_full_blockloo_es": (_c_int, [_c_vp, _c_int, _P, _c_int, _c_int, _c_int, _c_dbl, _P, _P,
                                      _P, _P]),
    "gps_fitc_blockloo": (_c_int, [_c_vp, _P, _c_int, _c_int, _c_int, _P, _P, _P, _P]),
    "gps_energy_score": (_c_int, [_c_vp, _P, _P, _c_i64, _P, _c_int, _c_dbl, _P, _P]),
    "gps_fitc_predict": (_c_int, [_c_vp, _P, _P, _P]),
    "gps_fitc_intermediates": (_c_int, [_c_vp, _P, _P, _P, _P, _P]),
    "gps_full_predict_cov": (_c_int, [_c_vp, _c_i64, _c_i64, _P, _P, _c_i64]),
    "gps_fitc_predict_cov": (_c_int, [_c_vp, _c_i64, _c_i64, _P, _P, _c_i64]),
    "gps_full_predict_joint": (_c_int, [_c_vp, _c_int, _c_int, _c_int, _c_dbl, _P, _P, _P]),
    "gps_fitc_predict_joint": (_c_int, [_c_vp, _c_int, _c_int, _c_int, _c_dbl, _P, _P, _P]),
    "gps_full_predict_draws": (_c_int, [_c_vp, _c_i64, _c_i64, _c_int, _P, _P]),
    "gps_fitc_predict_draws": (_c_int, [_c_vp, _c_i64, _c_i64, _c_int, _P, _P]),
    "gps_full_surface": (_c_int, [_c_vp, _P, _P, _c_i64, _c_int, _c_dbl, _P, _c_i64, _P, _c_i64,
                                  _c_int, _P]),
    "gps_comm_unique_id": (_c_int, [_c_cp]),
    "gps_comm_init": (_c_int, [_c_vp, _c_int, _c_int, _c_cp]),
    "gps_comm_init_local": (_c_int, [_c_vp, _c_int, _c_int, ctypes.c_longlong]),
    "gps_comm_info": (_c_int, [_c_vp, ctypes.POINTER(_c_int), ctypes.POINTER(_c_int),
                               ctypes.POINTER(_c_int)]),
    "gps_comm_destroy": (_c_int, [_c_vp]),
}

_lib = None


def gemm_schedule(desc, kr=None, have_kscale=False, slots=512):
    lib = load()
    plan = np.zeros(len(GEMM_PLAN_NAMES), np.int32)
    krp = None if kr is None else kr.ctypes.data_as(_PI)
    pp = plan.ctypes.data_as(_PI)
    n = lib.gps_gemm_schedule(ctypes.byref(desc), krp, int(have_kscale), slots, pp, None, 0)
    if n < 0:
        raise GpsError(lib.gps_last_error(None).decode())
    items = np.zeros((n, 8), np.int32)
    lib.gps_gemm_schedule(ctypes.byref(desc), krp, int(have_kscale), slots, pp,
                          items.ctypes.data_as(_PI), n)
    return dict(zip(GEMM_PLAN_NAMES, (int(v) for v in plan))), items


class GpsError(RuntimeError):
    """A HIP / RCCL / argument error reported by libgpscore (status < 0)."""


class NotPositiveDefinite(GpsError):

    def __init__(self, info, msg):
        super().__init__(msg)
        self.info = info


def load():
    global _lib
    if _lib is not None:
        return _lib
    if not os.path.exists(LIB_PATH):
        raise ImportError(
            f"libgpscore.so not found at {LIB_PATH}: build it with "
            "`python -c 'import __graft_entry__ as g; g.build()'` (or make -C <pkg>/csrc)")
    lib = ctypes.CDLL(LIB_PATH)
    lib.gps_version.restype = _c_int
    lib.gps_version.argtypes = []
    if lib.gps_version() != ABI_VERSION:
        raise ImportError(f"{LIB_PATH} has ABI version {lib.gps_version()}, this binding "
                          f"expects {ABI_VERSION}: rebuild the library")
    for name, (res, args) in SIGNATURES.items():
        fn = getattr(lib, name)
        fn.restype = res
        fn.argtypes = args
    _lib = lib
    return lib


def rccl_info():
    lib = load()
    v = _c_int()
    buf = ctypes.create_string_buffer(4096)
    rc = lib.gps_rccl_info(ctypes.byref(v), buf, len(buf))
    if rc != 0:
        raise GpsError(f"gps_rccl_info failed ({rc})")
    return v.value, buf.value.decode()


def build_id():
    lib = load()
    buf = ctypes.create_string_buffer(80)
    lib.gps_build_id(buf, len(buf))
    return buf.value.decode()


def check_build_id():
    from . import buildid
    want = buildid.source_hash()
    got = build_id()
    if want is not None and got != want:
        raise ImportError(f"{LIB_PATH} was built from other sources (build id {got[:16]}, the "
                          f"checked-out csrc/ hashes to {want[:16]}): rebuild it with "
                          "`make -C <pkg>/csrc`")
    return got


def ptr(a):
    if a is None:
        return None
    return a.ctypes.data_as(_P)


def f64(a, ndim=None):
    a = np.ascontiguousarray(np.asarray(a, dtype=np.float64))
    if ndim == 2 and a.ndim == 1:
        a = a.reshape(-1, 1)
    return a


class Context:

    def __init__(self, device=0):
        self.lib = load()
        h = _c_vp()
        rc = self.lib.gps_ctx_create(int(device), ctypes.byref(h))
        if rc != 0:
            raise GpsError(f"gps_ctx_create(device={device}) failed: "
                           f"{self.lib.gps_last_error(None).decode()}")
        self.h = h
        self.device = device
        self.resident = {}

    def check(self, rc, what):
        if rc == 0:
            return
        msg = self.lib.gps_last_error(self.h).decode()
        if rc > 0:
            raise NotPositiveDefinite(rc, f"{what}: {msg}")
        raise GpsError(f"{what} failed ({rc}): {msg}")

    def call(self, name, *args):
        self.check(getattr(self.lib, name)(self.h, *args), name)

    def close(self):
        if getattr(self, "h", None):
            self.lib.gps_ctx_destroy(self.h)
            self.h = None

    def __del__(self):
        try:
            self.close()
        except Exception:
            pass

    def prof(self, on=True):
        self.call("gps_prof_enable", 1 if on else 0)

    def prof_collect(self):
        import json
        buf = ctypes.create_string_buffer(1 << 16)
        self.call("gps_prof_collect", buf, len(buf))
        return json.loads(buf.value.decode())

    def phases(self, on=True):
        self.call("gps_phase_enable", 1 if on else 0)

    def phase_collect(self):
        import json
        buf = ctypes.create_string_buffer(1 << 20)
        self.call("gps_phase_collect", buf, len(buf))
        return json.loads(buf.value.decode())

    def set_overlap(self, on=True):
        self.call("gps_ctx_set_option", GPS_OPT_OVERLAP, 1 if on else 0)

    def set_tiny_gemm(self, on=True):
        self.call("gps_ctx_set_option", GPS_OPT_TINY_GEMM, 1 if on else 0)

    def set_gram_reg(self, on=True):
        v = on if isinstance(on, int) and not isinstance(on, bool) else (2 if on else 0)
        self.call("gps_ctx_set_option", GPS_OPT_GRAM_REG, v)

    def set_graphs(self, on=True):
        self.call("gps_ctx_set_option", GPS_OPT_GRAPH, 1 if on else 0)

    def set_ar_chunks(self, chunks):
        self.call("gps_ctx_set_option", GPS_OPT_AR_CHUNKS, int(chunks))

    def set_dag(self, on=True, tiles=None):
        self.call("gps_ctx_set_option", GPS_OPT_DAG, 1 if on else 0)
        if tiles is not None:
            self.call("gps_ctx_set_option", GPS_OPT_DAG_TILES, int(tiles))

    def set_pred_pre(self, on=True):
        self.call("gps_ctx_set_option", GPS_OPT_PRED_PRE, 1 if on else 0)

    def synchronize(self):
        self.call("gps_ctx_synchronize")

    def stats(self):
        out = np.zeros(GPS_N_STATS, np.int64)
        rc = self.lib.gps_ctx_stats(self.h, out.ctypes.data_as(ctypes.c_void_p), GPS_N_STATS)
        self.check(0 if rc >= 0 else rc, "gps_ctx_stats")
        return dict(zip(("graphs", "graph_cap", "graph_overflow", "device_bytes", "graph_dropped",
                         "graph_evicted"), (int(v) for v in out)))

    def gemm_diag(self, desc, A, B, C=None, kscale=None, w=None, kr=None, out0=None, out1=None):
        plan = np.zeros(len(GEMM_PLAN_NAMES), np.int32)
        krp = None if kr is None else kr.ctypes.data_as(_PI)
        self.check(self.lib.gps_gemm_diag(self.h, ctypes.byref(desc), ptr(A), ptr(B), ptr(C),
                                          ptr(kscale), ptr(w), krp, ptr(out0), ptr(out1),
                                          plan.ctypes.data_as(_PI)), "gps_gemm_diag")
        return dict(zip(GEMM_PLAN_NAMES, (int(v) for v in plan)))

    def comm_info(self):
        n, r, k = _c_int(), _c_int(), _c_int()
        self.call("gps_comm_info", ctypes.byref(n), ctypes.byref(r), ctypes.byref(k))
        return n.value, r.value, COMM_KINDS.get(k.value, str(k.value))

    def set_stream(self, stream_handle):
        self.call("gps_ctx_set_stream", _c_vp(stream_handle))


_default_ctx = None


def default_context():
    global _default_ctx
    if _default_ctx is None:
        dev = int(os.environ.get("GPSCORE_DEVICE", os.environ.get("LOCAL_RANK", "0")))
        _default_ctx = Context(dev)
    return _default_ctx
```

Before: 8.086 fit+predict+score units/s (C3 full GP, whole job).

## Precompute load-balanced tile lists for triangular GEMMs in recursive Cholesky-inverse

Adds a persistent list-driven GEMM kernel for triangular-K GEMMs in the recursive potrf/inverse. Tile-to-workgroup assignments are built on the host by cost-based bin packing, or by greedy dealing when there are many tiles, cached per shape on the device, and prepared before graph capture. The aim is to remove the load imbalance caused by uneven per-tile K ranges in triangular products. In exchange it adds host-side table construction, a synchronous upload per new shape, and the loss of the stream-K/remap paths for those launches.

```diff
diff --git a/include/gpscore.h b/include/gpscore.h
--- a/include/gpscore.h
+++ b/include/gpscore.h
@@ -25,7 +25,7 @@
   GPS_SC_MSE = 4, GPS_SC_COVER = 5, GPS_N_SC = 6
 };
 
-#define GPS_ABI_VERSION 800
+#define GPS_ABI_VERSION 810
 int gps_version(void);
 int gps_build_id(char* out, int cap);
 int gps_ctx_create(int device, gps_ctx** out);
@@ -51,7 +51,9 @@
   GPS_OPT_SLAB_XCD = 26,
   GPS_OPT_DAG_ORDER = 25,
   GPS_OPT_FITC_DEP = 27,
+  GPS_OPT_TILE_LISTS = 28,
 };
+#define GPS_TILE_LIST_C0 2
 int gps_ctx_set_option(gps_ctx* ctx, int key, int value);
 
 enum { GPS_STAT_GRAPHS = 0, GPS_STAT_GRAPH_CAP = 1, GPS_STAT_GRAPH_OVERFLOW = 2,
@@ -71,7 +73,7 @@
   int32_t kend;
   int32_t tile, ksplit, map_mode;
   int32_t use_ws, sk_alone, dep_mode;
-  int32_t reserved;
+  int32_t lists;
   int64_t ld_out, c_kslice_stride;
 } gps_gemm_desc;
 enum { GPS_GEMM_PLAN_TILE = 0, GPS_GEMM_PLAN_KSPLIT = 1, GPS_GEMM_PLAN_MAP = 2,
diff --git a/scoring-rules-for-gaussian-process-regression-a-new-approach-to-inference_amd/csrc/api.hip b/scoring-rules-for-gaussian-process-regression-a-new-approach-to-inference_amd/csrc/api.hip
--- a/scoring-rules-for-gaussian-process-regression-a-new-approach-to-inference_amd/csrc/api.hip
+++ b/scoring-rules-for-gaussian-process-regression-a-new-approach-to-inference_amd/csrc/api.hip
@@ -146,10 +146,33 @@
   return 2.0 * M * N * K;
 }
 
-int gemm(gps_ctx* ctx, int al, int bl, int epi, const GemmParams& p, hipStream_t st,
-         GemmLaunchInfo* info) {
-  if (!st) st = ctx->stream;
-  GemmParams q = p;
+static int tile_list_for(gps_ctx* ctx, const GemmParams& r, int tile, const int** tab) {
+  const std::vector<int> key = {r.tiles_m, r.tiles_n, r.tri, r.tri_off, r.K, r.kend, tile,
+                                r.list_grid, r.lists};
+  auto it = ctx->list_tabs.find(key);
+  if (it == ctx->list_tabs.end()) {
+    hipStreamCaptureStatus cs = hipStreamCaptureStatusNone;
+    HIPCHK(hipStreamIsCapturing(ctx->stream, &cs));
+    if (cs != hipStreamCaptureStatusNone)
+      return fail(ctx, -2, "tile lists: the launch's table was not prepared before the capture");
+    const std::vector<int32_t> t = tile_lists_build(r, tile, r.list_grid);
+    DBuf b;
+    HIPCHK(ensure(ctx, b, t.size() * 4));
+    hipError_t e = hipMemcpyAsync(b.p, t.data(), t.size() * 4, hipMemcpyHostToDevice, ctx->stream);
+    if (e == hipSuccess) e = hipStreamSynchronize(ctx->stream);
+    if (e != hipSuccess) {
+      release(ctx, b);
+      HIPCHK(e);
+    }
+    it = ctx->list_tabs.emplace(key, b).first;
+  }
+  *tab = static_cast<const int*>(it->second.p);
+  return 0;
+}
+
+static int gemm_resolve(gps_ctx* ctx, int al, int bl, int epi, const GemmParams& p, hipStream_t st,
+                        GemmParams& q) {
+  q = p;
   if (q.map_mode == 0) q.map_mode = ctx->gemm_map;
   if (epi == EPI_STORE && (q.ksplit == 1 || q.tile == 64) && !q.ws) {
     DBuf& ws = st == ctx->side      ? ctx->ws_side
@@ -164,12 +187,29 @@
       q.sk_slots = 2 * ctx->ncu;
     }
   }
+  if (q.lists < 0) q.lists = ctx->tile_lists ? 1 + GPS_TILE_LIST_C0 : 0;
+  if (q.lists > 0) {
+    GemmLaunchInfo li{};
+    GemmParams r = q;
+    const bool list_mode = launch_gemm(al, bl, epi, q, nullptr, &li, &r) == hipSuccess && r.list_grid > 0;
+    if (!list_mode || (p.lists < 0 && li.tile != kListProdTile)) q.lists = 0;
+    else if (int rc = tile_list_for(ctx, r, li.tile, &q.list_tab)) return rc;
+  }
+  return 0;
+}
+
+int gemm(gps_ctx* ctx, int al, int bl, int epi, const GemmParams& p, hipStream_t st,
+         GemmLaunchInfo* info) {
+  if (!st) st = ctx->stream;
+  GemmParams q;
+  if (int rc = gemm_resolve(ctx, al, bl, epi, p, st, q)) return rc;
   std::string tag = gemm_tag(al, bl, epi, p);
   if (ctx->prof > 1) {
     const GemmPlan plan = gemm_plan(epi, q, q.ws ? q.ws_cap : 0);
     char buf[160];
-    snprintf(buf, sizeof(buf), " %c%c %dx%dx%d tri%d t%d ks%d ld%lld", al ? 'T' : 'N',
-             bl ? 'T' : 'N', p.M, p.N, p.K, (int)p.tri, plan.tile, plan.ksplit, (long long)p.lda);
+    snprintf(buf, sizeof(buf), " %c%c %dx%dx%d tri%d t%d ks%d ld%lld%s", al ? 'T' : 'N',
+             bl ? 'T' : 'N', p.M, p.N, p.K, (int)p.tri, plan.tile, plan.ksplit, (long long)p.lda,
+             q.list_tab ? " lists" : "");
     tag += buf;
   }
   Prof pr(ctx, tag, gemm_flops(p), 0, st);
@@ -257,6 +297,31 @@
 int dag_width(const gps_ctx* ctx, int64_t nb, bool half) {
   const int auto_w = half ? std::max(4, ctx->ncu / 2) : ctx->ncu;
   return (int)std::min<int64_t>(ctx->dag_wgs > 0 ? ctx->dag_wgs : auto_w, std::max<int64_t>(4, 2 * nb * nb));
+}
+
+static GemmParams rec_shape(int which, int n1, int n2) {
+  GemmParams p = gp0();
+  p.M = n2; p.N = n1; p.K = which == 2 ? n2 : n1;
+  p.tri = which == 0 ? TRI_K_LE_J : which == 1 ? TRI_K_GE_J : TRI_K_LE_I;
+  if (which == 2) p.alpha = -1.0;
+  p.lists = -1;
+  return p;
+}
+static const int kRecLay[3][2] = {{LAY_N, LAY_T}, {LAY_N, LAY_N}, {LAY_N, LAY_N}};
+
+static int potrf_list_prep(gps_ctx* ctx, int nb) {
+  if (nb <= 1 || dag_block(ctx, nb)) return 0;
+  const int n1b = nb / 2, n2b = nb - n1b;
+  for (int which = 0; which < 3; ++which) {
+    GemmParams p = rec_shape(which, n1b * GPS_TILE, n2b * GPS_TILE);
+    p.lda = p.ldb = p.ldc = 2;
+    hipStream_t st = which == 1 && ctx->overlap ? ctx->side : ctx->stream;
+    GemmParams q;
+    if (int rc = gemm_resolve(ctx, kRecLay[which][0], kRecLay[which][1], EPI_STORE, p, st, q)) return rc;
+    if (q.list_tab) ctx->list_ptrs.push_back((uintptr_t)q.list_tab);
+  }
+  if (int rc = potrf_list_prep(ctx, n1b)) return rc;
+  return potrf_list_prep(ctx, n2b);
 }
 
 int potrf_inv_rec(gps_ctx* ctx, double* A, int64_t lda, double* Linv, int64_t ldl, double* W,
@@ -320,10 +385,9 @@
     return rc;
   }
   {
-    GemmParams p = gp0();
+    GemmParams p = rec_shape(0, n1, n2);
     p.A = A21; p.lda = lda; p.B = Linv; p.ldb = ldl; p.C = W; p.ldc = n1;
-    p.M = n2; p.N = n1; p.K = n1; p.tri = TRI_K_LE_J;
-    if ((rc = gemm(ctx, LAY_N, LAY_T, EPI_STORE, p))) return rc;
+    if ((rc = gemm(ctx, kRecLay[0][0], kRecLay[0][1], EPI_STORE, p))) return rc;
   }
   if (Lout) HIPCHK(hipMemcpy2DAsync(Lout + (int64_t)n1 * ldlo, ldlo * 8, W, (size_t)n1 * 8,
                                     (size_t)n1 * 8, n2, hipMemcpyDeviceToDevice, s));
@@ -343,10 +407,9 @@
     if ((rc = gemm(ctx, LAY_N, LAY_T, EPI_STORE, p))) return rc;
   }
   {
-    GemmParams p = gp0();
+    GemmParams p = rec_shape(1, n1, n2);
     p.A = W; p.lda = n1; p.B = Linv; p.ldb = ldl; p.C = A21; p.ldc = lda;
-    p.M = n2; p.N = n1; p.K = n1; p.tri = TRI_K_GE_J;
-    if ((rc = gemm(ctx, LAY_N, LAY_N, EPI_STORE, p, ts))) return rc;
+    if ((rc = gemm(ctx, kRecLay[1][0], kRecLay[1][1], EPI_STORE, p, ts))) return rc;
   }
   if (forked) HIPCHK(hipEventRecord(join, ts));
   if (pre_here) {
@@ -369,10 +432,9 @@
     return rc;
   if (forked) HIPCHK(hipStreamWaitEvent(s, join, 0));
   {
-    GemmParams p = gp0();
+    GemmParams p = rec_shape(2, n1, n2);
     p.A = Li22; p.lda = ldl; p.B = A21; p.ldb = lda; p.C = Li21; p.ldc = ldl;
-    p.M = n2; p.N = n1; p.K = n2; p.alpha = -1.0; p.tri = TRI_K_LE_I;
-    if ((rc = gemm(ctx, LAY_N, LAY_N, EPI_STORE, p))) return rc;
+    if ((rc = gemm(ctx, kRecLay[2][0], kRecLay[2][1], EPI_STORE, p))) return rc;
   }
   if (top && ctx->pre.join) {
     HIPCHK(hipStreamWaitEvent(s, ctx->pre.join, 0));
@@ -430,6 +492,9 @@
     HIPCHK(hipMemsetAsync(ctx->dag_cnt.p, 0, ctx->dag_cnt.cap, ctx->stream));
     HIPCHK(hipStreamSynchronize(ctx->stream));
   }
+  ctx->list_ptrs.clear();
+  if (ctx->tile_lists)
+    if (int rc = potrf_list_prep(ctx, (int)(n_pad / GPS_TILE))) return rc;
   auto eager = [&]() {
     ctx->sync_used = 0;
     ctx->pre.join = nullptr;
@@ -451,7 +516,9 @@
       pre ? (uintptr_t)ctx->Knm.p : 0, pre ? (uintptr_t)ctx->fslab.p : 0,
       pre ? (uintptr_t)ctx->fn_pad : 0, pre ? (uintptr_t)ctx->m_pad : 0, pre ? (uintptr_t)ctx->pre.sig : 0,
       (uintptr_t)ctx->dag, (uintptr_t)ctx->dag_tiles, (uintptr_t)ctx->dag_group, (uintptr_t)ctx->dag_wgs, (uintptr_t)ctx->dag_half,
-      (uintptr_t)ctx->dag_cnt.p, (uintptr_t)ctx->sk_cnt.p, (uintptr_t)ctx->dag_sig};
+      (uintptr_t)ctx->dag_cnt.p, (uintptr_t)ctx->sk_cnt.p, (uintptr_t)ctx->dag_sig,
+      (uintptr_t)ctx->tile_lists};
+  for (uintptr_t t : ctx->list_ptrs) key.push_back(t);
   for (int T : dsizes) key.push_back((uintptr_t)ctx->dag_lists[dag_list_key(ctx, T)].first.p);
   for (auto& g : ctx->pgraphs)
     if (g.key == key) {
@@ -628,6 +695,7 @@
   ctx->pgraphs.clear();
   for (DBuf* b : ctx_buffers(ctx)) release(ctx, *b);
   for (auto& kv : ctx->dag_lists) release(ctx, kv.second.first);
+  for (auto& kv : ctx->list_tabs) release(ctx, kv.second);
   for (hipEvent_t e : ctx->ev) (void)hipEventDestroy(e);
   for (hipEvent_t e : ctx->ph_ev) (void)hipEventDestroy(e);
   for (hipEvent_t e : ctx->sync_ev) (void)hipEventDestroy(e);
@@ -691,6 +759,7 @@
       ctx->dag_wgs = value;
       return 0;
     case GPS_OPT_FITC_DEP: ctx->fitc_dep = value != 0; return 0;
+    case GPS_OPT_TILE_LISTS: ctx->tile_lists = value != 0; return 0;
     case GPS_OPT_DAG_ORDER:
       ARGCHK(value >= 0 && value <= 2, "GPS_OPT_DAG_ORDER must be 0, 1 or 2");
       ctx->dag_order = value;
diff --git a/scoring-rules-for-gaussian-process-regression-a-new-approach-to-inference_amd/csrc/api_diag.hip b/scoring-rules-for-gaussian-process-regression-a-new-approach-to-inference_amd/csrc/api_diag.hip
--- a/scoring-rules-for-gaussian-process-regression-a-new-approach-to-inference_amd/csrc/api_diag.hip
+++ b/scoring-rules-for-gaussian-process-regression-a-new-approach-to-inference_amd/csrc/api_diag.hip
@@ -19,6 +19,8 @@
     }                       \
   } while (0)
   DIAG_REQ(d.dep_mode == 0, "dep_mode: the dependent row-norm launch cannot run alone");
+  DIAG_REQ(d.lists >= 0 && d.lists < 768 && (d.lists == 0 || (d.lists & 255)),
+           "lists must be 0 or 1 + c0 (c0 in 0..254) | kind << 8 (kind 0, 1, 2)");
   DIAG_REQ((d.lay_a == LAY_N || d.lay_a == LAY_T) && (d.lay_b == LAY_N || d.lay_b == LAY_T),
            "layouts must be 0 or 1");
   DIAG_REQ(d.epi == EPI_STORE || d.epi == EPI_ROWSQ || d.epi == EPI_COLRED || d.epi == EPI_ROWSQ_DOT,
@@ -115,6 +117,7 @@
   p.lower_out = d.lower_out; p.ksplit = d.ksplit; p.tri = d.tri; p.tri_off = d.tri_off;
   p.map_mode = d.map_mode; p.tile = d.tile; p.mirror = d.mirror; p.kend = d.kend;
   p.sk_alone = d.sk_alone;
+  p.lists = d.lists;
   return p;
 }
 static bool own_slabs(const gps_gemm_desc& d) {
diff --git a/scoring-rules-for-gaussian-process-regression-a-new-approach-to-inference_amd/csrc/api_internal.h b/scoring-rules-for-gaussian-process-regression-a-new-approach-to-inference_amd/csrc/api_internal.h
--- a/scoring-rules-for-gaussian-process-regression-a-new-approach-to-inference_amd/csrc/api_internal.h
+++ b/scoring-rules-for-gaussian-process-regression-a-new-approach-to-inference_amd/csrc/api_internal.h
@@ -109,6 +109,9 @@
   int* dag_sig = nullptr;
   DBuf dsig;
   std::map<int, std::pair<DBuf, int>> dag_lists;
+  bool tile_lists = true;
+  std::map<std::vector<int>, DBuf> list_tabs;
+  std::vector<uintptr_t> list_ptrs;
   std::map<uintptr_t, int64_t> zeroed;
   DBuf dag_cnt;
   DBuf sk_cnt;
diff --git a/scoring-rules-for-gaussian-process-regression-a-new-approach-to-inference_amd/csrc/gemm_schedule.h b/scoring-rules-for-gaussian-process-regression-a-new-approach-to-inference_amd/csrc/gemm_schedule.h
--- a/scoring-rules-for-gaussian-process-regression-a-new-approach-to-inference_amd/csrc/gemm_schedule.h
+++ b/scoring-rules-for-gaussian-process-regression-a-new-approach-to-inference_amd/csrc/gemm_schedule.h
@@ -125,6 +125,13 @@
   return valid;
 }
 
+GPS_HD int list_begin(const int* tab, int grid, int b) { return grid + tab[b]; }
+GPS_HD bool list_tile(const GemmParams& p, int v, int& ti, int& tj) {
+  ti = v >> 16;
+  tj = v & 0xffff;
+  return ti < p.tiles_m && tj < p.tiles_n;
+}
+
 struct StreamKPart {
   int64_t I, S;
   GPS_HD int64_t bnd(int64_t q) const { return q * I / S; }
diff --git a/scoring-rules-for-gaussian-process-regression-a-new-approach-to-inference_amd/csrc/gps_internal.h b/scoring-rules-for-gaussian-process-regression-a-new-approach-to-inference_amd/csrc/gps_internal.h
--- a/scoring-rules-for-gaussian-process-regression-a-new-approach-to-inference_amd/csrc/gps_internal.h
+++ b/scoring-rules-for-gaussian-process-regression-a-new-approach-to-inference_amd/csrc/gps_internal.h
@@ -69,6 +69,7 @@
   int kend;
   int sk_alone;
   int* dep_sig; int* dep_q; int* dep_err; int dep_grid; int dep_mode;
+  int lists; const int* list_tab; int list_grid;
 };
 constexpr int kSigStarted = 0;
 constexpr int kSigRowCnt = 64;
@@ -79,6 +80,9 @@
 struct GemmPlan { int tile, ksplit; };
 GemmPlan gemm_plan(int epi, const GemmParams& p, int64_t ws_cap_doubles);
 struct GemmLaunchInfo { int tile, ksplit, map_mode, sk_dp, sk_wgs, slab_xcd, grid_x, grid_y; };
+constexpr int kListDealtOver = 4;
+constexpr int kListProdTile = 128;
+std::vector<int32_t> tile_lists_build(const GemmParams& q, int tile, int grid);
 extern int g_gram_reg;
 extern int g_tiny_gemm;
 extern int g_stream_k;
diff --git a/scoring-rules-for-gaussian-process-regression-a-new-approach-to-inference_amd/csrc/kernels_gemm.hip b/scoring-rules-for-gaussian-process-regression-a-new-approach-to-inference_amd/csrc/kernels_gemm.hip
--- a/scoring-rules-for-gaussian-process-regression-a-new-approach-to-inference_amd/csrc/kernels_gemm.hip
+++ b/scoring-rules-for-gaussian-process-regression-a-new-approach-to-inference_amd/csrc/kernels_gemm.hip
@@ -1,3 +1,8 @@
+#include <algorithm>
+#include <cmath>
+#include <queue>
+#include <vector>
+
 #include "gemm_schedule.h"
 #include "gps_internal.h"
 
@@ -137,6 +142,19 @@
   const int nblk = p.sk_wgs > 0 ? p.sk_dp : (int)gridDim.x;
   if (!tile_of(p, remap ? xcd_remap(blockIdx.x, nblk) : (int)blockIdx.x, ti, tj)) return;
   gemm_tile<ALAY, BLAY, EPI, TILE>(p, ti, tj, blockIdx.y, smem);
+}
+
+template <int ALAY, int BLAY, int TILE>
+__global__ __launch_bounds__(256) void gemm_f64_list_kernel(GemmParams p) {
+  constexpr int STAGE = 2 * BK * (TILE + 16);
+  __shared__ __attribute__((aligned(16))) double smem[2 * STAGE];
+  for (int e = list_begin(p.list_tab, p.list_grid, (int)blockIdx.x);; ++e) {
+    const int v = p.list_tab[e];
+    int ti, tj;
+    if (v < 0 || !list_tile(p, v, ti, tj)) return;
+    gemm_tile<ALAY, BLAY, EPI_STORE, TILE>(p, ti, tj, 0, smem);
+    __syncthreads();
+  }
 }
 
 template <int TILE>
@@ -648,6 +666,153 @@
   return {64, ks};
 }
 
+std::vector<int32_t> tile_lists_build(const GemmParams& q, int tile, int grid) {
+  const int c0 = (q.lists & 255) - 1, kind = (q.lists >> 8) & 3;
+  struct Item { int32_t v; int cost; };
+  const bool wi = q.tri == TRI_K_LE_I || q.tri == TRI_K_GE_I;
+  const bool down = q.tri == TRI_K_LE_I || q.tri == TRI_K_LE_J;
+  const int nb = wi ? q.tiles_n : q.tiles_m, nw = wi ? q.tiles_m : q.tiles_n;
+  auto cost_of = [&](int ti, int tj) {
+    int kb, ke;
+    tile_k_range(q, ti * tile, tj * tile, tile, kb, ke);
+    if (q.kend > 0 && ke > q.kend) ke = q.kend;
+    return (ke > kb ? (ke - kb) / BK : 0) + c0;
+  };
+  std::vector<Item> seq;
+  seq.reserve((size_t)nb * nw);
+  int64_t total = 0;
+  for (int bi = 0; bi < nb; ++bi)
+    for (int wk = 0; wk < nw; ++wk) {
+      const int widx = down ? nw - 1 - wk : wk;
+      const int ti = wi ? widx : bi, tj = wi ? bi : widx;
+      seq.push_back({(int32_t)(ti << 16 | tj), cost_of(ti, tj)});
+      total += seq.back().cost;
+    }
+  std::vector<std::vector<Item>> lists((size_t)grid);
+  auto pack = [&]() {
+    int64_t packed_max = 0;
+    int cls_n[8], last = 0;
+    for (int x = 0; x < 8; ++x) {
+      cls_n[x] = x < grid ? (grid - x + 7) / 8 : 0;
+      if (cls_n[x]) last = x;
+    }
+    std::vector<Item> part[8];
+    int x = 0, blocks = cls_n[0];
+    int64_t cum = 0;
+    for (const Item& it : seq) {
+      while (x < last && 2 * cum + it.cost > 2 * total * blocks / grid) blocks += cls_n[++x];
+      part[x].push_back(it);
+      cum += it.cost;
+    }
+    static const double slacks[] = {0.0, 0.0025, 0.005, 0.01, 0.015, 0.02, 0.03, 0.05};
+    for (x = 0; x < 8; ++x) {
+      const int n = cls_n[x];
+      if (!n) continue;
+      std::stable_sort(part[x].begin(), part[x].end(),
+                       [](const Item& a, const Item& b) { return a.cost > b.cost; });
+      int64_t w = 0;
+      for (const Item& it : part[x]) w += it.cost;
+      std::vector<int> best_bin;
+      int64_t best_max = -1;
+      for (double sl : slacks) {
+        const int64_t cap = (int64_t)std::ceil((double)w / n * (1.0 + sl));
+        std::vector<int64_t> load((size_t)n, 0);
+        std::vector<int> bin(part[x].size());
+        for (size_t i = 0; i < part[x].size(); ++i) {
+          int fit = -1, low = 0;
+          for (int j = 0; j < n; ++j) {
+            if (load[j] + part[x][i].cost <= cap && (fit < 0 || load[j] > load[fit])) fit = j;
+            if (load[j] < load[low]) low = j;
+          }
+          bin[i] = fit >= 0 ? fit : low;
+          load[bin[i]] += part[x][i].cost;
+        }
+        const int64_t mx = *std::max_element(load.begin(), load.end());
+        if (best_max < 0 || mx < best_max) {
+          best_max = mx;
+          best_bin = bin;
+        }
+      }
+      {
+        std::vector<int64_t> load((size_t)n, 0);
+        for (size_t i = 0; i < part[x].size(); ++i) load[(size_t)best_bin[i]] += part[x][i].cost;
+        for (int round = 0; round < 4096; ++round) {
+          const int a = (int)(std::max_element(load.begin(), load.end()) - load.begin());
+          int64_t best = load[(size_t)a];
+          size_t mi = 0, mj = 0;
+          int mb = -1;
+          bool swap = false;
+          for (size_t i = 0; i < part[x].size(); ++i) {
+            if (best_bin[i] != a) continue;
+            const int ci = part[x][i].cost;
+            for (int b = 0; b < n; ++b) {
+              const int64_t v = std::max(load[(size_t)a] - ci, load[(size_t)b] + ci);
+              if (b != a && v < best) { best = v; mi = i; mb = b; swap = false; }
+            }
+            for (size_t j = 0; j < part[x].size(); ++j) {
+              const int b = best_bin[j], dc = ci - part[x][j].cost;
+              if (b == a || dc <= 0) continue;
+              const int64_t v = std::max(load[(size_t)a] - dc, load[(size_t)b] + dc);
+              if (v < best) { best = v; mi = i; mj = j; mb = b; swap = true; }
+            }
+          }
+          if (mb < 0) break;
+          const int d = part[x][mi].cost - (swap ? part[x][mj].cost : 0);
+          load[(size_t)a] -= d;
+          load[(size_t)mb] += d;
+          best_bin[mi] = mb;
+          if (swap) best_bin[mj] = a;
+        }
+        best_max = *std::max_element(load.begin(), load.end());
+      }
+      for (size_t i = 0; i < part[x].size(); ++i) lists[(size_t)(x + 8 * best_bin[i])].push_back(part[x][i]);
+      packed_max = std::max(packed_max, best_max);
+    }
+    return packed_max;
+  };
+  auto deal_out = [&](std::vector<std::vector<Item>>& deal) {
+    GemmParams m = q;
+    m.map_mode = 3;
+    const int span = wi ? 8 * ((q.tiles_n + 7) / 8) * q.tiles_m : 8 * ((q.tiles_m + 7) / 8) * q.tiles_n;
+    typedef std::pair<int64_t, int> Slot;
+    std::priority_queue<Slot, std::vector<Slot>, std::greater<Slot>> free_at;
+    for (int j = 0; j < grid; ++j) free_at.push({0, j});
+    int64_t mx = 0;
+    for (int t = 0; t < span; ++t) {
+      int ti, tj;
+      if (!tile_of(m, t, ti, tj)) continue;
+      Slot s = free_at.top();
+      free_at.pop();
+      const int c = cost_of(ti, tj);
+      deal[(size_t)s.second].push_back({(int32_t)(ti << 16 | tj), c});
+      s.first += c;
+      mx = std::max(mx, s.first);
+      free_at.push(s);
+    }
+    for (auto& l : deal)
+      std::stable_sort(l.begin(), l.end(), [](const Item& a, const Item& b) { return a.cost > b.cost; });
+    return mx;
+  };
+  const bool many = (int64_t)seq.size() > (int64_t)kListDealtOver * grid;
+  if (kind == 2 || (kind == 0 && many)) {
+    deal_out(lists);
+  } else {
+    const int64_t packed_max = pack();
+    if (kind == 0) {
+      std::vector<std::vector<Item>> deal((size_t)grid);
+      if (deal_out(deal) < packed_max) lists.swap(deal);
+    }
+  }
+  std::vector<int32_t> tab((size_t)grid + seq.size() + (size_t)grid);
+  int32_t e = 0;
+  for (int b = 0; b < grid; ++b) {
+    tab[(size_t)b] = e;
+    for (const Item& it : lists[(size_t)b]) tab[(size_t)grid + (size_t)e++] = it.v;
+    tab[(size_t)grid + (size_t)e++] = -1;
+  }
+  return tab;
+}
+
 hipError_t launch_gemm(int alay, int blay, int epi, const GemmParams& pin, hipStream_t s,
                        GemmLaunchInfo* info, GemmParams* resolved) {
   GemmParams p = pin;
@@ -741,6 +906,13 @@
     tiles = (q.tri == TRI_K_LE_I || q.tri == TRI_K_GE_I) ? 8 * ((q.tiles_n + 7) / 8) * q.tiles_m
                                                           : 8 * ((q.tiles_m + 7) / 8) * q.tiles_n;
   }
+  q.list_grid = 0;
+  if (q.lists > 0 && q.sk_slots > 0 && epi == EPI_STORE && q.map_mode == 3 && q.ksplit == 1 &&
+      q.tiles_m < 32768 && q.tiles_n < 32768 && (int64_t)q.tiles_m * q.tiles_n > q.sk_slots) {
+    if (!resolved && !q.list_tab) return hipErrorInvalidValue;
+    q.list_grid = q.sk_slots;
+    tiles = q.list_grid;
+  }
   q.sk_dp = q.sk_wgs = 0;
   if ((g_stream_k == 1 || (g_stream_k == 2 && q.sk_alone)) && epi == EPI_STORE && tile == 128 &&
       q.ksplit == 1 && q.sk_cnt && q.ws &&
@@ -758,12 +930,26 @@
   q.slab_xcd = g_slab_xcd && q.ksplit > 1 && q.sk_wgs == 0 &&
                (q.map_mode == 0 || q.map_mode == 2) && (q.lower_out || q.tri == TRI_NONE);
   dim3 grid(tiles, q.ksplit), block(256);
-  if (info) *info = {tile, q.ksplit, q.map_mode, q.sk_dp, q.sk_wgs, q.slab_xcd, tiles, q.ksplit};
+  if (info)
+    *info = {tile, q.ksplit, q.list_grid ? 7 : q.map_mode, q.sk_dp, q.sk_wgs, q.slab_xcd, tiles, q.ksplit};
   if (resolved) {
     *resolved = q;
     return hipSuccess;
   }
   hipError_t err = hipErrorInvalidValue;
+  if (q.list_grid > 0) {
+#define GPS_LIST_CASE(AL, BL, T)                                                      \
+    if (err == hipErrorInvalidValue && alay == AL && blay == BL && tile == T) {      \
+      hipLaunchKernelGGL((gemm_f64_list_kernel<AL, BL, T>), grid, block, 0, s, q);   \
+      err = hipGetLastError();                                                        \
+    }
+    GPS_LIST_CASE(LAY_N, LAY_T, 128) GPS_LIST_CASE(LAY_N, LAY_N, 128)
+    GPS_LIST_CASE(LAY_T, LAY_N, 128) GPS_LIST_CASE(LAY_T, LAY_T, 128)
+    GPS_LIST_CASE(LAY_N, LAY_T, 64) GPS_LIST_CASE(LAY_N, LAY_N, 64)
+    GPS_LIST_CASE(LAY_T, LAY_N, 64) GPS_LIST_CASE(LAY_T, LAY_T, 64)
+#undef GPS_LIST_CASE
+    return err;
+  }
 #define GPS_GEMM_CASE(AL, BL, EP, T)                                                        \
   if (err == hipErrorInvalidValue && alay == AL && blay == BL && epi == EP && tile == T) { \
     hipLaunchKernelGGL((gemm_f64_kernel<AL, BL, EP, T>), grid, block, 0, s, q);            \
@@ -839,6 +1025,7 @@
   };
   const bool rowsq = epi == EPI_ROWSQ || epi == EPI_ROWSQ_DOT;
   const bool remap = q.map_mode == 2 || (q.map_mode == 0 && q.tri == TRI_NONE);
+  std::vector<int32_t> list_tab;
   for (int by = 0; by < info.grid_y; ++by)
     for (int bx = 0; bx < info.grid_x; ++bx) {
       const int wg = bx + by * info.grid_x;
@@ -862,6 +1049,13 @@
         }
         continue;
       }
+      if (q.list_grid > 0) {
+        if (bx == 0) list_tab = tile_lists_build(q, tile, q.list_grid);
+        for (int e = list_begin(list_tab.data(), q.list_grid, bx);
+             list_tab[(size_t)e] >= 0 && list_tile(q, list_tab[(size_t)e], ti, tj); ++e)
+          tile_item(wg, ti, tj, 0);
+        continue;
+      }
       if (rowsq && q.map_mode == 6) {
         int ri, c, ch;
         const bool second = pair_of(q, bx, info.grid_x, ri, c, ch);
diff --git a/scoring-rules-for-gaussian-process-regression-a-new-approach-to-inference_amd/gpscore/_lib.py b/scoring-rules-for-gaussian-process-regression-a-new-approach-to-inference_amd/gpscore/_lib.py
--- a/scoring-rules-for-gaussian-process-regression-a-new-approach-to-inference_amd/gpscore/_lib.py
+++ b/scoring-rules-for-gaussian-process-regression-a-new-approach-to-inference_amd/gpscore/_lib.py
@@ -7,7 +7,7 @@
 
 _HERE = os.path.dirname(os.path.abspath(__file__))
 LIB_PATH = os.environ.get("GPSCORE_LIB", os.path.join(_HERE, "libgpscore.so"))
-ABI_VERSION = 800
+ABI_VERSION = 810
 GPS_N_STATS = 6
 GPS_COMM_NONE, GPS_COMM_RCCL, GPS_COMM_LOCAL = 0, 1, 2
 COMM_KINDS = {GPS_COMM_NONE: "none", GPS_COMM_RCCL: "rccl", GPS_COMM_LOCAL: "local"}
@@ -25,6 +25,8 @@
 GPS_OPT_DAG_ORDER = 25
 GPS_OPT_SLAB_XCD = 26
 GPS_OPT_FITC_DEP = 27
+GPS_OPT_TILE_LISTS = 28
+GPS_TILE_LIST_C0 = 2
 GPS_OPT_AR_CHUNKS = 15
 OBJ_NAMES = ("nlml", "loo_crps", "loo_logs", "logdet", "quad")
 SURFACE_NAMES = ("loo_crps", "insample_crps", "nlml", "loo_logs")
@@ -48,7 +50,7 @@
                 ("kend", ctypes.c_int32),
                 ("tile", ctypes.c_int32), ("ksplit", ctypes.c_int32), ("map_mode", ctypes.c_int32),
                 ("use_ws", ctypes.c_int32), ("sk_alone", ctypes.c_int32),
-                ("dep_mode", ctypes.c_int32), ("reserved", ctypes.c_int32),
+                ("dep_mode", ctypes.c_int32), ("lists", ctypes.c_int32),
                 ("ld_out", _c_i64), ("c_kslice_stride", _c_i64)]
 
 
@@ -282,6 +284,9 @@
         if tiles is not None:
             self.call("gps_ctx_set_option", GPS_OPT_DAG_TILES, int(tiles))
 
+    def set_tile_lists(self, on=True):
+        self.call("gps_ctx_set_option", GPS_OPT_TILE_LISTS, 1 if on else 0)
+
     def set_pred_pre(self, on=True):
         self.call("gps_ctx_set_option", GPS_OPT_PRED_PRE, 1 if on else 0)
 
```

Result: no change. 8.152 fit+predict+score units/s (C3 full GP, whole job) (median of 6 runs) (+0.8%).
